# DecaYale/SYN3R

Hardware: AMD Instinct MI355X
Metric: llff_3view_train_loop_iters_per_sec (higher is better)
Workload: dtype f32 raster / f16 UNet (f32 accumulate); 1 GPU; LLFF fern-like 3-view block: 50 raster fwd+bwd iters (l1 loss) (200000 Gaussians, 1920x1080, SH3) + 1 SVD (step,pass): CFG UNet fwd [2,14,8,72,128] f16 + fused Euler step; frames=14, parallelism=scene-parallel x1

## Files before the change

include/syn3r_hip.h:

```cpp
#ifndef SYN3R_HIP_H
#define SYN3R_HIP_H

#include <stddef.h>
#include <stdint.h>

#ifdef __cplusplus
extern "C" {
#endif

#define SYN3R_OK 0
#define SYN3R_E_INVALID (-1)
#define SYN3R_E_WORKSPACE (-2)
#define SYN3R_E_HIP (-3)

#define SYN3R_F32 0
#define SYN3R_F16 1

const char* syn3r_last_error(void);
int syn3r_version(void);
const char* syn3r_arch(void);

int syn3r_trace_enable(int on);
void* syn3r_trace_session(void);
int syn3r_trace_attach(void* session);
// ... 119 lines not shown
                              float* dL_dconfidence, void* workspace, size_t workspace_bytes, int raw, int flags,
                              const float* filter3d, void* stream);
int syn3r_raster_backward_abs(int N, int sh_degree, int sh_coeffs, long long P, const float* means3D,
                              const float* scales, const float* rotations, const float* opacities, const float* shs,
                              const float* confidence, float scale_modifier, const float* viewmatrix,
                              const float* projmatrix, const float* campos, float tanfovx, float tanfovy, int H, int W,
                              const float* bg, const int* radii, void* geom, size_t geom_bytes,
                              const unsigned* point_list, void* image, size_t image_bytes, const float* dL_dcolor,
                              const float* dL_ddepth, const float* dL_dalpha, float* dL_dmeans3D, float* dL_dscales,
                              float* dL_drotations, float* dL_dopacities, float* dL_dshs, float* dL_dmeans2D,
                              float* dL_dconfidence, void* workspace, size_t workspace_bytes, int raw, int flags,
                              const float* filter3d, float* dL_dmeans2D_abs, void* stream);
size_t syn3r_raster_backward_cam_workspace_bytes(int N);
int syn3r_raster_backward_cam(int N, int sh_degree, int sh_coeffs, long long P, const float* means3D,
                              const float* scales, const float* rotations, const float* opacities, const float* shs,
                              const float* confidence, float scale_modifier, const float* viewmatrix,
                              const float* projmatrix, const float* campos, float tanfovx, float tanfovy, int H, int W,
                              const float* bg, const int* radii, void* geom, size_t geom_bytes,
                              const unsigned* point_list, void* image, size_t image_bytes, const float* dL_dcolor,
                              const float* dL_ddepth, const float* dL_dalpha, float* dL_dmeans3D, float* dL_dscales,
                              float* dL_drotations, float* dL_dopacities, float* dL_dshs, float* dL_dmeans2D,
                              float* dL_dconfidence, void* workspace, size_t workspace_bytes, int raw, int flags,
                              const float* filter3d, float* dL_dmeans2D_abs, float* dL_dcamera, int accumulate,
                              void* stream);

size_t syn3r_sort_pairs_workspace_bytes(long long n);
int syn3r_sort_pairs(unsigned long long* keys, unsigned* vals, unsigned long long* keys_tmp, unsigned* vals_tmp,
                     long long n, int nbits, void* workspace, size_t workspace_bytes, int* result_in_tmp,
                     void* stream);


int syn3r_gemm_f16(const void* A, long long lda, const void* W, void* out, long long ldc, const void* bias,
                   const void* rowvec, long long ldrv, int rows_per_vec, int rv_group_rows, const void* residual, long long ldr,
                   const void* aux, long long ldaux, float s_acc, float s_res, float s_aux, int M, int N, int K,
                   void* gn_partials, size_t gn_partials_bytes, int* gn_written, void* stream);

int syn3r_gemm_2src_supported(int M, int N, int K1, int K2, long long lda1, long long lda2);
int syn3r_gemm_2src_f16(const void* A1, long long lda1, int K1, const void* A2, long long lda2, int K2, const void* W,
                        void* out, long long ldc, const void* bias, int M, int N, void* gn_partials, size_t gn_partials_bytes,
                        int* gn_written, void* stream);

int syn3r_gemm_set_tile(int bm);

int syn3r_gemm_set_splitk_workspace(void* workspace, size_t bytes);

int syn3r_gemm_geglu_f16(const void* A, long long lda, const void* Wpacked, const void* bias_packed, void* out,
                         long long ldc, int M, int D, int K, void* stream);

size_t syn3r_feedforward_workspace_bytes(int M, int D);
int syn3r_feedforward_f16(const void* x, long long ldx, const void* w1_packed, const void* b1_packed, int D,
                          const void* w2, const void* b2, void* out, long long ldc, const void* residual,
                          long long ldr, const void* aux, long long ldaux, float s_acc, float s_res, float s_aux,
                          int M, int C_in, int C_out, void* workspace, size_t workspace_bytes, void* stream);

int syn3r_feedforward_p64_supported(int M, int D, int C_in);
int syn3r_feedforward_p64_f16(const void* x, long long ldx, const void* w1_packed64, const void* b1_packed64, int D,
                              const void* w2, const void* b2, void* out, long long ldc, const void* residual,
                              long long ldr, const void* aux, long long ldaux, float s_acc, float s_res, float s_aux,
                              int M, int C_in, int C_out, void* workspace, size_t workspace_bytes, void* stream);

int syn3r_feedforward_fused_f16(const void* x, long long ldx, const void* w1_chunked, const void* b1_chunked, int D,
                                const void* w2, const void* b2, void* out, long long ldc, const void* residual,
                                long long ldr, const void* aux, long long ldaux, float s_acc, float s_res, float s_aux,
                                int M, int C, void* stream);

int syn3r_feedforward_fused_ln_f16(const void* x, long long ldx, const void* ln_gamma, const void* ln_beta, float ln_eps,
                                   const void* w1_chunked, const void* b1_chunked, int D, const void* w2, const void* b2,
                                   void* out, long long ldc, const void* residual, long long ldr, const void* aux,
                                   long long ldaux, float s_acc, float s_res, float s_aux, int M, int C, void* stream);

int syn3r_feedforward_fused_addln_f16(const void* x, long long ldx, const void* addvec, int rows_per_vec, const void* ln_gamma,
                                      const void* ln_beta, float ln_eps, const void* w1_chunked, const void* b1_chunked, int D,
                                      const void* w2, const void* b2, void* out, long long ldc, const void* aux, long long ldaux,
                                      float s_acc, float s_res, float s_aux, int M, int C, void* stream);

int syn3r_layernorm_linear320_f16(const void* x, long long ldx, const void* ln_gamma, const void* ln_beta, float ln_eps,
                                  const void* W, void* out, long long ldc, int M, int N, int C, void* stream);

int syn3r_conv2d3x3_f16(const void* X, const void* W, void* out, long long ldc, const void* bias,
                        const void* rowvec, long long ldrv, int rows_per_vec, const void* residual, long long ldr,
                        float s_acc, float s_res, int NB, int Hi, int Wi, int Cin, int Cout, int stride, int upsample,
                        int pad_lo, void* gn_partials, size_t gn_partials_bytes, int* gn_written, void* stream);

int syn3r_tconv3_f16(const void* X, const void* W, void* out, long long ldc, const void* bias, const void* rowvec,
                     long long ldrv, int rows_per_vec, const void* residual, long long ldr, float s_acc, float s_res,
                     int B, int F, int HW, int Cin, int Cout, void* gn_partials, size_t gn_partials_bytes, int* gn_written,
                     void* stream);

int syn3r_attention_f16(const void* q, const void* k, const void* v, long long ld, void* out, long long ldo,
                        int nseq, int S, int heads, void* stream);

int syn3r_attention_temporal_f16(const void* q, const void* k, const void* v, long long ld, void* out,
                                 long long ldo, int B, int F, int HW, int heads, void* stream);

size_t syn3r_groupnorm_workspace_bytes(int samples, int rows);
int syn3r_groupnorm_f16(const void* x, void* y, int samples, int rows, int C, const void* gamma, const void* beta,
                        float eps, int silu, void* workspace, size_t workspace_bytes, void* stream);
int syn3r_groupnorm_2src_f16(const void* x1, int C1, const void* x2, int C2, void* y, int samples, int rows,
                             const void* gamma, const void* beta, float eps, int silu, void* workspace,
                             size_t workspace_bytes, void* stream);
size_t syn3r_gn_partials_bytes(int M, int N);
int syn3r_groupnorm_pre_f16(const void* x1, int C1, const void* part1, const void* x2, int C2, const void* part2, void* y,
                            int samples, int rows, const void* gamma, const void* beta, float eps, int silu,
                            void* workspace, size_t workspace_bytes, void* stream);

int syn3r_layernorm_f16(const void* x, void* y, void* xsum, const void* addvec, int rows_per_vec, long long M,
                        int C, const void* gamma, const void* beta, float eps, void* stream);

int syn3r_geglu_f16(const void* x, void* y, long long M, int D, void* stream);

int syn3r_softmax_rows_f16(const void* x, void* y, long long M, int N, long long ld, float scale, void* stream);

int syn3r_time_conv_out(const void* x, long long ldx, const float* w, const float* bias, float* out, int B, int F,
                        long long HW, void* stream);


size_t syn3r_l1_loss_workspace_bytes(long long n);
int syn3r_l1_loss(const float* image, const float* target, long long n, float weight, float* loss, void* ws,
                  size_t ws_bytes, void* stream);
int syn3r_l1_loss_backward(const float* image, const float* target, long long n, float weight,
                           const float* grad_loss, float* grad_image, void* stream);

int syn3r_image_mse(const float* image, const float* target, long long n, float* mse, void* ws, size_t ws_bytes,
                    void* stream);

size_t syn3r_photo_loss_workspace_bytes(int C, int H, int W);
int syn3r_photo_loss(const float* image, const float* target, int C, int H, int W, float lambda_dssim, float weight,
                     float* loss3, void* ws, size_t ws_bytes, void* stream);
int syn3r_photo_loss_backward(const float* image, const float* target, int C, int H, int W, float lambda_dssim,
                              float weight, const float* grad_loss, const void* ws, float* grad_image, void* stream);
int syn3r_photo_loss_step(const float* image, const float* target, int C, int H, int W, float lambda_dssim, float weight,
                          const float* grad_loss, float* loss3, float* grad_image, void* ws, size_t ws_bytes, void* stream);

size_t syn3r_photo_loss_map_workspace_bytes(int C, int H, int W);
int syn3r_photo_loss_map(const float* image, const float* target, const float* map, int C, int H, int W, float lambda_dssim,
                         float weight, float* loss4, void* ws, size_t ws_bytes, void* stream);
int syn3r_photo_loss_map_backward(const float* image, const float* target, const float* map, int C, int H, int W,
                                  float lambda_dssim, float weight, const float* grad_loss, const void* ws, float* grad_image,
                                  void* stream);
int syn3r_photo_loss_map_step(const float* image, const float* target, const float* map, int C, int H, int W, float lambda_dssim,
                              float weight, const float* grad_loss, float* loss4, float* grad_image, void* ws, size_t ws_bytes,
                              void* stream);
int syn3r_l1_loss_map(const float* image, const float* target, const float* map, long long n, long long plane, float weight,
                      float* loss, void* ws, size_t ws_bytes, void* stream);
int syn3r_l1_loss_map_backward(const float* image, const float* target, const float* map, long long n, long long plane,
                               float weight, const float* grad_loss, float* grad_image, void* stream);

#define SYN3R_DCORR_MIN 0
#define SYN3R_DCORR_A 1
#define SYN3R_DCORR_B 2
size_t syn3r_depth_corr_loss_workspace_bytes(long long n);
int syn3r_depth_corr_loss(const float* depth, const float* prior, long long n, float weight, float offset, int mode, float* parts,
                          void* ws, size_t ws_bytes, void* stream);
int syn3r_depth_corr_loss_backward(const float* depth, const float* prior, long long n, float weight, float offset, int mode,
                                   const float* grad_loss, const void* ws, size_t ws_bytes, float* grad_depth, void* stream);
int syn3r_depth_corr_loss_step(const float* depth, const float* prior, long long n, float weight, float offset, int mode,
                               const float* grad_loss, float* parts, float* grad_depth, void* ws, size_t ws_bytes, void* stream);

int syn3r_exposure_apply(const float* image, const float* A, int H, int W, float* out, void* stream);
size_t syn3r_exposure_backward_workspace_bytes(int H, int W);
int syn3r_exposure_backward(const float* image, const float* A, const float* grad_out, int H, int W, float* grad_image, float* grad_A,
                            int accumulate, void* ws, size_t ws_bytes, void* stream);

int syn3r_adam_step(float* param, const float* grad, float* exp_avg, float* exp_avg_sq, long long n, float lr,
                    float beta1, float beta2, float eps, int step, void* stream);
int syn3r_adam_step_multi(int count, float* const* params, const float* const* grads, float* const* exp_avgs,
// ... 74 lines not shown
```

syn3r_amd/_lib.py:

```python
from __future__ import annotations

import ctypes as C
from pathlib import Path

import torch

_LIB_PATH = Path(__file__).resolve().parent / "lib" / "libsyn3r_hip.so"
_lib = None

c_f = C.c_float
c_i = C.c_int
c_p = C.c_void_p
c_sz = C.c_size_t
c_ll = C.c_longlong
c_d = C.c_double

F32, F16 = 0, 1
RASTER_ANTIALIAS = 1

FILTER3D_VARIANCE, FILTER3D_NEAR, FILTER3D_MARGIN = 0.2, 0.2, 0.15

_SCENE = [c_p, c_p, c_p, c_p, c_p, c_p, c_f, c_p, c_p, c_p, c_f, c_f, c_i, c_i]
_RASTER_PREPROCESS = [c_i, c_i, c_i] + _SCENE + [c_p, c_p, c_sz, C.POINTER(c_ll)]
_RASTER_BACKWARD = ([c_i, c_i, c_i, c_ll] + _SCENE + [c_p, c_p, c_p, c_sz, c_p, c_p, c_sz]
                    + [c_p] * 10 + [c_p, c_sz])
_STREAM, _EX, _F3D, _ABS = [c_p], [c_i, c_i, c_p], [c_i, c_i, c_p, c_p], [c_i, c_i, c_p, c_p, c_p]
_CAM = [c_i, c_i, c_p, c_p, c_p, c_i, c_p]
CAMERA_GRAD = 35

SIGNATURES = {
    "syn3r_last_error": (C.c_char_p, []),
    "syn3r_version": (c_i, []),
    "syn3r_arch": (C.c_char_p, []),
    "syn3r_trace_enable": (c_i, [c_i]),
    "syn3r_trace_filter": (c_i, [C.c_char_p]),
    "syn3r_trace_report": (c_i, [C.c_char_p, c_sz]),
    "syn3r_trace_session": (c_p, []),
    "syn3r_trace_attach": (c_i, [c_p]),
    "syn3r_inverse_warp_workspace_bytes": (c_sz, [c_i]),
    "syn3r_inverse_warp": (c_i, [c_p, c_p, c_p, c_p, c_p, c_p, c_p, c_f, c_i, c_i, c_i,
                                 c_p, c_p, c_p, c_p, c_p, c_p, c_p, c_p, c_p, c_p, c_p, c_p, c_sz, c_p]),
    "syn3r_reproj_error": (c_i, [c_p, c_p, c_p, c_p, c_p, c_p, c_p, c_i, c_i, c_p, c_p]),
    "syn3r_warp_post": (c_i, [c_p, c_p, c_p, c_i, c_i, c_i, c_i, c_i, c_p, c_p, c_p, c_p, c_p, c_p, c_p]),
    "syn3r_fuse_uncertainty": (c_i, [c_p, c_p, c_p, c_i, c_i, c_i, c_i, c_i, c_p, c_p, c_p, c_p]),
    "syn3r_forward_warp_workspace_bytes": (c_sz, [c_i, c_i]),
    "syn3r_forward_warp": (c_i, [c_p, c_p, c_p, c_p, c_p, c_p, c_i, c_i, c_p, c_p, c_p, c_p, c_sz, c_p]),
    "syn3r_step_workspace_bytes": (c_sz, [c_i, c_i, c_i, c_i]),
    "syn3r_step_interp": (c_i, [c_p, c_i, c_p, c_i, c_p, c_p, c_p, c_f, c_f, c_f, c_f, c_f, c_f, c_i,
                                c_p, c_p, c_p, c_i, c_i, c_i, c_i, c_p, c_sz, c_p]),
    "syn3r_step_replace": (c_i, [c_p, c_i, c_p, c_i, c_p, c_p, c_p, c_f, c_f, c_f, c_f,
                                 c_p, c_p, c_i, c_i, c_i, c_i, c_p, c_sz, c_p]),
    "syn3r_raster_geom_bytes": (c_sz, [c_i]),
    "syn3r_raster_image_bytes": (c_sz, [c_i, c_i]),
    "syn3r_raster_binning_bytes": (c_sz, [c_ll]),
    "syn3r_raster_preprocess": (c_i, _RASTER_PREPROCESS + _STREAM),
    "syn3r_raster_preprocess_raw": (c_i, _RASTER_PREPROCESS + _STREAM),
    "syn3r_raster_preprocess_ex": (c_i, _RASTER_PREPROCESS + _EX),
    "syn3r_raster_preprocess_f3d": (c_i, _RASTER_PREPROCESS + _F3D),
    "syn3r_raster_render": (c_i, [c_i, c_i, c_i, c_p, c_p, c_p, c_sz, c_p, c_sz, c_p, c_sz, c_ll, c_p, c_p, c_p,
                                  C.POINTER(c_p), c_p]),
    "syn3r_raster_backward_workspace_bytes": (c_sz, [c_i]),
    "syn3r_raster_backward": (c_i, _RASTER_BACKWARD + _STREAM),
    "syn3r_raster_backward_raw": (c_i, _RASTER_BACKWARD + _STREAM),
    "syn3r_raster_backward_ex": (c_i, _RASTER_BACKWARD + _EX),
    "syn3r_raster_backward_f3d": (c_i, _RASTER_BACKWARD + _F3D),
    "syn3r_raster_backward_abs": (c_i, _RASTER_BACKWARD + _ABS),
    "syn3r_raster_backward_cam_workspace_bytes": (c_sz, [c_i]),
    "syn3r_raster_backward_cam": (c_i, _RASTER_BACKWARD + _CAM),
    "syn3r_filter3d_workspace_bytes": (c_sz, [c_i]),
    "syn3r_filter3d_compute": (c_i, [c_p, c_i, c_p, c_i, c_f, c_f, c_f, c_p, c_p, c_sz, c_p]),
    "syn3r_sort_pairs_workspace_bytes": (c_sz, [c_ll]),
    "syn3r_sort_pairs": (c_i, [c_p, c_p, c_p, c_p, c_ll, c_i, c_p, c_sz, C.POINTER(c_i), c_p]),
    "syn3r_gaussian_activate": (c_i, [c_i, c_p, c_p, c_p, c_p, c_p, c_p, c_p]),
    "syn3r_gaussian_activate_backward": (c_i, [c_i, c_p, c_p, c_p, c_p, c_p, c_p, c_p, c_p, c_p, c_p, c_p]),
    "syn3r_densification_stats": (c_i, [c_i, c_p, c_p, c_p, c_p, c_p, c_p]),
    "syn3r_densification_stats_abs": (c_i, [c_i, c_p, c_p, c_p, c_p, c_p, c_p, c_p, c_p]),
    "syn3r_gemm_f16": (c_i, [c_p, c_ll, c_p, c_p, c_ll, c_p, c_p, c_ll, c_i, c_i, c_p, c_ll, c_p, c_ll, c_f, c_f, c_f,
                             c_i, c_i, c_i, c_p, c_sz, C.POINTER(c_i), c_p]),
    "syn3r_gemm_set_tile": (c_i, [c_i]),
    "syn3r_gemm_geglu_f16": (c_i, [c_p, c_ll, c_p, c_p, c_p, c_ll, c_i, c_i, c_i, c_p]),
    "syn3r_feedforward_workspace_bytes": (c_sz, [c_i, c_i]),
    "syn3r_feedforward_f16": (c_i, [c_p, c_ll, c_p, c_p, c_i, c_p, c_p, c_p, c_ll, c_p, c_ll, c_p, c_ll, c_f, c_f, c_f,
                                    c_i, c_i, c_i, c_p, c_sz, c_p]),
    "syn3r_feedforward_p64_f16": (c_i, [c_p, c_ll, c_p, c_p, c_i, c_p, c_p, c_p, c_ll, c_p, c_ll, c_p, c_ll, c_f, c_f, c_f,
                                    c_i, c_i, c_i, c_p, c_sz, c_p]),
    "syn3r_feedforward_p64_supported": (c_i, [c_i, c_i, c_i]),
    "syn3r_feedforward_fused_f16": (c_i, [c_p, c_ll, c_p, c_p, c_i, c_p, c_p, c_p, c_ll, c_p, c_ll, c_p, c_ll, c_f, c_f, c_f,
                                          c_i, c_i, c_p]),
    "syn3r_feedforward_fused_ln_f16": (c_i, [c_p, c_ll, c_p, c_p, c_f, c_p, c_p, c_i, c_p, c_p, c_p, c_ll, c_p, c_ll, c_p, c_ll,
                                             c_f, c_f, c_f, c_i, c_i, c_p]),
    "syn3r_feedforward_fused_addln_f16": (c_i, [c_p, c_ll, c_p, c_i, c_p, c_p, c_f, c_p, c_p, c_i, c_p, c_p, c_p, c_ll, c_p, c_ll,
                                                c_f, c_f, c_f, c_i, c_i, c_p]),
    "syn3r_layernorm_linear320_f16": (c_i, [c_p, c_ll, c_p, c_p, c_f, c_p, c_p, c_ll, c_i, c_i, c_i, c_p]),
    "syn3r_conv2d3x3_f16": (c_i, [c_p, c_p, c_p, c_ll, c_p, c_p, c_ll, c_i, c_p, c_ll, c_f, c_f,
                                  c_i, c_i, c_i, c_i, c_i, c_i, c_i, c_i, c_p, c_sz, C.POINTER(c_i), c_p]),
    "syn3r_tconv3_f16": (c_i, [c_p, c_p, c_p, c_ll, c_p, c_p, c_ll, c_i, c_p, c_ll, c_f, c_f,
                               c_i, c_i, c_i, c_i, c_i, c_p, c_sz, C.POINTER(c_i), c_p]),
    "syn3r_attention_f16": (c_i, [c_p, c_p, c_p, c_ll, c_p, c_ll, c_i, c_i, c_i, c_p]),
    "syn3r_attention_temporal_f16": (c_i, [c_p, c_p, c_p, c_ll, c_p, c_ll, c_i, c_i, c_i, c_i, c_p]),
    "syn3r_groupnorm_workspace_bytes": (c_sz, [c_i, c_i]),
    "syn3r_groupnorm_f16": (c_i, [c_p, c_p, c_i, c_i, c_i, c_p, c_p, c_f, c_i, c_p, c_sz, c_p]),
    "syn3r_groupnorm_2src_f16": (c_i, [c_p, c_i, c_p, c_i, c_p, c_i, c_i, c_p, c_p, c_f, c_i, c_p, c_sz, c_p]),
    "syn3r_groupnorm_pre_f16": (c_i, [c_p, c_i, c_p, c_p, c_i, c_p, c_p, c_i, c_i, c_p, c_p, c_f, c_i, c_p, c_sz, c_p]),
    "syn3r_gn_partials_bytes": (c_sz, [c_i, c_i]),
    "syn3r_gemm_2src_supported": (c_i, [c_i, c_i, c_i, c_i, c_ll, c_ll]),
    "syn3r_gemm_2src_f16": (c_i, [c_p, c_ll, c_i, c_p, c_ll, c_i, c_p, c_p, c_ll, c_p, c_i, c_i, c_p, c_sz, C.POINTER(c_i), c_p]),
    "syn3r_layernorm_f16": (c_i, [c_p, c_p, c_p, c_p, c_i, c_ll, c_i, c_p, c_p, c_f, c_p]),
    "syn3r_geglu_f16": (c_i, [c_p, c_p, c_ll, c_i, c_p]),
    "syn3r_softmax_rows_f16": (c_i, [c_p, c_p, c_ll, c_i, c_ll, c_f, c_p]),
    "syn3r_time_conv_out": (c_i, [c_p, c_ll, c_p, c_p, c_p, c_i, c_i, c_ll, c_p]),
    "syn3r_l1_loss_workspace_bytes": (c_sz, [c_ll]),
    "syn3r_l1_loss": (c_i, [c_p, c_p, c_ll, c_f, c_p, c_p, c_sz, c_p]),
    "syn3r_l1_loss_backward": (c_i, [c_p, c_p, c_ll, c_f, c_p, c_p, c_p]),
    "syn3r_image_mse": (c_i, [c_p, c_p, c_ll, c_p, c_p, c_sz, c_p]),
    "syn3r_photo_loss_workspace_bytes": (c_sz, [c_i, c_i, c_i]),
    "syn3r_photo_loss": (c_i, [c_p, c_p, c_i, c_i, c_i, c_f, c_f, c_p, c_p, c_sz, c_p]),
    "syn3r_photo_loss_backward": (c_i, [c_p, c_p, c_i, c_i, c_i, c_f, c_f, c_p, c_p, c_p, c_p]),
    "syn3r_photo_loss_step": (c_i, [c_p, c_p, c_i, c_i, c_i, c_f, c_f, c_p, c_p, c_p, c_p, c_sz, c_p]),
    "syn3r_photo_loss_map_workspace_bytes": (c_sz, [c_i, c_i, c_i]),
    "syn3r_photo_loss_map": (c_i, [c_p, c_p, c_p, c_i, c_i, c_i, c_f, c_f, c_p, c_p, c_sz, c_p]),
    "syn3r_photo_loss_map_backward": (c_i, [c_p, c_p, c_p, c_i, c_i, c_i, c_f, c_f, c_p, c_p, c_p, c_p]),
    "syn3r_photo_loss_map_step": (c_i, [c_p, c_p, c_p, c_i, c_i, c_i, c_f, c_f, c_p, c_p, c_p, c_p, c_sz, c_p]),
    "syn3r_l1_loss_map": (c_i, [c_p, c_p, c_p, c_ll, c_ll, c_f, c_p, c_p, c_sz, c_p]),
    "syn3r_l1_loss_map_backward": (c_i, [c_p, c_p, c_p, c_ll, c_ll, c_f, c_p, c_p, c_p]),
    "syn3r_depth_corr_loss_workspace_bytes": (c_sz, [c_ll]),
    "syn3r_depth_corr_loss": (c_i, [c_p, c_p, c_ll, c_f, c_f, c_i, c_p, c_p, c_sz, c_p]),
    "syn3r_depth_corr_loss_backward": (c_i, [c_p, c_p, c_ll, c_f, c_f, c_i, c_p, c_p, c_sz, c_p, c_p]),
    "syn3r_depth_corr_loss_step": (c_i, [c_p, c_p, c_ll, c_f, c_f, c_i, c_p, c_p, c_p, c_p, c_sz, c_p]),
    "syn3r_exposure_apply": (c_i, [c_p, c_p, c_i, c_i, c_p, c_p]),
    "syn3r_exposure_backward_workspace_bytes": (c_sz, [c_i, c_i]),
    "syn3r_exposure_backward": (c_i, [c_p, c_p, c_p, c_i, c_i, c_p, c_p, c_i, c_p, c_sz, c_p]),
    "syn3r_adam_step": (c_i, [c_p, c_p, c_p, c_p, c_ll, c_f, c_f, c_f, c_f, c_i, c_p]),
    "syn3r_adam_step_multi": (c_i, [c_i, c_p, c_p, c_p, c_p, c_p, c_p, c_f, c_f, c_p, c_p, c_p]),
    "syn3r_adam_step_multi_rows": (c_i, [c_i, c_p, c_p, c_p, c_p, c_p, c_p, c_p, c_p, c_p, c_f, c_f, c_p, c_p, c_p]),
    "syn3r_knn3_workspace_bytes": (c_sz, [c_i]),
    "syn3r_knn3_mean_dist2": (c_i, [c_p, c_i, c_p, c_p, c_sz, c_p]),
    "syn3r_knn3_graph_workspace_bytes": (c_sz, [c_i]),
    "syn3r_knn3_graph": (c_i, [c_p, c_i, c_p, c_p, c_p, c_sz, c_p]),
    "syn3r_gaussian_unpool_workspace_bytes": (c_sz, [c_i]),
    "syn3r_gaussian_unpool_count": (c_i, [c_p, c_p, c_i, c_f, c_f, c_p, c_p, c_sz, c_p]),
    "syn3r_gaussian_unpool_emit": (c_i, [c_p, c_p, c_p, c_p, c_p, c_i, c_i, c_i, c_p, c_p, c_p, c_p, c_p, c_p, c_sz, c_p]),
    "syn3r_conv2d3x3_act_f16": (c_i, [c_p, c_p, c_p, c_p, c_i, c_p, c_i, c_i, c_i, c_i, c_i, c_p]),
    "syn3r_lpips_image_f16": (c_i, [c_p, c_i, c_i, c_p, c_p]),
    "syn3r_lpips_image_bwd": (c_i, [c_p, c_i, c_i, c_f, c_p, c_p]),
    "syn3r_maxpool2_f16": (c_i, [c_p, c_i, c_i, c_i, c_p, c_p]),
    "syn3r_maxpool2_bwd_f16": (c_i, [c_p, c_p, c_i, c_i, c_i, c_p, c_p]),
    "syn3r_lpips_layer_workspace_bytes": (c_sz, [c_ll, c_i]),
    "syn3r_lpips_layer_f16": (c_i, [c_p, c_p, c_p, c_ll, c_i, c_i, c_p, c_p, c_sz, c_p]),
    "syn3r_lpips_layer_bwd_f16": (c_i, [c_p, c_p, c_p, c_ll, c_i, c_f, c_i, c_p, c_p]),
    "syn3r_conv2d3x3_split_f16": (c_i, [c_p, c_p, c_p, c_ll, c_p, c_i, c_i, c_p, c_ll, c_i, c_i, c_i, c_i, c_i, c_p]),
    "syn3r_lpips_image_split_f16": (c_i, [c_p, c_i, c_i, c_p, c_p]),
    "syn3r_maxpool2_split_f16": (c_i, [c_p, c_i, c_i, c_i, c_p, c_p]),
    "syn3r_maxpool2_bwd_split_f16": (c_i, [c_p, c_p, c_i, c_i, c_i, c_p, c_p]),
    "syn3r_lpips_layer_split_f16": (c_i, [c_p, c_p, c_p, c_ll, c_i, c_i, c_p, c_p, c_sz, c_p]),
    "syn3r_lpips_layer_bwd_split_f16": (c_i, [c_p, c_p, c_p, c_ll, c_i, c_f, c_i, c_p, c_p]),
    "syn3r_pcd_outlier_workspace_bytes": (c_sz, [c_i]),
    "syn3r_pcd_statistical_outlier": (c_i, [c_p, c_i, c_i, c_d, c_p, c_p, c_p, c_p, c_sz, c_p]),
    "syn3r_flow_cycle_mask": (c_i, [c_p, c_p, c_i, c_i, c_i, c_f, c_p, c_p, c_p]),
    "syn3r_gemm_set_splitk_workspace": (c_i, [c_p, c_sz]),
    "syn3r_unet_create": (c_i, [C.c_char_p, C.c_char_p, C.POINTER(c_p)]),
    "syn3r_unet_destroy": (c_i, [c_p]),
    "syn3r_unet_workspace_bytes": (c_sz, [c_p, c_i, c_i, c_i, c_i, c_i]),
    "syn3r_unet_forward": (c_i, [c_p, c_p, c_d, c_p, c_i, c_p, c_p, c_i, c_i, c_i, c_i, c_i, c_p, c_sz, c_p]),
}


class Syn3rError(RuntimeError):
    pass


def lib_path() -> Path:
    return _LIB_PATH


def set_library_path(path) -> None:
    global _LIB_PATH
    if _lib is not None:
        raise Syn3rError("set_library_path() after the library was loaded")
# ... 119 lines not shown
```

syn3r_amd/csrc/gemm.hip:

```cpp
#include "common.h"
#include <cstdlib>
#include <algorithm>
#include <atomic>
#include <type_traits>

using namespace syn3r;

namespace {

#include "gemm_common.h"
#include "gemm_dma160.h"
#include "gemm_dma.h"
#include "gemm_wide.h"
#include "gemm_z.h"
#include "gemm_dmap.h"
#include "gemm_dmapd.h"
#include "gemm_g256.h"
#include "gemm_ffn.h"

int persistent_blocks() {
    static std::atomic<int> cus_of[64];
    static const int forced = tune_env("SYN3R_PERSISTENT_BLOCKS", 0);
    if (forced > 0) return forced < 8 ? 8 : forced;
    int dev = 0;
// ... 1 lines not shown
    int n = cus_of[dev].load(std::memory_order_relaxed);
    if (n == 0) {
        int v = 0;
        n = (hipDeviceGetAttribute(&v, hipDeviceAttributeMultiprocessorCount, dev) == hipSuccess && v > 0) ? v : 256;
        if (n < 8) n = 8;
        cus_of[dev].store(n, std::memory_order_relaxed);
    }
    return n;
}

size_t gn_partials_bytes(long long M, long long N) { return (size_t)(M / 32) * 2 * (size_t)(N / 10) * sizeof(float); }
int gn_request(GemmParams& p, void* buf, size_t bytes, const char* who) {
    SYN3R_REQUIRE((buf == nullptr) == (bytes == 0), "%s: gn_partials pointer and size must both be given or both be zero", who);
    SYN3R_REQUIRE(((uintptr_t)buf % 16) == 0, "%s: the gn_partials buffer must be 16-byte aligned", who);
    if (!buf || p.M % 32 != 0 || p.N % 80 != 0 || p.geglu_D > 0 || p.out_tiled || bytes < gn_partials_bytes(p.M, p.N)) return SYN3R_OK;
    p.gn_part = (float*)buf; p.gn_units = p.N / 10;
    return SYN3R_OK;
}

template <void (*KERNEL)(GemmParams)>
int launch_tiles(const char* family, size_t lds, long long grid, int block, hipStream_t stream, const GemmParams& q, int* gn_written,
                 const char* base, int b0 = 0, int b1 = 0) {
    static DevOnce once;
    if (int rc = set_max_lds(once, (const void*)KERNEL, (int)lds, family)) return rc;
    char name[96];
    if (trace_on()) {
        const int n = snprintf(name, sizeof(name), base, b0, b1);
        if (trace_detail()) snprintf(name + n, sizeof(name) - n, "[M%d,N%d,K%d,e%d]", q.M, q.N, q.K, q.geglu_D > 0 ? 2 : (q.residual != nullptr));
    }
    SYN3R_LAUNCH_NAMED(name, KERNEL, dim3((unsigned)grid), dim3(block), lds, stream, q);
    hipError_t e = hipGetLastError();
    if (e != hipSuccess) { set_error("%s launch: %s", family, hipGetErrorString(e)); return SYN3R_E_HIP; }
    if (gn_written) *gn_written = q.gn_part != nullptr;
    return SYN3R_OK;
}

long long wide_tiles(const GemmParams& p) { return (long long)((p.M + WBM - 1) / WBM) * ((p.N + WBN - 1) / WBN); }
bool wide_fills(const GemmParams& p) {
    const long long tiles = wide_tiles(p), rounds = (tiles + 255) / 256;
    return tiles * 10 >= rounds * 256 * 8;
}

int band_width(const GemmParams& p) {
    static const int band_env = tune_env("SYN3R_Z_BAND", 0);
    if (band_env > 0) return band_env;
    return ((p.N + WBN - 1) / WBN > 4 && p.K <= 640) ? 3 : 4;
}

int launch_widep(const GemmParams& p, hipStream_t stream, int* gn_written) {
    constexpr size_t lds = (size_t)2 * W_STAGE + 16384;
    static_assert(8 * WM * EPI_LD * sizeof(__half) <= lds - W_STAGE, "epilogue staging must fit behind ring slot 0");
    GemmParams q = p;
    q.band = band_width(p);
    return launch_tiles<k_gemm_widep>("gemm_widep", lds, std::min<long long>(wide_tiles(p), persistent_blocks()), 512, stream, q, gn_written, "k_gemm_widep");
}

bool g256_admits(const GemmParams& p) {
    return p.geglu_D > 0 && p.bias != nullptr && p.out_tiled && !p.a_tiled && !p.A2 && !p.rowvec && !p.residual && !p.aux && p.s_acc == 1.0f && p.M % 128 == 0 && p.M >= 256 &&
           p.geglu_D % 128 == 0 && p.N == 2 * p.geglu_D && p.K >= 2 * BK && p.lda % 8 == 0 && (long long)p.M * p.lda < (1ll << 31) &&
           (long long)p.N * p.K < (1ll << 31);
}
int launch_g256(const GemmParams& p, hipStream_t stream) {
    const int tiles = ((p.M + 255) / 256) * (p.N / 256);
    GemmParams q = p;
    static const int band_env = tune_env("SYN3R_G256_BAND", 0);
    q.band = band_env > 0 ? band_env : 4;
    return launch_tiles<k_gemm_g256>("gemm_g256", G_LDS, std::min(tiles, persistent_blocks()), 512, stream, q, nullptr, "k_gemm_g256");
}

template <int MODE = MODE_DENSE>
int launch_z(const GemmParams& p, hipStream_t stream, int* gn_written) {
    const long long blocks = std::min<long long>(wide_tiles(p), persistent_blocks());
    GemmParams q = p;
    q.band = band_width(p);
    if constexpr (MODE == MODE_CONV2D) q.a_bytes = (unsigned)((long long)(p.M / (p.Ho * p.Wo)) * p.Hi * p.Wi * p.Cin * 2);
    if constexpr (MODE == MODE_TCONV) q.a_bytes = (unsigned)((long long)p.M * p.Cin * 2);
    if constexpr (MODE == MODE_DENSE) {
        if (p.A2) return launch_tiles<k_gemm_z<true, MODE_DENSE>>("gemm_z", Z_LDS, blocks, 512, stream, q, gn_written, "k_gemm_z<%d>", MODE);
    }
    if constexpr (MODE == MODE_CONV2D) {
        if (p.ups) return launch_tiles<k_gemm_z<false, MODE_CONV2D, true>>("gemm_z", Z_LDS, blocks, 512, stream, q, gn_written, "k_gemm_z<%d>", MODE);
    }
    return launch_tiles<k_gemm_z<false, MODE>>("gemm_z", Z_LDS, blocks, 512, stream, q, gn_written, "k_gemm_z<%d>", MODE);
}

thread_local int g_dma_bm = 0;
thread_local void* g_splitk_ws = nullptr;
thread_local size_t g_splitk_bytes = 0;

int wide_launch(const GemmParams& p, hipStream_t stream, int* gn_written) {
    static const int z_env = tune_env("SYN3R_GEMM_Z", -1);
    const bool z = g_dma_bm == -322 ? true : (g_dma_bm == -320 ? false : (z_env < 0 ? p.geglu_D > 0 : z_env != 0));
    return z ? launch_z<MODE_DENSE>(p, stream, gn_written) : launch_widep(p, stream, gn_written);
}

bool widep_admits(const GemmParams& p) {
    const bool lean = (!p.rowvec || p.geglu_D <= 0) && (!p.aux || p.residual) && (p.geglu_D <= 0 || (p.geglu_D % 8 == 0 && p.s_acc == 1.0f));
    const bool small = (p.a_tiled ? (long long)((p.M + 127) / 128) * 128 * p.K : (long long)p.M * p.lda) < (1ll << 31) &&
                       (long long)p.N * p.K < (1ll << 31) && (!p.A2 || (long long)p.M * p.lda2 < (1ll << 31));
    return lean && small && p.M % 8 == 0 && p.N % 8 == 0 && p.M >= 8 && p.N >= 8;
}

long long tiles256(const GemmParams& p) { return (long long)((p.M + 255) / 256) * ((p.N + BN - 1) / BN); }

int launch_dmapd(const GemmParams& p, hipStream_t stream) {
    return launch_tiles<k_gemm_dmapd>("gemm_dmapd", DMA256_LDS, std::min<long long>(tiles256(p), persistent_blocks()), 512, stream, p, nullptr, "k_gemm_dmapd");
}

bool dmapd_admits(const GemmParams& p) {
    return p.geglu_D <= 0 && !p.A2 && !p.a_tiled && !p.out_tiled && !p.out_nt && !p.relu && !p.relu_mask && p.ksplit <= 1 && !p.aux &&
           !p.res_add && p.M % 256 == 0 && p.N % BN == 0 && p.K / BK >= 4 && p.ldc % 8 == 0 && (!p.residual || p.ldr % 8 == 0) &&
           (!p.rowvec || p.ldrv % 4 == 0);
}

template <int MODE>
int launch_dmap(const GemmParams& p, hipStream_t stream, int* gn_written) {
    static_assert(8 * 32 * EPI_LD * sizeof(__half) <= DMA256_STAGE, "the two-pass epilogue staging must fit in one ring slot");
    GemmParams q = p;
    q.tc_pb = q.tc_nf = 0;
    if constexpr (MODE == MODE_TCONV) {
        static const int tc_env = tune_env("SYN3R_TCONV_ORDER", 1);
        if (tc_env != 0 && p.HW % 256 == 0 && p.M % p.HW == 0 && p.M / p.HW > 1) { q.tc_pb = p.HW / 256; q.tc_nf = p.M / p.HW; }
    }
    return launch_tiles<k_gemm_dmap<MODE>>("gemm_dmap", DMA256_LDS, std::min<long long>(tiles256(p), persistent_blocks()), 512, stream, q, gn_written, "k_gemm_dmap<%d>", MODE);
}

template <int MODE, int BM>
int launch_dma_bm(const GemmParams& p, hipStream_t stream, int* gn_written) {
    if constexpr (BM == 256) {
        static const int pers_env = tune_env("SYN3R_DMA_PERSISTENT", 1);
        if (pers_env != 0 && MODE != MODE_CONV2D && p.geglu_D <= 0 && (!p.aux || p.residual) && p.N % 8 == 0 && p.N >= 8)
            return launch_dmap<MODE>(p, stream, gn_written);
    }
    constexpr size_t lds = BM == 256 ? DMA256_LDS : 2 * (BM * BK * 2 + DMA_B_BYTES);
    static_assert((BM / 32) * WM * EPI_LD * sizeof(__half) <= lds, "epilogue staging must fit in the ring");
    const int tiles = ((p.M + BM - 1) / BM) * ((p.N + BN - 1) / BN);
    return launch_tiles<k_gemm_dma<MODE, BM>>("gemm_dma", lds, tiles, BM * 2, stream, p, nullptr, "k_gemm_dma<%d,%d>", MODE, BM);
}

template <int MODE>
int launch_splitk(const GemmParams& p, hipStream_t stream, bool* done) {
    const long long tiles = tiles256(p);
    const int nkt_all = p.K / BK;
    const int S = (tiles * 4 <= 256 && nkt_all % 4 == 0 && nkt_all >= 16) ? 4 : ((tiles * 2 <= 256 && nkt_all % 2 == 0 && nkt_all >= 8) ? 2 : 1);
    const size_t need = (size_t)S * p.M * p.N * sizeof(float);
    if (S == 1 || g_dma_bm != 0 || !g_splitk_ws || need > g_splitk_bytes || p.N % 8 != 0 || p.M < 8 || p.relu || p.relu_mask ||
        p.geglu_D > 0 || p.out_tiled || (p.A2 && (MODE != MODE_DENSE || p.a_tiled || (p.K1 / BK) % (nkt_all / S) != 0)))
        return SYN3R_OK;
    GemmParams q = p;
    q.ksplit = S; q.split_ws = (float*)g_splitk_ws;
    if (int rc = launch_tiles<k_gemm_dma<MODE, 256>>("gemm split-K", DMA256_LDS, tiles * S, 512, stream, q, nullptr,
                                                     trace_detail() ? "k_gemm_dma<%d,256>/%d" : "k_gemm_dma<%d,256>/k", MODE, S))
        return rc;
    const long long chunks = (long long)p.M * (p.N / 8);
    SYN3R_LAUNCH(k_splitk_finish, dim3((unsigned)((chunks + 255) / 256)), dim3(256), 0, stream, q);
    SYN3R_LAUNCH_CHECK("gemm split-K launch");
    *done = true;
    return SYN3R_OK;
}

template <int MODE>
int launch_dma(const GemmParams& p, hipStream_t stream, int* gn_written = nullptr) {
    static const int wide_env = tune_env("SYN3R_GEMM_WIDE", -1);
    if constexpr (MODE == MODE_DENSE) {
        static const int ddw_env = tune_env("SYN3R_DMAPD_WIDE", 1);
        const bool won = p.residual ? (p.K >= 640 && p.K <= 1280 && p.N <= 1280) : (p.K == 1280 && p.N == 1280);
// ... 279 lines not shown
    return feedforward_fused(x, ldx, ln_gamma, ln_beta, ln_eps, w1_chunked, b1_chunked, D, w2, b2, out, ldc, residual, ldr, aux, ldaux,
                             s_acc, s_res, s_aux, M, C, stream);
}
extern "C" int syn3r_feedforward_fused_addln_f16(const void* x, long long ldx, const void* addvec, int rows_per_vec, const void* ln_gamma,
                                                 const void* ln_beta, float ln_eps, const void* w1_chunked, const void* b1_chunked, int D,
                                                 const void* w2, const void* b2, void* out, long long ldc, const void* aux, long long ldaux,
                                                 float s_acc, float s_res, float s_aux, int M, int C, void* stream) {
    SYN3R_REQUIRE(ln_gamma && ln_beta && addvec, "feedforward_fused_addln_f16: null LayerNorm parameters / add vector");
    SYN3R_REQUIRE(((uintptr_t)ln_gamma | (uintptr_t)ln_beta | (uintptr_t)addvec) % 16 == 0, "feedforward_fused_addln_f16: LayerNorm parameters and the add vector must be 16-byte aligned");
    SYN3R_REQUIRE(ln_eps > 0.f, "feedforward_fused_addln_f16: eps must be positive");
    SYN3R_REQUIRE(rows_per_vec > 0, "feedforward_fused_addln_f16: rows_per_vec=%d must be positive", rows_per_vec);
    return feedforward_fused(x, ldx, ln_gamma, ln_beta, ln_eps, w1_chunked, b1_chunked, D, w2, b2, out, ldc, x, ldx, aux, ldaux,
                             s_acc, s_res, s_aux, M, C, stream, addvec, rows_per_vec);
}
namespace {
int feedforward_fused(const void* x, long long ldx, const void* ln_gamma, const void* ln_beta, float ln_eps, const void* w1_chunked,
                      const void* b1_chunked, int D, const void* w2, const void* b2, void* out, long long ldc, const void* residual,
                      long long ldr, const void* aux, long long ldaux, float s_acc, float s_res, float s_aux, int M, int C, void* stream,
                      const void* addvec, int rows_per_vec) {
    SYN3R_REQUIRE(x && w1_chunked && b1_chunked && w2 && out, "feedforward_fused_f16: null operand");
    SYN3R_REQUIRE(C == F_C, "feedforward_fused_f16: the fused kernel is built for C = %d channels (got %d): use syn3r_feedforward_f16", F_C, C);
    SYN3R_REQUIRE(M > 0 && D >= F_HC && D % F_HC == 0, "feedforward_fused_f16: bad sizes M=%d D=%d (D must be a multiple of %d)", M, D, F_HC);
    FfnParams q{};
    GemmParams& p = q.e;
    p.A = (const __half*)x; p.lda = ldx; p.W = (const __half*)w2; p.out = (__half*)out; p.ldc = ldc;
    p.bias = (const __half*)b2; p.residual = (const __half*)residual; p.ldr = ldr; p.aux = (const __half*)aux; p.ldaux = ldaux;
    p.s_acc = s_acc; p.s_res = s_res; p.s_aux = s_aux; p.M = M; p.N = F_C; p.K = D;
    q.w1 = (const __half*)w1_chunked; q.b1 = (const __half*)b1_chunked; q.D = D;
    q.ln_g = (const __half*)ln_gamma; q.ln_b = (const __half*)ln_beta; q.ln_eps = ln_eps;
    q.ln_add = (const __half*)addvec; q.ln_add_rpv = rows_per_vec; p.res_add = (const __half*)addvec; p.res_add_rpv = rows_per_vec;
    int rc = check_common(p, "feedforward_fused_f16");
    if (rc) return rc;
    SYN3R_REQUIRE(ldx % 8 == 0 && ldx >= C, "feedforward_fused_f16: ldx=%lld must be >= C and a multiple of 8", ldx);
    SYN3R_REQUIRE(((uintptr_t)w1_chunked | (uintptr_t)b1_chunked) % 16 == 0, "feedforward_fused_f16: weights must be 16-byte aligned");
    return launch_ffn320(q, (hipStream_t)stream);
}
}

extern "C" int syn3r_layernorm_linear320_f16(const void* x, long long ldx, const void* ln_gamma, const void* ln_beta, float ln_eps,
                                             const void* W, void* out, long long ldc, int M, int N, int C, void* stream) {
    SYN3R_REQUIRE(x && ln_gamma && ln_beta && W && out, "layernorm_linear320_f16: null operand");
    SYN3R_REQUIRE(C == F_C, "layernorm_linear320_f16: the kernel is built for C = %d channels (got %d): use syn3r_layernorm_f16 + syn3r_gemm_f16", F_C, C);
    SYN3R_REQUIRE(SYN3R_DIM_OK(M) && SYN3R_DIM_OK(N) && N % F_C == 0, "layernorm_linear320_f16: bad sizes M=%d N=%d (N must be a multiple of %d)", M, N, F_C);
    SYN3R_REQUIRE(ldx % 8 == 0 && ldx >= C && ldc % 8 == 0 && ldc >= N, "layernorm_linear320_f16: bad strides ldx=%lld ldc=%lld", ldx, ldc);
    SYN3R_REQUIRE(((uintptr_t)x | (uintptr_t)ln_gamma | (uintptr_t)ln_beta | (uintptr_t)W | (uintptr_t)out) % 16 == 0, "layernorm_linear320_f16: operands must be 16-byte aligned");
    SYN3R_REQUIRE(ln_eps > 0.f, "layernorm_linear320_f16: eps must be positive");
    SYN3R_REQUIRE((long long)M * ldx < (1ll << 40) && (long long)M * ldc < (1ll << 40), "layernorm_linear320_f16: operand too large");
    LnLinParams p{};
    p.x = (const __half*)x; p.ldx = ldx; p.W = (const __half*)W; p.out = (__half*)out; p.ldc = ldc; p.M = M; p.N = N; p.C = C;
    p.ln_g = (const __half*)ln_gamma; p.ln_b = (const __half*)ln_beta; p.ln_eps = ln_eps;
    return launch_lnlin320(p, (hipStream_t)stream);
}

extern "C" int syn3r_conv2d3x3_f16(const void* X, const void* W, void* out, long long ldc, const void* bias,
                                   const void* rowvec, long long ldrv, int rows_per_vec, const void* residual,
                                   long long ldr, float s_acc, float s_res, int NB, int Hi, int Wi, int Cin, int Cout,
                                   int stride, int upsample, int pad_lo, void* gn_partials, size_t gn_partials_bytes, int* gn_written,
                                   void* stream) {
    if (gn_written) *gn_written = 0;
    SYN3R_REQUIRE(NB > 0 && Hi > 0 && Wi > 0 && Cin > 0 && Cout > 0, "conv2d3x3: bad sizes");
    SYN3R_REQUIRE(pad_lo == 0 || pad_lo == 1, "conv2d3x3: pad_lo must be 0 or 1");
    SYN3R_REQUIRE(stride == 1 || stride == 2, "conv2d3x3: stride must be 1 or 2");
    SYN3R_REQUIRE(!(upsample && stride != 1), "conv2d3x3: upsample requires stride 1");
    SYN3R_REQUIRE(Cin % BK == 0, "conv2d3x3: Cin=%d must be a multiple of %d (pad the input channels)", Cin, BK);
    GemmParams p{};
    p.A = (const __half*)X; p.W = (const __half*)W; p.out = (__half*)out; p.ldc = ldc; p.bias = (const __half*)bias;
    p.rowvec = (const __half*)rowvec; p.ldrv = ldrv; p.rows_per_vec = rows_per_vec;
    p.residual = (const __half*)residual; p.ldr = ldr; p.s_acc = s_acc; p.s_res = s_res; p.s_aux = 0.f;
    p.Hi = Hi; p.Wi = Wi; p.Cin = Cin; p.stride = stride; p.ups = upsample ? 1 : 0; p.pad = pad_lo;
    int Hg = upsample ? 2 * Hi : Hi, Wg = upsample ? 2 * Wi : Wi;
    p.Ho = (Hg + pad_lo + 1 - 3) / stride + 1;
    p.Wo = (Wg + pad_lo + 1 - 3) / stride + 1;
    SYN3R_REQUIRE(p.Ho > 0 && p.Wo > 0, "conv2d3x3: input too small");
    long long M = (long long)NB * p.Ho * p.Wo;
    SYN3R_REQUIRE(M < (1ll << 31), "conv2d3x3: too many output pixels");
    p.M = (int)M; p.N = Cout; p.K = 9 * Cin;
    int rc = gn_request(p, gn_partials, gn_partials_bytes, "conv2d3x3");
    if (rc) return rc;
    rc = check_common(p, "conv2d3x3");
    if (rc) return rc;
    return launch_dma<MODE_CONV2D>(p, (hipStream_t)stream, gn_written);
}

extern "C" int syn3r_conv2d3x3_act_f16(const void* X, const void* W, void* out, const void* bias, int relu, const void* relu_mask,
                                       int NB, int Hi, int Wi, int Cin, int Cout, void* stream) {
    SYN3R_REQUIRE(NB > 0 && Hi > 0 && Wi > 0 && Cin > 0 && Cout > 0, "conv2d3x3_act: bad sizes");
    SYN3R_REQUIRE(Cin % BK == 0 && Cout % 8 == 0, "conv2d3x3_act: Cin=%d must be a multiple of %d, Cout=%d of 8", Cin, BK, Cout);
    GemmParams p{};
    p.A = (const __half*)X; p.W = (const __half*)W; p.out = (__half*)out; p.ldc = Cout; p.bias = (const __half*)bias;
    p.s_acc = 1.0f; p.s_res = 0.f; p.s_aux = 0.f;
    p.relu = relu ? 1 : 0; p.relu_mask = (const __half*)relu_mask;
    p.Hi = Hi; p.Wi = Wi; p.Cin = Cin; p.stride = 1; p.ups = 0; p.pad = 1; p.Ho = Hi; p.Wo = Wi;
    long long M = (long long)NB * Hi * Wi;
    SYN3R_REQUIRE(M < (1ll << 31), "conv2d3x3_act: too many output pixels");
    p.M = (int)M; p.N = Cout; p.K = 9 * Cin;
    int rc = check_common(p, "conv2d3x3_act");
    if (rc) return rc;
    SYN3R_REQUIRE(((uintptr_t)relu_mask % 16) == 0, "conv2d3x3_act: mask must be 16-byte aligned");
    return launch_dma<MODE_CONV2D>(p, (hipStream_t)stream);
}

extern "C" int syn3r_conv2d3x3_split_f16(const void* X, const void* W, void* out, long long ld_out, const void* bias, int relu, int split_out,
                                         const void* relu_mask, long long ld_mask, int NB, int Hi, int Wi, int Cin, int Cout, void* stream) {
    SYN3R_REQUIRE(NB > 0 && Hi > 0 && Wi > 0 && Cin > 0 && Cout > 0, "conv2d3x3_split: bad sizes");
    SYN3R_REQUIRE(Cin % BK == 0 && Cout % 8 == 0, "conv2d3x3_split: Cin=%d must be a multiple of %d, Cout=%d of 8", Cin, BK, Cout);
    SYN3R_REQUIRE(ld_out >= (split_out ? 2ll : 1ll) * Cout, "conv2d3x3_split: ld_out=%lld is short of %d columns", ld_out, (split_out ? 2 : 1) * Cout);
    SYN3R_REQUIRE(!(split_out && relu_mask), "conv2d3x3_split: a mask goes with the plain output only");
    SYN3R_REQUIRE(!relu_mask || (ld_mask >= Cout && ld_mask % 8 == 0 && ld_mask < (1ll << 31)), "conv2d3x3_split: bad mask stride %lld", ld_mask);
    GemmParams p{};
    p.A = (const __half*)X; p.W = (const __half*)W; p.out = (__half*)out; p.ldc = ld_out; p.bias = (const __half*)bias;
    p.s_acc = 1.0f; p.s_res = 0.f; p.s_aux = 0.f;
    p.relu = relu ? 1 : 0; p.relu_mask = (const __half*)relu_mask; p.ld_mask = (int)ld_mask;
    p.Hi = Hi; p.Wi = Wi; p.Cin = Cin; p.stride = 1; p.ups = 0; p.pad = 1; p.Ho = Hi; p.Wo = Wi;
    long long M = (long long)NB * Hi * Wi;
    SYN3R_REQUIRE(M < (1ll << 31), "conv2d3x3_split: too many output pixels");
    p.M = (int)M; p.N = Cout; p.K = 9 * Cin;
    int rc = check_common(p, "conv2d3x3_split");
    if (rc) return rc;
    SYN3R_REQUIRE((((uintptr_t)relu_mask | (uintptr_t)bias) % 16) == 0, "conv2d3x3_split: mask and bias must be 16-byte aligned");
    static_assert(8 * WM * EPI_LD * sizeof(__half) <= DMA256_LDS, "one staged fp16 plane must fit in the ring");
    if (split_out)
        return launch_tiles<k_gemm_dma<MODE_CONV2D, 256, EPI_SPLIT_OUT>>("conv split", DMA256_LDS, tiles256(p), 512, (hipStream_t)stream, p, nullptr, "k_gemm_dma<1,256,split>");
    return launch_tiles<k_gemm_dma<MODE_CONV2D, 256, EPI_SPLIT_MASK>>("conv split", DMA256_LDS, tiles256(p), 512, (hipStream_t)stream, p, nullptr, "k_gemm_dma<1,256,mask>");
}

extern "C" int syn3r_tconv3_f16(const void* X, const void* W, void* out, long long ldc, const void* bias,
                                const void* rowvec, long long ldrv, int rows_per_vec, const void* residual,
                                long long ldr, float s_acc, float s_res, int B, int F, int HW, int Cin, int Cout,
                                void* gn_partials, size_t gn_partials_bytes, int* gn_written, void* stream) {
    if (gn_written) *gn_written = 0;
    SYN3R_REQUIRE(B > 0 && F > 0 && HW > 0 && Cin > 0 && Cout > 0, "tconv3: bad sizes");
    SYN3R_REQUIRE(Cin % BK == 0, "tconv3: Cin=%d must be a multiple of %d", Cin, BK);
    GemmParams p{};
    p.A = (const __half*)X; p.W = (const __half*)W; p.out = (__half*)out; p.ldc = ldc; p.bias = (const __half*)bias;
    p.rowvec = (const __half*)rowvec; p.ldrv = ldrv; p.rows_per_vec = rows_per_vec;
    p.residual = (const __half*)residual; p.ldr = ldr; p.s_acc = s_acc; p.s_res = s_res; p.s_aux = 0.f;
    p.F = F; p.HW = HW; p.Cin = Cin;
    long long M = (long long)B * F * HW;
    SYN3R_REQUIRE(M < (1ll << 31), "tconv3: too many rows");
    p.M = (int)M; p.N = Cout; p.K = 3 * Cin;
    int rc = gn_request(p, gn_partials, gn_partials_bytes, "tconv3");
    if (rc) return rc;
    rc = check_common(p, "tconv3");
    if (rc) return rc;
    return launch_dma<MODE_TCONV>(p, (hipStream_t)stream, gn_written);
}

#ifdef SYN3R_TIMING
extern "C" __attribute__((visibility("default"))) int syn3r_debug_wide_timing(unsigned long long* out64) {
    return (int)hipMemcpyFromSymbol(out64, HIP_SYMBOL(g_wide_timing), sizeof(unsigned long long) * 64);
}
extern "C" __attribute__((visibility("default"))) int syn3r_debug_g256_timing(unsigned long long* out64) {
    return (int)hipMemcpyFromSymbol(out64, HIP_SYMBOL(g_g256_timing), sizeof(unsigned long long) * 64);
}
#endif
```

syn3r_amd/csrc/gemm_common.h:

```cpp


typedef _Float16 half8 __attribute__((ext_vector_type(8)));
typedef float float4v __attribute__((ext_vector_type(4)));
typedef unsigned u32x4 __attribute__((ext_vector_type(4)));

constexpr int BN = 160, BK = 64;
constexpr int WM = 64, WN = 80;
constexpr int TM = WM / 16, TN = WN / 16;
constexpr int B_TILE = BN * BK;
constexpr int EPI_LD = 88;

enum { MODE_DENSE = 0, MODE_CONV2D = 1, MODE_TCONV = 2 };

__device__ __forceinline__ int rowvec_index(int m, int rows_per_vec, int rv_group) {
    if (rows_per_vec > 0) return m / rows_per_vec;
    const int P = -rows_per_vec;
    return (rv_group > 0 ? (m / rv_group) * P : 0) + m % P;
}

struct GemmParams {
    const __half* A; long long lda;
    const __half* W;
    __half* out; long long ldc;
    const __half* bias;
    const __half* rowvec; long long ldrv; int rows_per_vec;
    int rv_group;
    const __half* residual; long long ldr;
    const __half* aux; long long ldaux;
    float s_acc, s_res, s_aux;
    int M, N, K;
    int Ho, Wo, Hi, Wi, Cin, stride, ups, pad;
    int F, HW;
    int tc_pb, tc_nf;
    int geglu_D;
    int out_tiled;
    int out_nt;
    int a_tiled;
    const __half* A2; long long lda2; int K1;
    const __half* res_add; int res_add_rpv;
    int band;
    int ksplit; float* split_ws;
    int relu;
    int ld_mask;
    const __half* relu_mask;
    float* gn_part; int gn_units;
    unsigned a_bytes;
};

__device__ __forceinline__ long long tiled_off(int m, int d, int D) {
    return ((long long)(m >> 7) * (D >> 6) + (d >> 6)) * 8192 + (m & 127) * 64 + (d & 63);
}

struct XcdTiles { unsigned start, len, stride; };
__device__ __forceinline__ XcdTiles xcd_tiles(unsigned nblk) {
    const unsigned xcd = blockIdx.x % 8, q8 = nblk / 8, r8 = nblk % 8;
    XcdTiles t;
    t.start = xcd < r8 ? xcd * (q8 + 1) : r8 * (q8 + 1) + (xcd - r8) * q8;
    t.len = q8 + (xcd < r8 ? 1u : 0u);
    t.stride = (gridDim.x - xcd + 7) / 8;
    return t;
}

__device__ __forceinline__ int swz(int row, int chunk) { return row * BK + ((chunk ^ (row & 7)) << 3); }

#define OUT_STORE(ptr, val) do { if (p.out_nt) __builtin_nontemporal_store((val), (ptr)); else *(ptr) = (val); } while (0)

template <int PREFETCH_RES = 1, bool RES_ADD = false>
__device__ __forceinline__ void gemm_epilogue(const GemmParams& p, float4v (&acc)[TM][TN], char* smem_raw, int lane,
                                              int wv, int wm, int wn, int m0, int n0, int tile_n) {
    const int fr = lane & 15, fq = lane >> 4;
    __half* st = (__half*)smem_raw + wv * (WM * EPI_LD);
    const int gm0 = m0 + wm * WM, gn0 = n0 + wn * WN;
    typedef _Float16 half4e __attribute__((ext_vector_type(4)));
    half8 res[WM * (WN / 8) / 64];
    half8 radd[RES_ADD ? WM * (WN / 8) / 64 : 1];
    auto prefetch_residual = [&]() {
#pragma unroll
        for (int it = 0; it < WM * (WN / 8) / 64; ++it) {
            const int q = lane + it * 64;
            int row = q / (WN / 8), ch = q - row * (WN / 8);
            int m = gm0 + row, n = gn0 + ch * 8;
            if (m < p.M && n + 8 <= p.N) {
                res[it] = *(const half8*)(p.residual + (long long)m * p.ldr + n);
                if constexpr (RES_ADD) { if (p.res_add) radd[it] = *(const half8*)(p.res_add + (long long)(m / p.res_add_rpv) * p.N + n); }
            } else {
#pragma unroll
                for (int e = 0; e < 8; ++e) res[it][e] = (m < p.M && n + e < p.N) ? ((const _Float16*)p.residual)[(long long)m * p.ldr + n + e] : (_Float16)0.f;
            }
        }
    };
    if (PREFETCH_RES == 1 && p.residual && p.geglu_D <= 0) prefetch_residual();
    float bias4[TN][4];
#pragma unroll
    for (int j = 0; j < TN; ++j) {
        const int n = gn0 + j * 16 + fq * 4;
#pragma unroll
        for (int r = 0; r < 4; ++r) bias4[j][r] = 0.0f;
        if (p.bias) {
            if (n + 4 <= p.N) {
                half4e b = *(const half4e*)(p.bias + n);
#pragma unroll
                for (int r = 0; r < 4; ++r) bias4[j][r] = (float)b[r];
            } else {
                for (int r = 0; r < 4; ++r) if (n + r < p.N) bias4[j][r] = __half2float(p.bias[n + r]);
            }
        }
    }
#pragma unroll
    for (int i = 0; i < TM; ++i) {
        const int row = i * 16 + fr;
        const int m = gm0 + row;
        const __half* rv = nullptr;
        if (p.rowvec && m < p.M) {
            const int vi = rowvec_index(m, p.rows_per_vec, p.rv_group);
            rv = p.rowvec + (long long)vi * p.ldrv;
        }
#pragma unroll
        for (int j = 0; j < TN; ++j) {
            const int col = j * 16 + fq * 4;
            const int n = gn0 + col;
            float add[4];
#pragma unroll
            for (int r = 0; r < 4; ++r) add[r] = bias4[j][r];
            if (rv) {
                if (n + 4 <= p.N) {
                    half4e t = *(const half4e*)(rv + n);
#pragma unroll
                    for (int r = 0; r < 4; ++r) add[r] += (float)t[r];
                } else {
// ... 153 lines not shown
```

syn3r_amd/csrc/gemm_wide.h:

```cpp

constexpr int WBM = 256, WBN = 320, WTN = 10;
constexpr int W_A_BYTES = WBM * BK * 2;
constexpr int W_B_BYTES = WBN * BK * 2;
constexpr int W_STAGE = W_A_BYTES + W_B_BYTES;

#ifdef SYN3R_TIMING
__device__ unsigned long long g_wide_timing[64];
#endif

template <int NI>
__device__ __forceinline__ void gn_tile_stats(const GemmParams& p, const __half* st, int lane, int gm0, int gn0, int N) {
    typedef _Float16 half2e __attribute__((ext_vector_type(2)));
    constexpr int NU = NI == 4 ? 8 : 4, NC = NI == 4 ? 10 : 5;
    const int row = NI == 4 ? lane : (lane & 31);
    const int half_ = NI == 4 ? 0 : (lane >> 5);
    float s[NU], q[NU];
#pragma unroll
    for (int u = 0; u < NU; ++u) { s[u] = 0.f; q[u] = 0.f; }
    const half2e one = {(_Float16)1.0f, (_Float16)1.0f};
    const __half* src = st + row * EPI_LD + half_ * 40;
#pragma unroll
    for (int c = 0; c < NC; ++c) {
        const half8 v = *(const half8*)(src + c * 8);
#pragma unroll
        for (int k = 0; k < 4; ++k) {
            const half2e pr = {v[2 * k], v[2 * k + 1]};
            s[(4 * c + k) / 5] = __builtin_amdgcn_fdot2(pr, one, s[(4 * c + k) / 5], false);
            q[(4 * c + k) / 5] = __builtin_amdgcn_fdot2(pr, pr, q[(4 * c + k) / 5], false);
        }
    }
    float w[NU];
#pragma unroll
    for (int u = 0; u < NU; ++u) {
        auto r = __builtin_amdgcn_permlane16_swap(__float_as_int(s[u]), __float_as_int(q[u]), false, false);
        w[u] = __int_as_float(r[0]) + __int_as_float(r[1]);
        w[u] += __int_as_float(__builtin_amdgcn_update_dpp(0, __float_as_int(w[u]), 0x128 , 0xF, 0xF, false));
        w[u] += __int_as_float(__builtin_amdgcn_update_dpp(0, __float_as_int(w[u]), 0x124 , 0xF, 0xF, false));
        w[u] += __int_as_float(__builtin_amdgcn_update_dpp(0, __float_as_int(w[u]), 0x122 , 0xF, 0xF, false));
        w[u] += __int_as_float(__builtin_amdgcn_update_dpp(0, __float_as_int(w[u]), 0x121 , 0xF, 0xF, false));
    }
    if ((lane & 15) == 0) {
        const int rowp = lane >> 4;
        const int m = gm0 + (NI == 4 ? 32 * (rowp >> 1) : 0);
        const int n = gn0 + (NI == 4 ? 0 : 40 * (rowp >> 1));
        if (m < p.M && n < N) {
            float* dst = p.gn_part + ((size_t)(m >> 5) * 2 + (rowp & 1)) * (size_t)p.gn_units + n / 10;
#pragma unroll
            for (int u = 0; u < NU; u += 4) *(float4v*)(dst + u) = (float4v){w[u], w[u + 1], w[u + 2], w[u + 3]};
        }
    }
}

template <int NI, bool HOIST = false>
__device__ __forceinline__ void lean_store(const GemmParams& p, float4v (*acc)[TN], __half* st, int lane, int gm0,
                                           int gn0, int N, const __half* bias, const __half* residual, const __half* aux, bool full) {
    typedef _Float16 half4e __attribute__((ext_vector_type(4)));
    const int fr = lane & 15, fq = lane >> 4;
    const __half* rv[NI];
    if (p.rowvec) {
#pragma unroll
        for (int i = 0; i < NI; ++i) {
            const int m = gm0 + i * 16 + fr;
            const int vi = m < p.M ? rowvec_index(m, p.rows_per_vec, p.rv_group) : 0;
            rv[i] = p.rowvec + (long long)vi * p.ldrv;
        }
    }
    if constexpr (HOIST) {
        half4e bq[TN], rq[NI][TN];
#pragma unroll
        for (int j = 0; j < TN; ++j) {
            const int n = gn0 + j * 16 + fq * 4;
            bq[j] = (half4e){(_Float16)0.f, (_Float16)0.f, (_Float16)0.f, (_Float16)0.f};
            if (bias && n < N) bq[j] = *(const half4e*)(bias + n);
#pragma unroll
            for (int i = 0; i < NI; ++i) {
                rq[i][j] = (half4e){(_Float16)0.f, (_Float16)0.f, (_Float16)0.f, (_Float16)0.f};
                if (p.rowvec && n < N) rq[i][j] = *(const half4e*)(rv[i] + n);
            }
        }
#pragma unroll
        for (int j = 0; j < TN; ++j) {
            float b4[4];
#pragma unroll
            for (int r = 0; r < 4; ++r) b4[r] = (float)bq[j][r];
#pragma unroll
            for (int i = 0; i < NI; ++i) {
                float a4[4] = {b4[0], b4[1], b4[2], b4[3]};
                if (p.rowvec) {
#pragma unroll
                    for (int r = 0; r < 4; ++r) a4[r] += (float)rq[i][j][r];
                }
                half4e o;
#pragma unroll
                for (int r = 0; r < 4; ++r) o[r] = (_Float16)((acc[i][j][r] + a4[r]) * p.s_acc);
                *(half4e*)(st + (i * 16 + fr) * EPI_LD + j * 16 + fq * 4) = o;
            }
        }
    } else {
#pragma unroll
        for (int j = 0; j < TN; ++j) {
            const int n = gn0 + j * 16 + fq * 4;
            float b4[4] = {0.f, 0.f, 0.f, 0.f};
            if (bias && n < N) {
                const half4e b = *(const half4e*)(bias + n);
#pragma unroll
                for (int r = 0; r < 4; ++r) b4[r] = (float)b[r];
            }
#pragma unroll
            for (int i = 0; i < NI; ++i) {
                float a4[4] = {b4[0], b4[1], b4[2], b4[3]};
                if (p.rowvec && n < N) {
                    const half4e t = *(const half4e*)(rv[i] + n);
#pragma unroll
                    for (int r = 0; r < 4; ++r) a4[r] += (float)t[r];
                }
                half4e o;
#pragma unroll
                for (int r = 0; r < 4; ++r) o[r] = (_Float16)((acc[i][j][r] + a4[r]) * p.s_acc);
                *(half4e*)(st + (i * 16 + fr) * EPI_LD + j * 16 + fq * 4) = o;
            }
        }
    }
    __builtin_amdgcn_wave_barrier();
    static_assert(NI % 2 == 0, "lean_store: an even number of row tiles");
    constexpr int NQ = NI * 16 * (WN / 8) / 64;
    auto put = [&](int m, int n, const half8& v) {
        if (!(full || (m < p.M && n < N))) return;
        if (p.out_tiled) OUT_STORE((half8*)(p.out + tiled_off(m, n, N)), v);
        else OUT_STORE((half8*)(p.out + (long long)m * p.ldc + n), v);
    };
    if (residual && aux) {
        constexpr int RB = 5;
#pragma unroll
        for (int h5 = 0; h5 < NQ; h5 += RB) {
            half8 res[RB], ax[RB];
#pragma unroll
            for (int it = 0; it < RB; ++it) {
                const int q = lane + (h5 + it) * 64, row = q / (WN / 8), ch = q - row * (WN / 8);
                int m = gm0 + row, n = gn0 + ch * 8;
                m = m < p.M ? m : p.M - 1; n = n < N ? n : N - 8;
                res[it] = *(const half8*)(residual + (long long)m * p.ldr + n);
                ax[it] = *(const half8*)(aux + (long long)m * p.ldaux + n);
            }
#pragma unroll
            for (int it = 0; it < RB; ++it) {
                const int q = lane + (h5 + it) * 64, row = q / (WN / 8), ch = q - row * (WN / 8);
                half8 v = *(const half8*)(st + row * EPI_LD + ch * 8);
#pragma unroll
                for (int e = 0; e < 8; ++e) {
                    float f = (float)v[e];
                    f += p.s_res * (float)res[it][e];
                    f += p.s_aux * (float)ax[it][e];
                    v[e] = (_Float16)f;
                }
                if (p.gn_part) *(half8*)(st + row * EPI_LD + ch * 8) = v;
                put(gm0 + row, gn0 + ch * 8, v);
            }
        }
    } else if (residual) {
        half8 res[NQ];
#pragma unroll
        for (int it = 0; it < NQ; ++it) {
            const int q = lane + it * 64, row = q / (WN / 8), ch = q - row * (WN / 8);
            int m = gm0 + row, n = gn0 + ch * 8;
            m = m < p.M ? m : p.M - 1; n = n < N ? n : N - 8;
            res[it] = *(const half8*)(residual + (long long)m * p.ldr + n);
        }
#pragma unroll
        for (int it = 0; it < NQ; ++it) {
            const int q = lane + it * 64, row = q / (WN / 8), ch = q - row * (WN / 8);
            half8 v = *(const half8*)(st + row * EPI_LD + ch * 8);
#pragma unroll
            for (int e = 0; e < 8; ++e) v[e] = (_Float16)((float)v[e] + p.s_res * (float)res[it][e]);
            if (p.gn_part) *(half8*)(st + row * EPI_LD + ch * 8) = v;
            put(gm0 + row, gn0 + ch * 8, v);
        }
    } else {
#pragma unroll
        for (int it = 0; it < NQ; ++it) {
            const int q = lane + it * 64, row = q / (WN / 8), ch = q - row * (WN / 8);
            const half8 v = *(const half8*)(st + row * EPI_LD + ch * 8);
            put(gm0 + row, gn0 + ch * 8, v);
        }
    }
    __builtin_amdgcn_wave_barrier();
    if (p.gn_part) {
        gn_tile_stats<NI>(p, st, lane, gm0, gn0, N);
        __builtin_amdgcn_wave_barrier();
    }
}

__device__ __forceinline__ void widep_store(const GemmParams& p, float4v (&acc)[TM][TN], char* epi, int lane, int wv, int gm0,
                                            int gn0, int N, const __half* bias, const __half* residual, const __half* aux, bool full) {
    lean_store<TM>(p, acc, (__half*)epi + wv * (WM * EPI_LD), lane, gm0, gn0, N, bias, residual, aux, full);
}

__global__ void __launch_bounds__(512, 2) k_gemm_widep(GemmParams p) {
    extern __shared__ __attribute__((aligned(16))) char smem_raw[];
    const int tid = threadIdx.x, lane = tid & 63;
    const int wv = __builtin_amdgcn_readfirstlane(tid >> 6);
    const int wm = wv >> 1, wn = wv & 1;
    const int tiles_n = (p.N + WBN - 1) / WBN;
    const int tiles_m = (p.M + WBM - 1) / WBM;
    const unsigned nblk = (unsigned)(tiles_m * tiles_n);
    const XcdTiles tiles = xcd_tiles(nblk);

    unsigned oa[4], ob[5];
    int m0 = 0, n0 = 0, tile_n = 0;
    const unsigned a_step = p.a_tiled ? 16384u : 2u * BK;
    const char* abase = (const char*)p.A;
    const int kt_switch = p.A2 ? p.K1 / BK : 0x7fffffff;
    int ks = 0;
    const unsigned bw0 = p.band > 0 ? (unsigned)p.band : 4u;
    const unsigned bw = (unsigned)tiles_n >= bw0 ? bw0 : (unsigned)tiles_n;
    const unsigned band_sz = (unsigned)tiles_m * bw, full_bands = (unsigned)tiles_n / bw;
    auto setup_tile = [&](unsigned tile) {
        unsigned b = tile / band_sz, w = bw, t2 = tile - b * band_sz;
        if (b >= full_bands) { b = full_bands; t2 = tile - full_bands * band_sz; w = (unsigned)tiles_n - full_bands * bw; }
        const int tile_m = (int)(t2 / w);
        tile_n = (int)(b * bw + t2 % w);
        m0 = tile_m * WBM; n0 = tile_n * WBN;
        ks = 0; abase = (const char*)p.A;
#pragma unroll
        for (int i = 0; i < 4; ++i) {
            int r = m0 + wv * 32 + i * 8;
            r = r < p.M - 8 ? r : p.M - 8;
            if (p.a_tiled) oa[i] = 2u * ((unsigned)(r >> 7) * (unsigned)(p.K >> 6) * 8192u + (unsigned)(r & 127) * 64u);
            else oa[i] = 2u * (unsigned)r * (unsigned)p.lda;
        }
#pragma unroll
        for (int j = 0; j < 5; ++j) {
            int n = n0 + (wv * 5 + j) * 8;
            n = n < p.N - 8 ? n : p.N - 8;
            ob[j] = 2u * (unsigned)n * (unsigned)p.K;
        }
    };
    unsigned voff_a = 0, voff_a2 = 0, voff_b = 0;
    auto issue_stage = [&](int buf, auto LOAD) {
        constexpr bool load = decltype(LOAD)::value;
        char* st = smem_raw + buf * W_STAGE;
        if (ks == kt_switch) {
            abase = (const char*)p.A2;
#pragma unroll
            for (int i = 0; i < 4; ++i) {
                int r = m0 + wv * 32 + i * 8;
                r = r < p.M - 8 ? r : p.M - 8;
                oa[i] = 2u * (unsigned)r * (unsigned)p.lda2;
            }
        }
        const unsigned va = ks >= kt_switch ? voff_a2 : voff_a;
        ++ks;
#pragma unroll
        for (int i = 0; i < 4; ++i) {
            if constexpr (load) __builtin_amdgcn_global_load_lds((gbl_void_t*)(abase + (size_t)(oa[i] + va)), (lds_void_t*)(st + (wv * 4 + i) * 1024), 16, 0, 0);
            oa[i] += a_step;
        }
#pragma unroll
        for (int j = 0; j < 5; ++j) {
            if constexpr (load) __builtin_amdgcn_global_load_lds((gbl_void_t*)((const char*)p.W + (size_t)(ob[j] + voff_b)), (lds_void_t*)(st + W_A_BYTES + (wv * 5 + j) * 1024), 16, 0, 0);
            ob[j] += 2u * BK;
        }
    };

    float4v acc[2][TM][TN];
    const int nkt = p.K / BK;
    const unsigned lds0 = (unsigned)(size_t)(__attribute__((address_space(3))) char*)smem_raw;
    unsigned a_row = 0, b_row = 0, swz[2] = {0, 0};
    const bool defer = wv >= 4;
    const bool xpf = (nkt & 1) == 0;
#ifdef SYN3R_TIMING
    unsigned long long tph[3] = {0, 0, 0}, tkt[2] = {0, 0}, tgate = 0, ntile = 0, t_a = __builtin_amdgcn_s_memtime();
    const unsigned long long t_begin = t_a, r_begin = __builtin_amdgcn_s_memrealtime();
#define PSTAMP(i) { __builtin_amdgcn_sched_barrier(0); const unsigned long long t_ = __builtin_amdgcn_s_memtime(); tph[i] += t_ - t_a; t_a = t_; __builtin_amdgcn_sched_barrier(0); }
#else
#define PSTAMP(i)
#endif
    bool staged = false;
// ... 135 lines not shown
```

syn3r_amd/csrc/gemm_z.h:

```cpp

constexpr int Z_SLOT1 = W_STAGE + 16384;
constexpr int Z_LDS = Z_SLOT1 + W_STAGE;

#define Z_DS_READ128(dst, addr, OFF) asm volatile("ds_read_b128 %0, %1 offset:%2" : "=v"(dst) : "v"(addr), "i"(OFF))

template <int KH, int NAF>
__device__ __forceinline__ void z_read_a(half8 (&af)[NAF][TM], const unsigned (&ra)[2]) {
    Z_DS_READ128(af[KH % NAF][0], ra[KH], 0); Z_DS_READ128(af[KH % NAF][1], ra[KH], 2048);
    Z_DS_READ128(af[KH % NAF][2], ra[KH], 4096); Z_DS_READ128(af[KH % NAF][3], ra[KH], 6144);
}
template <int Q, int RB>
__device__ __forceinline__ void z_read_b(half8 (&bf)[RB], const unsigned (&rb)[2]) {
    Z_DS_READ128(bf[Q % RB], rb[Q / 10], (Q % 10) * 2048);
}
template <int Q, int RB, int NAF>
__device__ __forceinline__ void z_mma(float4v (&acc)[2][TM][TN], half8 (&af)[NAF][TM], half8 (&bf)[RB]) {
    constexpr int kh = (Q / 10) % NAF, j = Q % 10;
#pragma unroll
    for (int i = 0; i < TM; ++i)
        acc[j / TN][i][j % TN] = __builtin_amdgcn_mfma_f32_16x16x32_f16(bf[Q % RB], af[kh][i], acc[j / TN][i][j % TN], 0, 0, 0);
    __builtin_amdgcn_sched_barrier(0);
}
template <int Q, int RB, int N, int NAF>
__device__ __forceinline__ void z_wait(half8 (&af)[NAF][TM], half8 (&bf)[RB]) {
    constexpr int kh = (Q / 10) % NAF, j = Q % 10;
    if constexpr (j == 0)
        asm volatile("s_waitcnt lgkmcnt(%5)" : "+v"(bf[Q % RB]), "+v"(af[kh][0]), "+v"(af[kh][1]), "+v"(af[kh][2]), "+v"(af[kh][3]) : "i"(N));
    else
        asm volatile("s_waitcnt lgkmcnt(%1)" : "+v"(bf[Q % RB]) : "i"(N));
}

template <bool TWOSRC, int MODE, bool UPS = false>
__global__ void __launch_bounds__(512, 2) k_gemm_z(GemmParams p) {
    static_assert(!UPS || MODE == MODE_CONV2D, "UPS is a conv2d option");
    extern __shared__ __attribute__((aligned(16))) char smem_raw[];
    const int tid = threadIdx.x, lane = tid & 63;
    const int wv = __builtin_amdgcn_readfirstlane(tid >> 6);
    const int wm = wv >> 1, wn = wv & 1;
    const int tiles_n = (p.N + WBN - 1) / WBN;
    const int tiles_m = (p.M + WBM - 1) / WBM;
    const unsigned nblk = (unsigned)(tiles_m * tiles_n);
    const XcdTiles tiles = xcd_tiles(nblk);
    const int nkt = p.K / BK;
    const unsigned bw0 = p.band > 0 ? (unsigned)p.band : 4u;
    const unsigned bw = (unsigned)tiles_n >= bw0 ? bw0 : (unsigned)tiles_n;
    const unsigned band_sz = (unsigned)tiles_m * bw, full_bands = (unsigned)tiles_n / bw;
    auto tile_origin = [&](unsigned tile, int& m0, int& n0, int& tn) {
        unsigned b = tile / band_sz, w = bw, t2 = tile - b * band_sz;
        if (b >= full_bands) { b = full_bands; t2 = tile - full_bands * band_sz; w = (unsigned)tiles_n - full_bands * bw; }
        tn = (int)(b * bw + t2 % w);
        m0 = (int)(t2 / w) * WBM; n0 = tn * WBN;
    };

    unsigned oa[4], ob[5];
    const unsigned a_step = p.a_tiled ? 16384u : 2u * BK;
    const char* abase = (const char*)p.A;
    const int kt_switch = TWOSRC ? p.K1 / BK : 0x7fffffff;
    unsigned c_tl = blockIdx.x / 8;
    int c_ks = 0, c_m0 = 0;
    unsigned c_slot = 0;
    unsigned voff_a, voff_a2 = 0, voff_b;
    {
        const int prow = lane >> 3, csrc = (lane & 7) ^ prow;
        voff_a = p.a_tiled ? (unsigned)((prow * 64 + csrc * 8) * 2) : (unsigned)(prow * (int)p.lda + csrc * 8) * 2u;
        if constexpr (TWOSRC) voff_a2 = (unsigned)(prow * (int)p.lda2 + csrc * 8) * 2u;
        voff_b = (unsigned)(prow * p.K + csrc * 8) * 2u;
    }
    bool second = false;
    constexpr unsigned kPad = 0xffffffffu;
    constexpr int NCV = MODE == MODE_DENSE ? 1 : 4;
    const __amdgpu_buffer_rsrc_t rsrc_a = __builtin_amdgcn_make_buffer_rsrc((void*)p.A, 0, (int)(MODE == MODE_DENSE ? 0u : p.a_bytes), 0x00020000);
    unsigned cv_off[NCV];
    unsigned cv_base[MODE == MODE_CONV2D ? 4 : 1], cv_flags = 0;
    int c_tap = 0, c_left = 0, c_chunk = 0;
    unsigned kb = 0;
    int tap_off = 0;
    unsigned tap_mask = 0;
    unsigned add_y = 0, add_x = 0;
    const int cpb = MODE == MODE_DENSE ? 1 : p.Cin / BK;
    auto udiv = [](unsigned m, unsigned d, float rcp, unsigned& rem) -> unsigned {
        unsigned q = (unsigned)((float)m * rcp);
        int r = (int)(m - q * d);
        if (r < 0) { --q; r += (int)d; }
        if (r >= (int)d) { ++q; r -= (int)d; }
        rem = (unsigned)r;
        return q;
    };
    const unsigned d_hw = MODE == MODE_CONV2D ? (unsigned)(p.Ho * p.Wo) : (unsigned)(MODE == MODE_TCONV ? p.HW : 1);
    const unsigned d_w = MODE == MODE_CONV2D ? (unsigned)p.Wo : (unsigned)(MODE == MODE_TCONV ? p.F : 1);
    const float r_hw = 1.0f / (float)d_hw, r_w = 1.0f / (float)d_w;
    auto conv_tile = [&]() {
        if constexpr (MODE == MODE_CONV2D) {
            int l = (int)__builtin_amdgcn_mbcnt_hi(~0u, __builtin_amdgcn_mbcnt_lo(~0u, 0u));
            asm volatile("" : "+v"(l));
            const unsigned lanechunk = (unsigned)(((l & 7) ^ (l >> 3)) * 16);
            cv_flags = 0;
#pragma unroll
            for (int i = 0; i < 4; ++i) {
                unsigned m = (unsigned)(c_m0 + wv * 32 + i * 8 + (l >> 3));
                m = m < (unsigned)p.M ? m : (unsigned)p.M - 1u;
                unsigned r, x;
                const unsigned n = udiv(m, d_hw, r_hw, r), y = udiv(r, d_w, r_w, x);
                unsigned f = 0;
                if constexpr (UPS) {
                    const int yu = (int)y - 1, xu = (int)x - 1;
                    const int y0 = yu >> 1, x0 = xu >> 1;
                    cv_base[i] = (unsigned)(((int)(n * (unsigned)p.Hi) + y0) * p.Wi + x0) * (unsigned)p.Cin * 2u + lanechunk;
#pragma unroll
                    for (int t = 0; t < 3; ++t) {
                        f |= (unsigned)(yu + t >= 0 && yu + t < 2 * p.Hi) << t;
                        f |= (unsigned)(xu + t >= 0 && xu + t < 2 * p.Wi) << (3 + t);
                    }
                    cv_flags |= ((y & 1u) << (24 + 2 * i)) | ((x & 1u) << (25 + 2 * i));
                } else {
                    const int y0 = (int)y * p.stride - p.pad, x0 = (int)x * p.stride - p.pad;
                    cv_base[i] = (unsigned)(((int)(n * (unsigned)p.Hi) + y0) * p.Wi + x0) * (unsigned)p.Cin * 2u + lanechunk;
#pragma unroll
                    for (int t = 0; t < 3; ++t) {
                        f |= (unsigned)(y0 + t >= 0 && y0 + t < p.Hi) << t;
                        f |= (unsigned)(x0 + t >= 0 && x0 + t < p.Wi) << (3 + t);
                    }
                }
                cv_flags |= f << (6 * i);
            }
        }
    };
    auto conv_tap = [&](int tap) {
        if constexpr (MODE == MODE_TCONV) {
            int l = (int)__builtin_amdgcn_mbcnt_hi(~0u, __builtin_amdgcn_mbcnt_lo(~0u, 0u));
            asm volatile("" : "+v"(l));
            const unsigned chunk = (unsigned)(((l & 7) ^ (l >> 3)) * 16);
#pragma unroll
            for (int i = 0; i < NCV; ++i) {
                unsigned m = (unsigned)(c_m0 + wv * 32 + i * 8 + (l >> 3));
                m = m < (unsigned)p.M ? m : (unsigned)p.M - 1u;
                unsigned r, f;
                const unsigned bf_ = udiv(m, d_hw, r_hw, r);
                (void)udiv(bf_, d_w, r_w, f);
                const int ff = (int)f + tap - 1;
                cv_off[i] = (ff >= 0 && ff < p.F) ? (unsigned)((int)m + (tap - 1) * p.HW) * (unsigned)p.Cin * 2u + chunk : kPad;
            }
        }
    };
    auto cursor_begin = [&]() {
        if (c_tl >= tiles.len) return;
        if (c_ks == 0) {
            int n0_, tn_;
            tile_origin(tiles.start + c_tl, c_m0, n0_, tn_);
            abase = (const char*)p.A;
            second = false;
            if constexpr (MODE != MODE_DENSE) { c_tap = 0; c_left = 0; c_chunk = 0; }
            conv_tile();
#pragma unroll
            for (int i = 0; i < 4; ++i) {
                int r = c_m0 + wv * 32 + i * 8;
                r = r < p.M - 8 ? r : p.M - 8;
                if (p.a_tiled) oa[i] = 2u * ((unsigned)(r >> 7) * (unsigned)(p.K >> 6) * 8192u + (unsigned)(r & 127) * 64u);
                else oa[i] = 2u * (unsigned)r * (unsigned)p.lda;
            }
#pragma unroll
            for (int j = 0; j < 5; ++j) {
                int n = n0_ + (wv * 5 + j) * 8;
                n = n < p.N - 8 ? n : p.N - 8;
                ob[j] = 2u * (unsigned)n * (unsigned)p.K;
            }
            if constexpr (MODE != MODE_DENSE) __builtin_amdgcn_s_waitcnt(0x0F70);
        } else if (TWOSRC && c_ks == kt_switch) {
            abase = (const char*)p.A2;
            second = true;
#pragma unroll
            for (int i = 0; i < 4; ++i) {
                int r = c_m0 + wv * 32 + i * 8;
                r = r < p.M - 8 ? r : p.M - 8;
                oa[i] = 2u * (unsigned)r * (unsigned)p.lda2;
            }
#pragma unroll
            for (int j = 0; j < 5; ++j) ob[j] += 2u * BK;
        } else if constexpr (MODE != MODE_CONV2D) {
#pragma unroll
            for (int i = 0; i < 4; ++i) oa[i] += a_step;
#pragma unroll
            for (int j = 0; j < 5; ++j) ob[j] += 2u * BK;
        }
        if constexpr (MODE == MODE_CONV2D) {
            const int ty = c_tap / 3, tx = c_tap - 3 * ty;
            if constexpr (UPS) {
                tap_off = (((ty == 2 ? p.Wi : 0) + (tx == 2 ? 1 : 0)) * p.Cin + c_chunk * BK) * 2;
                add_y = ty == 1 ? (unsigned)(p.Wi * p.Cin * 2) : 0u;
                add_x = tx == 1 ? (unsigned)(p.Cin * 2) : 0u;
            } else {
                tap_off = ((ty * p.Wi + tx) * p.Cin + c_chunk * BK) * 2;
            }
            tap_mask = (1u << ty) | (8u << tx);
            kb = (unsigned)(c_tap * p.Cin + c_chunk * BK) * 2u;
            if (++c_tap == 9) { c_tap = 0; ++c_chunk; }
        } else if constexpr (MODE == MODE_TCONV) {
            if (c_left == 0) { conv_tap(c_tap); ++c_tap; c_left = cpb; }
            else {
#pragma unroll
                for (int i = 0; i < NCV; ++i) cv_off[i] = cv_off[i] == kPad ? kPad : cv_off[i] + 2u * BK;
            }
            --c_left;
        }
        if (++c_ks == nkt) { c_ks = 0; c_tl += tiles.stride; }
    };
    auto cursor_end = [&]() { c_slot = c_slot ? 0u : (unsigned)Z_SLOT1; };
    auto piece = [&](auto IDX) {
        constexpr int idx = decltype(IDX)::value;
        char* st = smem_raw + c_slot;
        if constexpr (idx < 4 && MODE == MODE_CONV2D) {
            const unsigned mk = tap_mask << (6 * idx);
            const bool ok = (cv_flags & mk) == mk;
            unsigned o = cv_base[idx < 4 ? idx : 0] + (unsigned)tap_off;
            if constexpr (UPS) {
                o += (cv_flags & (1u << (24 + 2 * (idx & 3)))) ? 0u : add_y;
                o += (cv_flags & (2u << (24 + 2 * (idx & 3)))) ? 0u : add_x;
            }
            __builtin_amdgcn_raw_ptr_buffer_load_lds(rsrc_a, (lds_void_t*)(st + (wv * 4 + idx) * 1024), 16, (int)(ok ? o : kPad), 0, 0, 0);
        } else if constexpr (idx < 4 && MODE != MODE_DENSE) {
            __builtin_amdgcn_raw_ptr_buffer_load_lds(rsrc_a, (lds_void_t*)(st + (wv * 4 + idx) * 1024), 16, (int)cv_off[idx < NCV ? idx : 0], 0, 0, 0);
        } else if constexpr (idx < 4) {
            const unsigned va = (TWOSRC && second) ? voff_a2 : voff_a;
            __builtin_amdgcn_global_load_lds((gbl_void_t*)(abase + (size_t)(oa[idx] + va)), (lds_void_t*)(st + (wv * 4 + idx) * 1024), 16, 0, 0);
        } else {
            constexpr int j = idx - 4;
            __builtin_amdgcn_global_load_lds((gbl_void_t*)((const char*)p.W + (size_t)(ob[j] + (MODE == MODE_CONV2D ? kb : 0u) + voff_b)), (lds_void_t*)(st + W_A_BYTES + (wv * 5 + j) * 1024), 16, 0, 0);
        }
    };

    const unsigned lds0 = (unsigned)(size_t)(__attribute__((address_space(3))) char*)smem_raw;
    unsigned ra[2], rb[2];
    {
        const int fr = lane & 15, fq = lane >> 4;
        const unsigned a_row = (unsigned)((wm * WM + fr) * 128), b_row = (unsigned)(W_A_BYTES + (wn * 160 + fr) * 128);
#pragma unroll
        for (int kh = 0; kh < 2; ++kh) {
            const unsigned sw = (unsigned)(((kh * 4 + fq) ^ (fr & 7)) << 4);
            ra[kh] = lds0 + a_row + sw; rb[kh] = lds0 + b_row + sw;
        }
    }
    unsigned rslot = 0;
    auto flip_read_slot = [&]() {
        const unsigned d = rslot ? (unsigned)(-Z_SLOT1) : (unsigned)Z_SLOT1;
        ra[0] += d; ra[1] += d; rb[0] += d; rb[1] += d;
        rslot = rslot ? 0u : (unsigned)Z_SLOT1;
    };

#ifndef Z_LA
#define Z_LA 3
#endif
    constexpr int LA = Z_LA, RB = LA + 1;
    static_assert(20 % RB == 0 && LA >= 3 && LA <= 4, "ring of 4 or 5 weight fragments");
    float4v acc[2][TM][TN];
    constexpr int NAF = MODE == MODE_DENSE ? 2 : 1;
    half8 af[NAF][TM], bf[RB];

    cursor_begin();
    piece(std::integral_constant<int, 0>{}); piece(std::integral_constant<int, 1>{}); piece(std::integral_constant<int, 2>{});
    piece(std::integral_constant<int, 3>{}); piece(std::integral_constant<int, 4>{}); piece(std::integral_constant<int, 5>{});
    piece(std::integral_constant<int, 6>{}); piece(std::integral_constant<int, 7>{}); piece(std::integral_constant<int, 8>{});
    cursor_end();
    asm volatile("s_waitcnt vmcnt(0)" ::: "memory");
    __builtin_amdgcn_s_barrier();

    auto group_piece = [&](auto QC) {
        constexpr int q = decltype(QC)::value;
        constexpr int order[9] = {0, 4, 1, 5, 2, 6, 3, 7, 8};
        if constexpr (q < 9) piece(std::integral_constant<int, order[q < 9 ? q : 0]>{});
        if constexpr (q == 8) cursor_end();
    };
#define Z_YOUNGER(q) ((19 - (q) < LA ? 19 - (q) : LA) + ((NAF == 2 && (q) >= 7 && (q) < 7 + LA && (q) != 10) ? 4 : 0))
#define Z_NWAIT(q) (NAF == 1 ? ((q) == 10 ? 1 : ((q) == 0 ? 2 : Z_YOUNGER(q))) \
                             : ((q) == 10 ? (LA < 4 ? LA : ((10 + LA < 19 ? 10 + LA : 19) - (7 + LA) + 1)) : Z_YOUNGER(q)))
#define Z_GROUP(q) do { \
        group_piece(ZQ(q)); \
        if constexpr (NAF == 2 && (q) == 7) z_read_a<1, NAF>(af, ra); \
        if constexpr ((q) + LA <= 19) z_read_b<((q) + LA <= 19 ? (q) + LA : 0), RB>(bf, rb); \
        z_wait<(q), RB, Z_NWAIT(q), NAF>(af, bf); \
        z_mma<(q), RB, NAF>(acc, af, bf); \
        if constexpr (NAF == 1 && (q) == 9) z_read_a<1, NAF>(af, ra); } while (0)
#define ZQ(q) std::integral_constant<int, q>{}

#ifdef SYN3R_TIMING
    unsigned long long zt[8] = {0, 0, 0, 0, 0, 0, 0, 0}, z_a = __builtin_amdgcn_s_memtime();
#define ZSTAMP(i) { __builtin_amdgcn_sched_barrier(0); const unsigned long long t_ = __builtin_amdgcn_s_memtime(); zt[i] += t_ - z_a; z_a = t_; __builtin_amdgcn_sched_barrier(0); }
#else
#define ZSTAMP(i)
#endif
    for (unsigned tl = blockIdx.x / 8; tl < tiles.len; tl += tiles.stride) {
        int m0, n0, tile_n;
        tile_origin(tiles.start + tl, m0, n0, tile_n);
        if constexpr (MODE != MODE_DENSE) {
            if (c_ks == 1 && c_m0 == m0) {
                conv_tile();
                if constexpr (MODE == MODE_TCONV) conv_tap(0);
            }
        }
#pragma unroll
        for (int hh = 0; hh < 2; ++hh)
#pragma unroll
            for (int i = 0; i < TM; ++i)
#pragma unroll
                for (int j = 0; j < TN; ++j) acc[hh][i][j] = (float4v){0.f, 0.f, 0.f, 0.f};
#pragma unroll
        for (int i = 0; i < TM; ++i) { asm volatile("" : "=v"(af[0][i])); asm volatile("" : "=v"(af[NAF - 1][i])); }
#pragma unroll
        for (int j = 0; j < RB; ++j) asm volatile("" : "=v"(bf[j]));
        if constexpr (NAF == 1) {
            z_read_b<0, RB>(bf, rb); z_read_b<1, RB>(bf, rb);
            z_read_a<0, NAF>(af, ra);
            z_read_b<2, RB>(bf, rb);
        } else {
            z_read_a<0, NAF>(af, ra);
            z_read_b<0, RB>(bf, rb); z_read_b<1, RB>(bf, rb); z_read_b<2, RB>(bf, rb);
            if constexpr (LA >= 4) z_read_b<3, RB>(bf, rb);
        }
        asm volatile("" :: "v"(voff_a), "v"(voff_a2), "v"(voff_b), "v"(ra[0]), "v"(ra[1]), "v"(rb[0]), "v"(rb[1]));
        if constexpr (MODE == MODE_CONV2D) asm volatile("" :: "v"(cv_base[0]), "v"(cv_base[1]), "v"(cv_base[2]), "v"(cv_base[3]), "v"(cv_flags));
        if constexpr (MODE == MODE_TCONV) asm volatile("" :: "v"(cv_off[0]), "v"(cv_off[1]), "v"(cv_off[2]), "v"(cv_off[3]));
        for (int kt = 0; kt < nkt; ++kt) {
            ZSTAMP(5);
            cursor_begin();
            if constexpr (MODE == MODE_CONV2D) asm volatile("" :: "v"(cv_base[0]), "v"(cv_base[1]), "v"(cv_base[2]), "v"(cv_base[3]), "v"(cv_flags));
            if constexpr (MODE == MODE_TCONV) asm volatile("" :: "v"(cv_off[0]), "v"(cv_off[1]), "v"(cv_off[2]), "v"(cv_off[3]));
            Z_GROUP(0); Z_GROUP(1); Z_GROUP(2); Z_GROUP(3); Z_GROUP(4); Z_GROUP(5); Z_GROUP(6); Z_GROUP(7);
            Z_GROUP(8);
            ZSTAMP(0);
            Z_GROUP(9); Z_GROUP(10); Z_GROUP(11); Z_GROUP(12); Z_GROUP(13); Z_GROUP(14); Z_GROUP(15);
            Z_GROUP(16);
            ZSTAMP(1);
            asm volatile("s_waitcnt lgkmcnt(0)" : "+v"(bf[17 % RB]), "+v"(bf[18 % RB]), "+v"(bf[19 % RB]));
            z_mma<17, RB, NAF>(acc, af, bf);
            ZSTAMP(2);
            asm volatile("s_waitcnt vmcnt(0)" ::: "memory");
            ZSTAMP(3);
            __builtin_amdgcn_s_barrier();
            ZSTAMP(4);
            flip_read_slot();
#ifdef SYN3R_TIMING
            ++zt[7];
#endif
            if (kt + 1 < nkt) {
                if constexpr (NAF == 1) {
                    z_read_b<0, RB>(bf, rb);
                    z_mma<18, RB, NAF>(acc, af, bf);
                    z_read_b<1, RB>(bf, rb);
                    z_mma<19, RB, NAF>(acc, af, bf);
                    z_read_a<0, NAF>(af, ra);
                    z_read_b<2, RB>(bf, rb);
                } else {
                    z_read_a<0, NAF>(af, ra);
                    z_read_b<0, RB>(bf, rb);
                    z_mma<18, RB, NAF>(acc, af, bf);
                    z_read_b<1, RB>(bf, rb);
                    z_mma<19, RB, NAF>(acc, af, bf);
                    z_read_b<2, RB>(bf, rb);
                    if constexpr (LA == 4) z_read_b<3, RB>(bf, rb);
                }
            } else {
                z_mma<18, RB, NAF>(acc, af, bf);
                z_mma<19, RB, NAF>(acc, af, bf);
            }
        }
        ZSTAMP(5);
        int le = lane;
        asm volatile("" : "+v"(le));
        char* const epi = smem_raw + (rslot ? 0 : W_STAGE);
        const int gm0 = m0 + wm * WM;
        if (p.geglu_D > 0) {
            const int fq = le >> 4;
            const int gn = n0 + wn * 160;
#pragma unroll
            for (int j = 0; j < TN; ++j) {
                const int n = gn + j * 16 + fq * 4;
                float bh[4], bg[4];
#pragma unroll
                for (int r = 0; r < 4; ++r) {
                    bh[r] = (p.bias && n + r < p.N) ? __half2float(p.bias[n + r]) : 0.f;
                    bg[r] = (p.bias && n + 80 + r < p.N) ? __half2float(p.bias[n + 80 + r]) : 0.f;
                }
#pragma unroll
                for (int i = 0; i < TM; ++i)
#pragma unroll
                    for (int r = 0; r < 4; r += 2) {
                        const syn3r_f2 hv = (syn3r_f2){(float)(_Float16)(acc[0][i][j][r] + bh[r]), (float)(_Float16)(acc[0][i][j][r + 1] + bh[r + 1])};
                        const syn3r_f2 gv = (syn3r_f2){(float)(_Float16)(acc[1][i][j][r] + bg[r]), (float)(_Float16)(acc[1][i][j][r + 1] + bg[r + 1])};
                        const syn3r_f2 y = hv * gelu_pk(gv);
                        acc[0][i][j][r] = y.x; acc[0][i][j][r + 1] = y.y;
                    }
            }
            const int go0 = tile_n * 160 + wn * WN;
            const bool full = gm0 + WM <= p.M && go0 + WN <= p.geglu_D;
            widep_store(p, acc[0], epi, le, wv, gm0, go0, p.geglu_D, nullptr, nullptr, nullptr, full);
        } else {
            const int gn0 = n0 + wn * 160;
            const bool full = gm0 + WM <= p.M && gn0 + 160 <= p.N;
            widep_store(p, acc[0], epi, le, wv, gm0, gn0, p.N, p.bias, p.residual, p.aux, full);
            widep_store(p, acc[1], epi, le, wv, gm0, gn0 + WN, p.N, p.bias, p.residual, p.aux, full);
        }
        __builtin_amdgcn_s_barrier();
        ZSTAMP(6);
    }
#ifdef SYN3R_TIMING
    if (blockIdx.x == gridDim.x / 2 && lane == 0)
        for (int i = 0; i < 8; ++i) g_wide_timing[wv * 8 + i] = zt[i];
#endif
#undef ZSTAMP
#undef ZQ
#undef Z_GROUP
#undef Z_NWAIT
#undef Z_YOUNGER
}
```

syn3r_amd/csrc/unet.hip:

```cpp
#include "common.h"
#include <sys/mman.h>
#include <sys/stat.h>
#include <fcntl.h>
#include <unistd.h>
#include <math.h>
#include <string.h>
#include <ctype.h>
#include <exception>
#include <map>
#include <memory>
#include <algorithm>
#include <string>
#include <unordered_map>
#include <unordered_set>
#include <mutex>
#include <vector>

using namespace syn3r;

namespace {

typedef unsigned short u16;

__global__ void k_timestep_embedding(const float* __restrict__ t_dev, double t_host, float t_step, int n, int dim, __half* __restrict__ out) {
// ... 281 lines not shown
        const bool attn = dt[i] == "CrossAttnDownBlockSpatioTemporal";
        if (!attn && dt[i] != "DownBlockSpatioTemporal") return fail("unet_create: %s does not exist", dt[i]);
        BlockPlan bp{(int)i, attn, {}, i != n - 1, out_ch, m.heads[i]};
        for (int j = 0; j < m.layers[i]; ++j) bp.layers.emplace_back(j == 0 ? in_ch : out_ch, out_ch);
        m.down.push_back(bp);
    }
    std::vector<int> rev(m.boc.rbegin(), m.boc.rend()), rev_heads(m.heads.rbegin(), m.heads.rend()), rev_layers(m.layers.rbegin(), m.layers.rend());
    out_ch = rev[0];
    for (size_t i = 0; i < n; ++i) {
        const bool attn = ut[i] == "CrossAttnUpBlockSpatioTemporal";
        if (!attn && ut[i] != "UpBlockSpatioTemporal") return fail("unet_create: %s does not exist", ut[i]);
        const int prev_out = out_ch;
        out_ch = rev[i];
        const int in_ch = rev[std::min(i + 1, n - 1)];
        const int nl = rev_layers[i] + 1;
        BlockPlan bp{(int)i, attn, {}, i != n - 1, out_ch, rev_heads[i]};
        for (int j = 0; j < nl; ++j) {
            const int res_skip = j == nl - 1 ? in_ch : out_ch, res_in = j == 0 ? prev_out : out_ch;
            bp.layers.emplace_back(res_in + res_skip, out_ch);
        }
        m.up.push_back(bp);
    }
    return SYN3R_OK;
}

int pack_weights(syn3r_unet& m, const StFile& f, std::vector<HostPack>& packs) {
    std::string err;
    auto has_suffix = [](const std::string& s, const char* suf) { size_t n = strlen(suf); return s.size() >= n && !s.compare(s.size() - n, n, suf); };
    std::map<std::string, const StEntry*> names;
    for (auto& kv : f.entries) names[kv.first] = &kv.second;
    auto get = [&](const std::string& k, std::vector<u16>& out, std::vector<long long>* shape = nullptr) -> bool {
        auto it = f.entries.find(k);
        if (it == f.entries.end()) { err = "missing tensor " + k; return false; }
        if (shape) *shape = it->second.shape;
        return host_f16(f, it->second, out, err);
    };
    auto res_names = [&](const std::string& pre, std::vector<std::string>& out) {
        out.push_back(pre + ".spatial_res_block.time_emb_proj");
        out.push_back(pre + ".temporal_res_block.time_emb_proj");
    };
    for (auto& bp : m.down) for (size_t j = 0; j < bp.layers.size(); ++j) res_names("down_blocks." + std::to_string(bp.idx) + ".resnets." + std::to_string(j), m.temb_names);
    res_names("mid_block.resnets.0", m.temb_names);
    res_names("mid_block.resnets.1", m.temb_names);
    for (auto& bp : m.up) for (size_t j = 0; j < bp.layers.size(); ++j) res_names("up_blocks." + std::to_string(bp.idx) + ".resnets." + std::to_string(j), m.temb_names);

    for (auto& kv : names) {
        const std::string& k = kv.first;
        const StEntry& e = *kv.second;
        std::vector<u16> t;
        if (!host_f16(f, e, t, err)) return fail("unet_create: %s", k + ": " + err);
        const auto& s = e.shape;
        HostPack hp; hp.name = k;
        if (has_suffix(k, ".weight") && s.size() == 4 && s[3] == 3) {
            const long long O = s[0], I = s[1], IP = (I + 63) / 64 * 64, OP = (O + 7) / 8 * 8;
            hp.rows = OP; hp.cols = 9 * IP; hp.d.assign((size_t)(OP * 9 * IP), 0);
            for (long long o = 0; o < O; ++o) for (long long i = 0; i < I; ++i) for (int y = 0; y < 3; ++y) for (int x = 0; x < 3; ++x)
                hp.d[(size_t)(((o * 3 + y) * 3 + x) * IP + i)] = t[(size_t)(((o * I + i) * 3 + y) * 3 + x)];
        } else if (has_suffix(k, ".weight") && s.size() == 5) {
            const long long O = s[0], I = s[1];
            hp.rows = O; hp.cols = 3 * I; hp.d.resize((size_t)(O * 3 * I));
            for (long long o = 0; o < O; ++o) for (long long i = 0; i < I; ++i) for (int tt = 0; tt < 3; ++tt)
                hp.d[(size_t)((o * 3 + tt) * I + i)] = t[(size_t)((o * I + i) * 3 + tt)];
        } else if (has_suffix(k, "mix_factor")) {
            const float mf = f16_bits_to_f32(t[0]);
            const _Float16 a = (_Float16)(1.0f / (1.0f + expf(-mf)));
            const _Float16 om = (_Float16)((_Float16)1.0f - a);
            m.alpha[k] = {(double)(float)a, (double)(float)om};
            continue;
        } else {
            hp.rows = s.empty() ? 1 : s[0];
            long long n = 1;
            for (long long d : s) n *= d;
            hp.cols = hp.rows ? n / hp.rows : 0;
            hp.d = std::move(t);
        }
        packs.push_back(std::move(hp));
    }
    {
        std::vector<u16> b;
        if (!get("conv_out.bias", b)) return fail("unet_create: %s", err);
        b.resize((b.size() + 7) / 8 * 8, 0);
        for (auto& hp : packs) if (hp.name == "conv_out.bias") { hp.rows = (long long)b.size(); hp.cols = 1; hp.d = b; }
    }
    for (auto& kv : names) {
        const std::string& k = kv.first;
        if (has_suffix(k, "attn1.to_q.weight")) {
            const std::string pre = k.substr(0, k.size() - strlen("to_q.weight"));
            HostPack hp; hp.name = pre + "qkv";
            std::vector<long long> sh;
            for (const char* part : {"to_q.weight", "to_k.weight", "to_v.weight"}) {
                std::vector<u16> t;
                if (!get(pre + part, t, &sh)) return fail("unet_create: %s", err);
                hp.d.insert(hp.d.end(), t.begin(), t.end());
            }
            hp.cols = sh[1]; hp.rows = (long long)hp.d.size() / hp.cols;
            packs.push_back(std::move(hp));
        } else if (has_suffix(k, ".net.0.proj.weight")) {
            const std::string pre = k.substr(0, k.size() - strlen("weight"));
            std::vector<u16> wv, bv;
            std::vector<long long> sh;
            if (!get(k, wv, &sh) || !get(pre + "bias", bv)) return fail("unet_create: %s", err);
            const long long D2 = sh[0], K = sh[1], D = D2 / 2;
            HostPack pw, pb;
            if (K == 320) {
                if (D % 64) return fail("unet_create: %s: hidden width must be a multiple of 64", k);
                pw.name = pre + "geglu_cw"; pb.name = pre + "geglu_cb";
                pw.rows = 2 * D; pw.cols = K; pw.d.resize((size_t)(2 * D * K)); pb.rows = 2 * D; pb.cols = 1; pb.d.resize((size_t)(2 * D));
                long long r = 0;
                for (long long j = 0; j < D / 64; ++j) for (int q = 0; q < 64; q += 16) for (int half = 0; half < 2; ++half) for (int i = 0; i < 16; ++i, ++r) {
                    const long long src = (half ? D : 0) + 64 * j + q + i;
                    memcpy(&pw.d[(size_t)(r * K)], &wv[(size_t)(src * K)], (size_t)K * 2);
                    pb.d[(size_t)r] = bv[(size_t)src];
                }
            } else {
                const long long tiles = (D + 79) / 80;
                pw.name = pre + "geglu_w"; pb.name = pre + "geglu_b";
                pw.rows = tiles * 160; pw.cols = K; pw.d.assign((size_t)(tiles * 160 * K), 0); pb.rows = tiles * 160; pb.cols = 1; pb.d.assign((size_t)(tiles * 160), 0);
                for (long long t = 0; t < tiles; ++t) {
                    const long long n = std::min<long long>(80, D - 80 * t);
                    memcpy(&pw.d[(size_t)(160 * t * K)], &wv[(size_t)(80 * t * K)], (size_t)(n * K) * 2);
                    memcpy(&pw.d[(size_t)((160 * t + 80) * K)], &wv[(size_t)((D + 80 * t) * K)], (size_t)(n * K) * 2);
                    memcpy(&pb.d[(size_t)(160 * t)], &bv[(size_t)(80 * t)], (size_t)n * 2);
                    memcpy(&pb.d[(size_t)(160 * t + 80)], &bv[(size_t)(D + 80 * t)], (size_t)n * 2);
                }
            }
            packs.push_back(std::move(pw)); packs.push_back(std::move(pb));
            if (K != 320 && D % 128 == 0) {
                HostPack qw, qb;
                qw.name = pre + "geglu_w64"; qb.name = pre + "geglu_b64";
                qw.rows = 2 * D; qw.cols = K; qw.d.resize((size_t)(2 * D * K)); qb.rows = 2 * D; qb.cols = 1; qb.d.resize((size_t)(2 * D));
                for (long long j = 0; j < D / 64; ++j) {
                    memcpy(&qw.d[(size_t)(128 * j * K)], &wv[(size_t)(64 * j * K)], (size_t)(64 * K) * 2);
                    memcpy(&qw.d[(size_t)((128 * j + 64) * K)], &wv[(size_t)((D + 64 * j) * K)], (size_t)(64 * K) * 2);
                    memcpy(&qb.d[(size_t)(128 * j)], &bv[(size_t)(64 * j)], 64 * 2);
                    memcpy(&qb.d[(size_t)(128 * j + 64)], &bv[(size_t)(D + 64 * j)], 64 * 2);
                }
                packs.push_back(std::move(qw)); packs.push_back(std::move(qb));
            }
        }
    }
    {
        HostPack pw, pb; pw.name = "time_emb_proj.all.weight"; pb.name = "time_emb_proj.all.bias";
        int off = 0; long long K = 0;
        for (auto& nme : m.temb_names) {
            std::vector<u16> wv, bv;
            std::vector<long long> sh;
            if (!get(nme + ".weight", wv, &sh) || !get(nme + ".bias", bv)) return fail("unet_create: %s", err);
            K = sh[1];
            m.temb_slice[nme] = {off, off + (int)sh[0]};
            off += (int)sh[0];
            pw.d.insert(pw.d.end(), wv.begin(), wv.end());
            pb.d.insert(pb.d.end(), bv.begin(), bv.end());
        }
        pw.rows = off; pw.cols = K; pb.rows = off; pb.cols = 1;
        packs.push_back(std::move(pw)); packs.push_back(std::move(pb));
    }
    return SYN3R_OK;
}

}

namespace {
int unet_create_impl(const char* weights_dir, const char* variant, syn3r_unet** out);
}
extern "C" int syn3r_unet_create(const char* weights_dir, const char* variant, syn3r_unet** out) {
    SYN3R_REQUIRE(weights_dir && out, "unet_create: null argument");
    *out = nullptr;
    try {
        return unet_create_impl(weights_dir, variant, out);
    } catch (const std::exception& e) {
        set_error("unet_create: %s", e.what());
    } catch (...) {
        set_error("unet_create: unexpected exception");
    }
    *out = nullptr;
    return SYN3R_E_INVALID;
}
namespace {
int unet_create_impl(const char* weights_dir, const char* variant, syn3r_unet** out) {
    const std::string dir(weights_dir);
    std::string cfg_text;
    if (!read_file(dir + "/config.json", cfg_text)) return fail("unet_create: cannot read %s/config.json", dir);
    JParser jp{cfg_text.data(), cfg_text.data() + cfg_text.size()};
    JVal cfg = jp.value();
    if (!jp.ok || cfg.type != JVal::OBJ) return fail("unet_create: %s/config.json is not a JSON object", dir);
    std::unique_ptr<syn3r_unet> m(new syn3r_unet);
    int rc = build_plan(*m, cfg);
    if (rc) return rc;
    std::unique_ptr<StFile> fp;
    std::string err;
    auto absent = [](const std::string& e) { return e.compare(0, 11, "cannot open") == 0; };
    if (variant && *variant) {
        fp.reset(new StFile);
        if (!fp->open_(dir + "/diffusion_pytorch_model." + variant + ".safetensors", err)) {
            if (!absent(err)) return fail("unet_create: %s", err);
            fp.reset();
        }
    }
    if (!fp) {
        fp.reset(new StFile);
        if (!fp->open_(dir + "/diffusion_pytorch_model.safetensors", err)) {
            if (!absent(err)) return fail("unet_create: %s", err);
            return fail("unet_create: no safetensors weights under %s (diffusion_pytorch_model[.variant].safetensors)", dir);
        }
    }
    const StFile& f = *fp;
    std::vector<HostPack> packs;
    rc = pack_weights(*m, f, packs);
    if (rc) return rc;
    rc = check_hip(hipGetDevice(&m->device), "hipGetDevice");
    if (rc) return rc;
    size_t total = 0;
    for (auto& hp : packs) total += (hp.d.size() * 2 + 255) / 256 * 256;
    rc = check_hip(hipMalloc((void**)&m->blob, total ? total : 256), "hipMalloc(unet weights)");
    if (rc) return rc;
    m->blob_bytes = total;
    size_t off = 0;
    for (auto& hp : packs) {
        rc = check_hip(hipMemcpy(m->blob + off, hp.d.data(), hp.d.size() * 2, hipMemcpyHostToDevice), "hipMemcpy(unet weights)");
        if (rc) { (void)hipFree(m->blob); return rc; }
        m->w[hp.name] = Wt{(__half*)(m->blob + off), hp.rows, hp.cols};
        off += (hp.d.size() * 2 + 255) / 256 * 256;
    }
    m->ff_ln = tune_env("SYN3R_FF_LN", 1) != 0;
    m->ln_qkv = tune_env("SYN3R_LN_QKV", 1) != 0;
    *out = m.release();
    {
        std::lock_guard<std::mutex> lk(g_unet_mu);
        unet_registry().insert(*out);
    }
    return SYN3R_OK;
}
}

extern "C" int syn3r_unet_destroy(syn3r_unet* m) {
    if (!m) return SYN3R_OK;
    {
        std::lock_guard<std::mutex> lk(g_unet_mu);
        if (!unet_registry().erase(m)) { set_error("unet_destroy: not a live handle"); return SYN3R_E_INVALID; }
    }
    for (auto& kv : m->pos_cache) {
        if (kv.second.ready) (void)hipEventDestroy(kv.second.ready);
        (void)hipFree(kv.second.p);
    }
// ... 51 lines not shown

struct Run {
    syn3r_unet& m;
    Arena ar;
    bool dry = false;
    hipStream_t stream = nullptr;
    int B = 0, F = 0, h = 0, w = 0, G = 0;
    bool shared_ctx = false;
    T ehs, temb_all;
    std::unordered_map<std::string, T> cross;
    int rc = SYN3R_OK;
    explicit Run(syn3r_unet& m_) : m(m_) {}

    const Wt* W(const std::string& k) {
        auto it = m.w.find(k);
        if (it == m.w.end()) { if (!rc) { set_error("unet_forward: the checkpoint has no tensor %s", k.c_str()); rc = SYN3R_E_INVALID; } return nullptr; }
        return &it->second;
    }
    const __half* Wp(const std::string& k) { const Wt* t = W(k); return t ? t->p : nullptr; }
    bool ok() const { return rc == SYN3R_OK; }
    T make(long long rows, int cols) {
        T t; t.rows = rows; t.cols = cols;
        if (!ok()) return t;
        t.p = (__half*)ar.alloc((size_t)rows * cols * 2);
        if (!t.p) { set_error("unet_forward: workspace too small (needs syn3r_unet_workspace_bytes)"); rc = SYN3R_E_WORKSPACE; }
        return t;
    }
    void drop(T& t) { ar.release(t.p); t.p = nullptr; ar.release(t.gnp); t.gnp = nullptr; t.gn_ok = 0; }
    size_t gn_begin(T& out, bool want) {
        static const int gn_env = tune_env("SYN3R_GN_EPILOGUE", 1);
        const size_t nb = (want && gn_env != 0 && out.rows <= SYN3R_DIM_MAX) ? syn3r_gn_partials_bytes((int)out.rows, out.cols) : 0;
        if (!nb || !ok()) return 0;
        out.gnp = (float*)ar.alloc(nb);
        if (!out.gnp) { set_error("unet_forward: workspace too small (needs syn3r_unet_workspace_bytes)"); rc = SYN3R_E_WORKSPACE; return 0; }
        return nb;
    }
    void chk(int r) { if (r && !rc) rc = r; }
    bool go() const { return ok() && !dry; }

    T linear(const T& x, long long ldx, int K, const std::string& wname, const char* bias_name, const Epi& e = Epi(), bool gn = false) {
        const Wt* wt = W(wname);
        const __half* b = bias_name ? Wp(bias_name) : nullptr;
        T out = make(x.rows, wt ? (int)wt->rows : 0);
        const size_t gnb = gn_begin(out, gn);
        if (go())
            chk(syn3r_gemm_f16(x.p, ldx, wt->p, out.p, out.cols, b, e.rowvec, e.ldrv, e.rows_per_vec, e.rv_group,
                               e.residual ? e.residual->p : nullptr, e.residual ? e.residual->cols : 0, e.aux ? e.aux->p : nullptr,
                               e.aux ? e.aux->cols : 0, e.s_acc, e.s_res, e.s_aux, (int)x.rows, out.cols, K, out.gnp, gnb, &out.gn_ok, stream));
        return out;
    }
    T linear(const T& x, const std::string& wname, const std::string& bname, const Epi& e = Epi(), bool gn = false) {
        return linear(x, x.cols, x.cols, wname, bname.empty() ? nullptr : bname.c_str(), e, gn);
    }
    T linear_cat(const T& x1, const T& x2, const std::string& wname, const std::string& bname) {
        const Wt* wt = W(wname);
        const int N = wt ? (int)wt->rows : 0;
        if (ok() && syn3r_gemm_2src_supported((int)x1.rows, N, x1.cols, x2.cols, x1.cols, x2.cols)) {
            T out = make(x1.rows, N);
            if (go()) chk(syn3r_gemm_2src_f16(x1.p, x1.cols, x1.cols, x2.p, x2.cols, x2.cols, wt->p, out.p, N, Wp(bname), (int)x1.rows, N, nullptr, 0, nullptr, stream));
            return out;
        }
        T cat = make(x1.rows, x1.cols + x2.cols);
        if (go()) {
            const long long n = cat.rows * cat.cols;
            hipLaunchKernelGGL(k_cat_cols, dim3((unsigned)((n + 255) / 256)), dim3(256), 0, stream, x1.p, x1.cols, x2.p, x2.cols, cat.p, cat.rows);
        }
        T out = linear(cat, wname, bname);
        drop(cat);
        return out;
    }
    T conv3x3(const T& x, int NB, int Hi, int Wi, int Cin, const std::string& wname, const std::string& bname, int stride, bool ups,
              const Epi& e, int* Ho_ = nullptr, int* Wo_ = nullptr, bool gn = true) {
        const Wt* wt = W(wname);
        const int Cout = wt ? (int)wt->rows : 0;
        const int Hg = ups ? 2 * Hi : Hi, Wg = ups ? 2 * Wi : Wi;
        const int Ho = (Hg + 1 - 2) / stride + 1, Wo = (Wg + 1 - 2) / stride + 1;
        if (Ho_) *Ho_ = Ho;
        if (Wo_) *Wo_ = Wo;
        T out = make((long long)NB * Ho * Wo, Cout);
        const size_t gnb = gn_begin(out, gn);
        if (go())
            chk(syn3r_conv2d3x3_f16(x.p, wt->p, out.p, Cout, Wp(bname), e.rowvec, e.ldrv, e.rows_per_vec, e.residual ? e.residual->p : nullptr,
                                    e.residual ? Cout : 0, e.s_acc, e.s_res, NB, Hi, Wi, Cin, Cout, stride, ups ? 1 : 0, 1, out.gnp, gnb, &out.gn_ok, stream));
        return out;
    }
    T tconv3(const T& x, const std::string& wname, const std::string& bname, int HW, const Epi& e) {
        const Wt* wt = W(wname);
        const int Cout = wt ? (int)wt->rows : 0;
        T out = make(x.rows, Cout);
        const size_t gnb = gn_begin(out, true);
        if (go())
            chk(syn3r_tconv3_f16(x.p, wt->p, out.p, Cout, Wp(bname), e.rowvec, e.ldrv, e.rows_per_vec, e.residual ? e.residual->p : nullptr,
                                 e.residual ? Cout : 0, e.s_acc, e.s_res, B, F, HW, x.cols, Cout, out.gnp, gnb, &out.gn_ok, stream));
        return out;
    }
    T groupnorm(const T& x, const std::string& pre, int samples, float eps, bool silu, const T* x2 = nullptr) {
        const int rows = (int)(x.rows / samples);
        const size_t wsb = syn3r_groupnorm_workspace_bytes(samples, rows);
        T out = make(x.rows, x.cols + (x2 ? x2->cols : 0));
        void* ws = ok() ? ar.alloc(wsb) : nullptr;
        if (ok() && !ws) { set_error("unet_forward: workspace too small (needs syn3r_unet_workspace_bytes)"); rc = SYN3R_E_WORKSPACE; }
        const int Ct = x.cols + (x2 ? x2->cols : 0);
        if (go() && x.gn_ok && (!x2 || x2->gn_ok) && rows % 32 == 0 && Ct % 320 == 0 && x.cols % 10 == 0) {
            chk(syn3r_groupnorm_pre_f16(x.p, x.cols, x.gnp, x2 ? x2->p : nullptr, x2 ? x2->cols : 0, x2 ? x2->gnp : nullptr, out.p, samples, rows,
                                        Wp(pre + ".weight"), Wp(pre + ".bias"), eps, silu, ws, wsb, stream));
        } else if (go()) {
            if (x2) chk(syn3r_groupnorm_2src_f16(x.p, x.cols, x2->p, x2->cols, out.p, samples, rows, Wp(pre + ".weight"), Wp(pre + ".bias"), eps, silu, ws, wsb, stream));
            else chk(syn3r_groupnorm_f16(x.p, out.p, samples, rows, x.cols, Wp(pre + ".weight"), Wp(pre + ".bias"), eps, silu, ws, wsb, stream));
        }
        ar.release(ws);
        return out;
    }
    T layernorm(const T& x, const std::string& pre, const __half* addvec = nullptr, int rows_per_vec = 0, T* xsum = nullptr) {
        T out = make(x.rows, x.cols);
        if (xsum) *xsum = make(x.rows, x.cols);
        if (go())
            chk(syn3r_layernorm_f16(x.p, out.p, xsum ? xsum->p : nullptr, addvec, rows_per_vec, x.rows, x.cols, Wp(pre + ".weight"), Wp(pre + ".bias"), 1e-5f, stream));
        return out;
    }
    T norm_qkv(const std::string& blk, const T& x) {
        const Wt* wq = W(blk + ".attn1.qkv");
        if (m.ln_qkv && x.cols == 320 && wq && wq->rows % 320 == 0) {
            T out = make(x.rows, (int)wq->rows);
            if (go())
                chk(syn3r_layernorm_linear320_f16(x.p, x.cols, Wp(blk + ".norm1.weight"), Wp(blk + ".norm1.bias"), 1e-5f, wq->p, out.p, out.cols,
                                                  (int)x.rows, (int)wq->rows, x.cols, stream));
            return out;
        }
        T n1 = layernorm(x, blk + ".norm1");
        T qkv = linear(n1, blk + ".attn1.qkv", "");
        drop(n1);
        return qkv;
    }
    T attention(const T& qkv, int nseq, int S, int heads) {
        const int C = heads * 64;
        T out = make(qkv.rows, C);
        if (go()) chk(syn3r_attention_f16(qkv.p, qkv.p + C, qkv.p + 2 * C, 3 * C, out.p, C, nseq, S, heads, stream));
        return out;
    }
    T attention_temporal(const T& qkv, int HW, int heads) {
        const int C = heads * 64;
        T out = make(qkv.rows, C);
        if (go()) chk(syn3r_attention_temporal_f16(qkv.p, qkv.p + C, qkv.p + 2 * C, 3 * C, out.p, C, B, F, HW, heads, stream));
        return out;
    }
    T ff(const std::string& pre, const T& x_in, const std::string& norm, const Epi& e) {
        const Wt* w0 = W(pre + ".net.0.proj.weight");
        const int D = w0 ? (int)(w0->rows / 2) : 0;
        const std::string w2 = pre + ".net.2.weight", b2 = pre + ".net.2.bias";
        T x = x_in;
        bool own = false;
        T out;
        if (m.w.count(pre + ".net.0.proj.geglu_cw")) {
            const bool fuse_ln = !norm.empty() && m.ff_ln;
            if (!norm.empty() && !fuse_ln) { x = layernorm(x_in, norm); own = true; }
            out = make(x.rows, x.cols);
            if (go()) {
                const void *r = e.residual ? e.residual->p : nullptr, *a = e.aux ? e.aux->p : nullptr;
                const long long ldr = e.residual ? e.residual->cols : 0, lda = e.aux ? e.aux->cols : 0;
                if (fuse_ln)
                    chk(syn3r_feedforward_fused_ln_f16(x.p, x.cols, Wp(norm + ".weight"), Wp(norm + ".bias"), 1e-5f, Wp(pre + ".net.0.proj.geglu_cw"),
                                                       Wp(pre + ".net.0.proj.geglu_cb"), D, Wp(w2), Wp(b2), out.p, out.cols, r, ldr, a, lda,
                                                       e.s_acc, e.s_res, e.s_aux, (int)x.rows, x.cols, stream));
                else
                    chk(syn3r_feedforward_fused_f16(x.p, x.cols, Wp(pre + ".net.0.proj.geglu_cw"), Wp(pre + ".net.0.proj.geglu_cb"), D, Wp(w2), Wp(b2),
                                                    out.p, out.cols, r, ldr, a, lda, e.s_acc, e.s_res, e.s_aux, (int)x.rows, x.cols, stream));
// ... 189 lines not shown
                splitk = ok() ? ar.alloc(bytes) : nullptr;
                if (ok() && !splitk) { set_error("unet_forward: workspace too small (needs syn3r_unet_workspace_bytes)"); rc = SYN3R_E_WORKSPACE; }
                if (go()) chk(syn3r_gemm_set_splitk_workspace(splitk, bytes));
            }
        }
        forward_body(sample, timestep, ehs_in, ehs_rows, added_ids, out);
        if (splitk) {
            if (!dry) syn3r_gemm_set_splitk_workspace(nullptr, 0);
            ar.release(splitk);
        }
    }
    void forward_body(const __half* sample, double timestep, const __half* ehs_in, int ehs_rows, const float* added_ids, __half* out) {
        const int c0 = m.boc[0];
        T te = make(B, c0);
        if (go()) hipLaunchKernelGGL(k_timestep_embedding, dim3((unsigned)((B * (c0 / 2) + 255) / 256)), dim3(256), 0, stream, (const float*)nullptr, timestep, 0.0f, B, c0, te.p);
        T e1 = linear(te, "time_embedding.linear_1.weight", "time_embedding.linear_1.bias");
        drop(te);
        T e1s = silu(e1);
        drop(e1);
        T emb = linear(e1s, "time_embedding.linear_2.weight", "time_embedding.linear_2.bias");
        drop(e1s);
        const int nid = m.proj_in / m.add_dim;
        T ta = make((long long)B * nid, m.add_dim);
        if (go()) hipLaunchKernelGGL(k_timestep_embedding, dim3((unsigned)((B * nid * (m.add_dim / 2) + 255) / 256)), dim3(256), 0, stream, added_ids, 0.0, 0.0f, B * nid, m.add_dim, ta.p);
        T ta2 = ta; ta2.rows = B; ta2.cols = nid * m.add_dim;
        T a1 = linear(ta2, "add_embedding.linear_1.weight", "add_embedding.linear_1.bias");
        drop(ta);
        T a1s = silu(a1);
        drop(a1);
        T aug = linear(a1s, "add_embedding.linear_2.weight", "add_embedding.linear_2.bias");
        drop(a1s);
        T es = make(emb.rows, emb.cols);
        if (go()) { const long long n = es.rows * es.cols; hipLaunchKernelGGL(k_add, dim3((unsigned)((n + 255) / 256)), dim3(256), 0, stream, emb.p, aug.p, es.p, n); }
        drop(emb);
        drop(aug);
        T act = silu(es);
        drop(es);
        temb_all = linear(act, "time_emb_proj.all.weight", "time_emb_proj.all.bias");
        drop(act);
        ehs.p = (__half*)ehs_in; ehs.rows = ehs_rows; ehs.cols = m.cross[0];
        const int CP = (m.in_ch + 63) / 64 * 64;
        T xin = make((long long)B * F * h * w, CP);
        if (go()) { const long long n = xin.rows * CP; hipLaunchKernelGGL(k_nchw_to_nhwc, dim3((unsigned)((n + 255) / 256)), dim3(256), 0, stream, sample, xin.p, B * F, m.in_ch, h * w, CP); }
        T x = conv3x3(xin, B * F, h, w, CP, "conv_in.weight", "conv_in.bias", 1, false, Epi());
        drop(xin);
        std::vector<T> skips{x};
        for (auto& bp : m.down) {
            const std::string bpre = "down_blocks." + std::to_string(bp.idx);
            for (size_t j = 0; j < bp.layers.size(); ++j) {
                T y = resblock(bpre + ".resnets." + std::to_string(j), x, bp.layers[j].first, bp.layers[j].second, nullptr);
                if (bp.attn) { T z = transformer(bpre + ".attentions." + std::to_string(j), y, bp.layers[j].second, bp.heads); drop(y); y = z; }
                x = y;
                skips.push_back(x);
            }
            if (bp.resample) {
                int Ho, Wo;
                T y = conv3x3(x, B * F, h, w, bp.ch, bpre + ".downsamplers.0.conv.weight", bpre + ".downsamplers.0.conv.bias", 2, false, Epi(), &Ho, &Wo);
                h = Ho; w = Wo;
                x = y;
                skips.push_back(x);
            }
        }
        {
            const int mid = m.boc.back();
            T y = resblock("mid_block.resnets.0", x, mid, mid, nullptr);
            T z = transformer("mid_block.attentions.0", y, mid, m.heads.back());
            drop(y);
            x = resblock("mid_block.resnets.1", z, mid, mid, nullptr);
            drop(z);
        }
        for (auto& bp : m.up) {
            const std::string bpre = "up_blocks." + std::to_string(bp.idx);
            for (size_t j = 0; j < bp.layers.size(); ++j) {
                T sk = skips.back();
                skips.pop_back();
                T y = resblock(bpre + ".resnets." + std::to_string(j), x, bp.layers[j].first, bp.layers[j].second, &sk);
                drop(x);
                drop(sk);
                if (bp.attn) { T z = transformer(bpre + ".attentions." + std::to_string(j), y, bp.layers[j].second, bp.heads); drop(y); y = z; }
                x = y;
            }
            if (bp.resample) {
                int Ho, Wo;
                T y = conv3x3(x, B * F, h, w, bp.ch, bpre + ".upsamplers.0.conv.weight", bpre + ".upsamplers.0.conv.bias", 1, true, Epi(), &Ho, &Wo);
                drop(x);
                h = Ho; w = Wo;
                x = y;
            }
        }
        T gn = groupnorm(x, "conv_norm_out", B * F, 1e-5f, true);
        drop(x);
        T y = conv3x3(gn, B * F, h, w, c0, "conv_out.weight", "conv_out.bias", 1, false, Epi(), nullptr, nullptr, false);
        drop(gn);
        if (go()) { const long long n = (long long)B * F * m.out_ch * h * w; hipLaunchKernelGGL(k_nhwc_to_nchw, dim3((unsigned)((n + 255) / 256)), dim3(256), 0, stream, y.p, out, B * F, m.out_ch, h * w, y.cols); }
        drop(y);
        for (auto& kv : cross) drop(kv.second);
        cross.clear();
        drop(temb_all);
    }
};

int check_shape(const syn3r_unet* m, int B, int F, int h, int w, int ehs_rows, int ctx_group) {
    SYN3R_REQUIRE(unet_live(m), "unet: not a live handle (syn3r_unet_create)");
    SYN3R_REQUIRE(B > 0 && B <= 64 && F > 0 && F <= 32 && SYN3R_SIDE_OK(h) && SYN3R_SIDE_OK(w), "unet: bad sizes B=%d F=%d h=%d w=%d (F <= 32)", B, F, h, w);
    SYN3R_REQUIRE((long long)B * F * h * w <= SYN3R_DIM_MAX, "unet: B*F*h*w = %lld rows is beyond the operators' limit", (long long)B * F * h * w);
    const int down = 1 << (m->boc.size() - 1);
    SYN3R_REQUIRE(h % down == 0 && w % down == 0, "unet: h and w must be multiples of %d", down);
    SYN3R_REQUIRE(ehs_rows == 1 || ehs_rows == B, "unet: encoder_hidden_states must have 1 (shared) or B rows, got %d", ehs_rows);
    SYN3R_REQUIRE(ctx_group >= 0 && (ctx_group == 0 || B % ctx_group == 0), "unet: ctx_group=%d must divide the batch size %d", ctx_group, B);
    return SYN3R_OK;
}

}

extern "C" size_t syn3r_unet_workspace_bytes(syn3r_unet* m, int B, int F, int h, int w, int ehs_rows) {
    if (check_shape(m, B, F, h, w, ehs_rows, 0)) return 0;
    try {
    Run r(*m);
    r.dry = true;
    r.ar.reset((char*)4096, (size_t)1 << 46);
    r.B = B; r.F = F; r.h = h; r.w = w; r.G = 1;
    r.shared_ctx = B == 1 || ehs_rows == 1;
    r.forward(nullptr, 0.0, (const __half*)4096, r.shared_ctx ? 1 : B, nullptr, nullptr);
    return r.ok() ? r.ar.peak + 256 : 0;
    } catch (...) { set_error("unet_workspace_bytes: unexpected exception"); return 0; }
}

extern "C" int syn3r_unet_forward(syn3r_unet* m, const void* sample, double timestep, const void* encoder_hidden_states, int ehs_rows,
                                  const float* added_time_ids, void* out, int B, int F, int h, int w, int ctx_group, void* workspace,
                                  size_t workspace_bytes, void* stream) {
    int rc = check_shape(m, B, F, h, w, ehs_rows, ctx_group);
    if (rc) return rc;
    SYN3R_REQUIRE(sample && encoder_hidden_states && added_time_ids && out, "unet_forward: null tensor");
    SYN3R_REQUIRE(workspace && ((uintptr_t)workspace % 256) == 0, "unet_forward: workspace must be non-null and 256-byte aligned");
    SYN3R_REQUIRE((((uintptr_t)sample | (uintptr_t)encoder_hidden_states | (uintptr_t)out) % 16) == 0, "unet_forward: misaligned tensor");
    try {
    Run r(*m);
    r.ar.reset((char*)workspace, workspace_bytes / 256 * 256);
    r.stream = (hipStream_t)stream;
    r.B = B; r.F = F; r.h = h; r.w = w;
    r.G = ctx_group > 0 ? ctx_group : B;
    r.shared_ctx = B == 1 || ehs_rows == 1;
    r.forward((const __half*)sample, timestep, (const __half*)encoder_hidden_states, r.shared_ctx ? 1 : B, added_time_ids, (__half*)out);
    if (r.ok()) {
        hipError_t e = hipGetLastError();
        if (e != hipSuccess) return check_hip(e, "unet_forward launch");
    }
    return r.rc;
    } catch (const std::exception& e) { set_error("unet_forward: %s", e.what()); return SYN3R_E_INVALID;
    } catch (...) { set_error("unet_forward: unexpected exception"); return SYN3R_E_INVALID; }
}
```

syn3r_amd/unet/model.py:

```python
from __future__ import annotations

import math
from typing import Dict, Optional, Sequence, Tuple, Union

import torch
import torch.nn.functional as Fn

from .. import _lib as L
from ..tuning import FLAGS as TUNE
from . import ops

H = torch.float16


def timestep_embedding(t: torch.Tensor, dim: int) -> torch.Tensor:
    half = dim // 2
    exponent = -math.log(10000) * torch.arange(half, dtype=torch.float32, device=t.device) / half
    emb = t[:, None].float() * torch.exp(exponent)[None, :]
    return torch.cat([torch.cos(emb), torch.sin(emb)], dim=-1)


class _Params:

    def __init__(self):
# ... 150 lines not shown
            layers = []
            for j in range(nl):
                res_skip = in_ch if j == nl - 1 else out_ch
                res_in = prev_out if j == 0 else out_ch
                self._declare_resblock(f"up_blocks.{i}.resnets.{j}", res_in + res_skip, out_ch, temb)
                if has_attn:
                    self._declare_transformer(f"up_blocks.{i}.attentions.{j}", out_ch, rev_cross[i])
                layers.append((res_in + res_skip, out_ch))
            up = i != len(boc) - 1
            if up:
                p.declare(f"up_blocks.{i}.upsamplers.0.conv.weight", out_ch, out_ch, 3, 3)
                p.declare(f"up_blocks.{i}.upsamplers.0.conv.bias", out_ch)
            self.up_plan.append(dict(idx=i, attn=has_attn, layers=layers, up=up, ch=out_ch, heads=rev_heads[i]))
        p.norm("conv_norm_out", boc[0])
        p.declare("conv_out.weight", c["out_channels"], boc[0], 3, 3); p.declare("conv_out.bias", c["out_channels"])

    def parameter_shapes(self) -> Dict[str, Tuple[int, ...]]:
        return dict(self.p.shapes)

    def num_parameters(self) -> int:
        return sum(math.prod(s) for s in self.p.shapes.values())

    def load_state_dict(self, sd: Dict[str, torch.Tensor], device) -> "UNetSpatioTemporalConditionModel":
        missing = [k for k in self.p.shapes if k not in sd]
        extra = [k for k in sd if k not in self.p.shapes]
        if missing or extra:
            raise KeyError(f"state_dict mismatch: missing {missing[:5]} (+{max(0, len(missing) - 5)}), "
                           f"unexpected {extra[:5]} (+{max(0, len(extra) - 5)})")
        dev = torch.device(device)
        for k, shape in self.p.shapes.items():
            t = sd[k]
            if tuple(t.shape) != shape:
                raise ValueError(f"{k}: shape {tuple(t.shape)} != {shape}")
            self.p.t[k] = t.detach().to(device=dev, dtype=H)
        self.device = dev
        self._pack()
        return self

    def init_random(self, device, seed: int = 0, std: float = 0.02) -> "UNetSpatioTemporalConditionModel":
        dev = torch.device(device)
        g = torch.Generator(device=dev).manual_seed(seed)
        sd = {}
        for k, shape in self.p.shapes.items():
            if k.endswith("mix_factor"):
                sd[k] = torch.full(shape, 0.5, device=dev)
            elif ".norm" in k and k.endswith(".weight") or k == "conv_norm_out.weight":
                sd[k] = torch.ones(shape, device=dev)
            elif k.endswith(".bias"):
                sd[k] = torch.zeros(shape, device=dev)
            else:
                fan_in = math.prod(shape[1:])
                sd[k] = torch.randn(shape, generator=g, device=dev, dtype=torch.float32) * min(std, fan_in ** -0.5)
        return self.load_state_dict(sd, dev)

    @classmethod
    def from_pretrained(cls, directory: str, device, variant: Optional[str] = "fp16", **kw):
        import json
        from pathlib import Path
        from safetensors.torch import load_file
        d = Path(directory)
        cfg = json.loads((d / "config.json").read_text())
        keys = ("sample_size in_channels out_channels down_block_types up_block_types block_out_channels "
                "addition_time_embed_dim projection_class_embeddings_input_dim layers_per_block cross_attention_dim "
                "transformer_layers_per_block num_attention_heads num_frames").split()
        model = cls(**{k: cfg[k] for k in keys if k in cfg})
        names = ([f"diffusion_pytorch_model.{variant}.safetensors"] if variant else []) + ["diffusion_pytorch_model.safetensors"]
        for name in names:
            if (d / name).exists():
                return model.load_state_dict(load_file(str(d / name)), device)
        raise FileNotFoundError(f"no safetensors weights under {d} (looked for {names})")

    def _pack(self):
        self._pos_cache = {}
        self._ctx_store = {}
        p, pk = self.p, {}
        for k, t in p.t.items():
            if k.endswith(".weight") and t.dim() == 4 and t.shape[-1] == 3:
                w = t
                if w.shape[1] % 64:
                    w = Fn.pad(w, (0, 0, 0, 0, 0, 64 - w.shape[1] % 64))
                if w.shape[0] % 8:
                    w = Fn.pad(w, (0, 0, 0, 0, 0, 0, 0, 8 - w.shape[0] % 8))
                pk[k] = w.permute(0, 2, 3, 1).contiguous()
            elif k.endswith(".weight") and t.dim() == 5:
                pk[k] = t[..., 0, 0].permute(0, 2, 1).contiguous()
            elif k.endswith("conv_shortcut.weight"):
                pk[k] = t.reshape(t.shape[0], t.shape[1]).contiguous()
        if p.t["conv_out.bias"].shape[0] % 8:
            pk["conv_out.bias"] = Fn.pad(p.t["conv_out.bias"], (0, 8 - p.t["conv_out.bias"].shape[0] % 8))
        for k in list(p.t):
            if k.endswith("attn1.to_q.weight"):
                pre = k[: -len("to_q.weight")]
                pk[pre + "qkv"] = torch.cat([p.t[pre + "to_q.weight"], p.t[pre + "to_k.weight"],
                                             p.t[pre + "to_v.weight"]], 0).contiguous()
        for k in list(p.t):
            if k.endswith(".net.0.proj.weight"):
                pre = k[: -len("weight")]
                if p.t[k].shape[1] == ops.FUSED_FF_CHANNELS and TUNE["ff_fused"]:
                    wp, bp, D = ops.pack_geglu_chunked(p.t[k], p.t[pre + "bias"])
                    pk[pre + "geglu_cw"], pk[pre + "geglu_cb"] = wp, bp
                else:
                    wp, bp, D = ops.pack_geglu(p.t[k], p.t[pre + "bias"])
                    pk[pre + "geglu_w"], pk[pre + "geglu_b"] = wp, bp
                    if TUNE["ff_g256"] and D % 128 == 0:
                        pk[pre + "geglu_w64"], pk[pre + "geglu_b64"], _ = ops.pack_geglu64(p.t[k], p.t[pre + "bias"])
        names = [k[: -len(".weight")] for k in p.t if k.endswith("time_emb_proj.weight")]
        self._temb_slices, off = {}, 0
        for nme in names:
            n_out = p.t[nme + ".weight"].shape[0]
            self._temb_slices[nme] = (off, off + n_out)
            off += n_out
        if names:
            pk["time_emb_proj.all.weight"] = torch.cat([p.t[nme + ".weight"] for nme in names], 0).contiguous()
            pk["time_emb_proj.all.bias"] = torch.cat([p.t[nme + ".bias"] for nme in names], 0).contiguous()
        self.packed = pk
        self.alpha = {}
        for k, t in p.t.items():
            if k.endswith("mix_factor"):
                a = torch.sigmoid(t.float()).to(H)
                self.alpha[k] = (float(a), float((1.0 - a).to(H)))

    def _context_cache(self, ehs: torch.Tensor, shared: bool) -> dict:
        key = (ehs.untyped_storage().data_ptr(), ehs.storage_offset(), tuple(ehs.shape), tuple(ehs.stride()), ehs._version, shared)
        store = self.__dict__.setdefault("_ctx_store", {})
        ent = store.get(key)
        if ent is None:
            if len(store) >= 8:
                store.pop(next(iter(store)))
            ent = store[key] = (ehs, {})
        return ent[1]

    def invalidate_context_cache(self) -> None:
        self.__dict__.setdefault("_ctx_store", {}).clear()
        self.__dict__.setdefault("_graphs", {}).clear()

    def w(self, name: str) -> torch.Tensor:
        return self.packed.get(name, self.p.t.get(name))

    def _blend_scales(self, name: str):
        return self.alpha[name]

    def _resblock(self, pre: str, x: torch.Tensor, st: dict, cin: int, cout: int, x2: Optional[torch.Tensor] = None) -> torch.Tensor:
        B, F, h, w_ = st["B"], st["F"], st["h"], st["w"]
        HW = h * w_
        s, t = pre + ".spatial_res_block", pre + ".temporal_res_block"
        W = self.w
        a0, a1 = self._temb_slices[s + ".time_emb_proj"]
        tp_s = st["temb_all"][:, a0:a1]
        hcur = ops.groupnorm(x, W(s + ".norm1.weight"), W(s + ".norm1.bias"), B * F, 1e-5, True, x2=x2)
        hcur = ops.conv3x3(hcur.view(B * F, h, w_, cin), W(s + ".conv1.weight"), W(s + ".conv1.bias"),
                           rowvec=tp_s, rows_per_vec=F * HW, gn_stats=TUNE["gn_epilogue"])
        hcur = ops.keep_gn(hcur.view(-1, cout), hcur)
        hcur = ops.groupnorm(hcur, W(s + ".norm2.weight"), W(s + ".norm2.bias"), B * F, 1e-5, True)
        skip = x
        if x2 is not None:
            skip = ops.linear_cat(x, x2, W(s + ".conv_shortcut.weight"), W(s + ".conv_shortcut.bias"))
        elif cin != cout:
            skip = ops.linear(x, W(s + ".conv_shortcut.weight"), W(s + ".conv_shortcut.bias"))
        xs = ops.conv3x3(hcur.view(B * F, h, w_, cout), W(s + ".conv2.weight"), W(s + ".conv2.bias"),
                         residual=skip, gn_stats=TUNE["gn_epilogue"])
        xs = ops.keep_gn(xs.view(-1, cout), xs)
        a0, a1 = self._temb_slices[t + ".time_emb_proj"]
        tp_t = st["temb_all"][:, a0:a1]
        hcur = ops.groupnorm(xs, W(t + ".norm1.weight"), W(t + ".norm1.bias"), B, 1e-5, True)
        hcur = ops.tconv3(hcur, W(t + ".conv1.weight"), W(t + ".conv1.bias"), B, F, HW, rowvec=tp_t, rows_per_vec=F * HW, gn_stats=TUNE["gn_epilogue"])
        hcur = ops.groupnorm(hcur, W(t + ".norm2.weight"), W(t + ".norm2.bias"), B, 1e-5, True)
# ... 84 lines not shown
                added_time_ids: torch.Tensor, return_dict: bool = False, ctx_group: Optional[int] = None):
        if self.device is None:
            raise L.Syn3rError("UNet weights are not loaded (load_state_dict / from_pretrained / init_random)")
        dev = L.require_gpu(sample, encoder_hidden_states, added_time_ids)
        c = self.config
        B, F, Cin, h, w_ = sample.shape
        if Cin != c["in_channels"]:
            raise ValueError(f"sample has {Cin} channels, the model expects {c['in_channels']}")
        if F > 32:
            raise NotImplementedError("temporal attention kernel supports up to 32 frames")
        W = self.w
        boc = c["block_out_channels"]
        down = 2 ** (len(boc) - 1)
        m_low = B * F * (h // down) * (w_ // down)
        splitk = None
        if TUNE["splitk"] and ((m_low + 255) // 256) * ((boc[-1] + 159) // 160) * 2 <= 256:
            nbytes = 4 * m_low * boc[-1] * 4
            splitk = L.workspace(dev, nbytes, "splitk")
            L.check(L.load().syn3r_gemm_set_splitk_workspace(L.ptr(splitk), nbytes), "syn3r_gemm_set_splitk_workspace")
        try:
            return self._forward(sample, timestep, encoder_hidden_states, added_time_ids, return_dict, ctx_group)
        finally:
            if splitk is not None:
                L.load().syn3r_gemm_set_splitk_workspace(None, 0)

    def _forward(self, sample, timestep, encoder_hidden_states, added_time_ids, return_dict, ctx_group):
        dev = L.require_gpu(sample, encoder_hidden_states, added_time_ids)
        c = self.config
        B, F, Cin, h, w_ = sample.shape
        W = self.w
        boc = c["block_out_channels"]
        ts = timestep if torch.is_tensor(timestep) else torch.tensor([timestep], dtype=torch.float64)
        ts = ts.reshape(-1).to(dev).expand(B)
        t_emb = timestep_embedding(ts, boc[0]).to(H)
        emb = ops.linear(t_emb, W("time_embedding.linear_1.weight"), W("time_embedding.linear_1.bias"))
        emb = ops.linear(Fn.silu(emb), W("time_embedding.linear_2.weight"), W("time_embedding.linear_2.bias"))
        te = timestep_embedding(added_time_ids.flatten().to(dev), c["addition_time_embed_dim"]).reshape(B, -1).to(H)
        aug = ops.linear(te, W("add_embedding.linear_1.weight"), W("add_embedding.linear_1.bias"))
        aug = ops.linear(Fn.silu(aug), W("add_embedding.linear_2.weight"), W("add_embedding.linear_2.bias"))
        emb = emb + aug
        shared_ctx = B == 1 or encoder_hidden_states.stride(0) == 0
        ctx = encoder_hidden_states[:1] if shared_ctx else encoder_hidden_states
        G = B if ctx_group is None else int(ctx_group)
        if G < 1 or B % G:
            raise ValueError(f"ctx_group={ctx_group} must divide the batch size {B}")
        st = dict(B=B, F=F, h=h, w=w_, temb_act=Fn.silu(emb).contiguous(), shared_ctx=shared_ctx, ctx_group=G,
                  ehs=ctx.reshape(ctx.shape[0], -1).to(H).contiguous(), ctx_cache=self._context_cache(encoder_hidden_states, shared_ctx))
        st["temb_all"] = ops.linear(st["temb_act"], W("time_emb_proj.all.weight"), W("time_emb_proj.all.bias"))
        x = sample.to(H).flatten(0, 1).permute(0, 2, 3, 1)
        x = Fn.pad(x, (0, 64 - Cin % 64 if Cin % 64 else 0)).contiguous()
        x = ops.conv3x3(x, W("conv_in.weight"), W("conv_in.bias"), gn_stats=TUNE["gn_epilogue"])
        x = ops.keep_gn(x.view(-1, boc[0]), x)
        skips = [(x, boc[0])]
        for blk in self.down_plan:
            i = blk["idx"]
            for j, (cin, cout) in enumerate(blk["layers"]):
                x = self._resblock(f"down_blocks.{i}.resnets.{j}", x, st, cin, cout)
                if blk["attn"]:
                    x = self._transformer(f"down_blocks.{i}.attentions.{j}", x, st, cout, blk["heads"])
                skips.append((x, cout))
            if blk["down"]:
                ch = blk["ch"]
                x = ops.conv3x3(x.view(B * F, st["h"], st["w"], ch), W(f"down_blocks.{i}.downsamplers.0.conv.weight"),
                                W(f"down_blocks.{i}.downsamplers.0.conv.bias"), stride=2, gn_stats=TUNE["gn_epilogue"])
                st["h"], st["w"] = x.shape[1], x.shape[2]
                x = ops.keep_gn(x.view(-1, ch), x)
                skips.append((x, ch))
        mid = boc[-1]
        x = self._resblock("mid_block.resnets.0", x, st, mid, mid)
        x = self._transformer("mid_block.attentions.0", x, st, mid, c["num_attention_heads"][-1])
        x = self._resblock("mid_block.resnets.1", x, st, mid, mid)
        for blk in self.up_plan:
            i = blk["idx"]
            for j, (cin, cout) in enumerate(blk["layers"]):
                sk, sk_ch = skips.pop()
                if TUNE["unet_cat"]:
                    x = self._resblock(f"up_blocks.{i}.resnets.{j}", torch.cat([x, sk], dim=1), st, cin, cout)
                else:
                    x = self._resblock(f"up_blocks.{i}.resnets.{j}", x, st, cin, cout, x2=sk)
                if blk["attn"]:
                    x = self._transformer(f"up_blocks.{i}.attentions.{j}", x, st, cout, blk["heads"])
            if blk["up"]:
                ch = blk["ch"]
                x = ops.conv3x3(x.view(B * F, st["h"], st["w"], ch), W(f"up_blocks.{i}.upsamplers.0.conv.weight"),
                                W(f"up_blocks.{i}.upsamplers.0.conv.bias"), upsample=True, gn_stats=TUNE["gn_epilogue"])
                st["h"], st["w"] = x.shape[1], x.shape[2]
                x = ops.keep_gn(x.view(-1, ch), x)
        x = ops.groupnorm(x, W("conv_norm_out.weight"), W("conv_norm_out.bias"), B * F, 1e-5, True)
        y = ops.conv3x3(x.view(B * F, st["h"], st["w"], boc[0]), W("conv_out.weight"), W("conv_out.bias"))
        y = y[..., : c["out_channels"]].permute(0, 3, 1, 2).reshape(B, F, c["out_channels"], st["h"], st["w"]).contiguous()
        if return_dict:
            from types import SimpleNamespace
            return SimpleNamespace(sample=y)
        return (y,)

    def forward_graphed(self, sample: torch.Tensor, timestep, encoder_hidden_states: torch.Tensor, added_time_ids: torch.Tensor,
                        ctx_group: Optional[int] = None):
        if L._active_trace is not None:
            return self.forward(sample, timestep, encoder_hidden_states, added_time_ids, ctx_group=ctx_group)
        dev = L.require_gpu(sample, encoder_hidden_states, added_time_ids)
        ehs = encoder_hidden_states
        ts = timestep if torch.is_tensor(timestep) else torch.tensor([timestep], dtype=torch.float64)
        ts = ts.reshape(-1)[:1].to(dev)
        key = (tuple(sample.shape), ctx_group, ehs.untyped_storage().data_ptr(), ehs.storage_offset(), tuple(ehs.shape),
               tuple(ehs.stride()), ehs._version, tuple(added_time_ids.shape), ts.dtype)
        graphs = self.__dict__.setdefault("_graphs", {})
        ent = graphs.get(key)
        if ent is None:
            if len(graphs) >= 8:
                graphs.pop(next(iter(graphs)))
            s_in, t_in, a_in = sample.to(H).clone(), ts.clone(), added_time_ids.clone()
            side = torch.cuda.Stream(device=dev)
            side.wait_stream(torch.cuda.current_stream(dev))
            with torch.cuda.stream(side):
                for _ in range(2):
                    self.forward(s_in, t_in, ehs, a_in, ctx_group=ctx_group)
            torch.cuda.current_stream(dev).wait_stream(side)
            g = torch.cuda.CUDAGraph()
            with torch.cuda.graph(g, stream=side):
                y = self.forward(s_in, t_in, ehs, a_in, ctx_group=ctx_group)[0]
            shared_ctx = sample.shape[0] == 1 or ehs.stride(0) == 0
            pinned = (self._context_cache(ehs, shared_ctx),
                      [buf for (di, st_, _tag), buf in L._ws_cache.items() if di == dev.index and st_ == side.cuda_stream], side)
            ent = graphs[key] = (g, s_in, t_in, a_in, y, ehs, pinned)
        g, s_in, t_in, a_in, y = ent[:5]
        s_in.copy_(sample)
        t_in.copy_(ts)
        a_in.copy_(added_time_ids)
        g.replay()
        return (y.clone(),)

    __call__ = forward
```

syn3r_amd/unet/ops.py:

```python
from __future__ import annotations

import ctypes
from typing import Optional

import torch

from .. import _lib as L

H = torch.float16

FLOPS = {"enabled": False, "gemm": 0.0, "attn": 0.0}


def _count(kind: str, flops: float) -> None:
    if FLOPS["enabled"]:
        FLOPS[kind] += flops


def _chk(*ts):
    dev = L.require_gpu(*[t for t in ts if t is not None])
    for t in ts:
        if t is not None and (t.dtype != H or not t.is_contiguous()):
            raise L.Syn3rError(f"UNet operators need contiguous fp16 tensors, got {t.dtype} contiguous={t.is_contiguous()}")
    return dev
# ... 119 lines not shown


def pack_geglu_chunked(weight: torch.Tensor, bias: torch.Tensor):
    D2, K = weight.shape
    D = D2 // 2
    if D % 64:
        raise ValueError("pack_geglu_chunked: hidden width must be a multiple of 64")
    idx = []
    for j in range(D // 64):
        for q in (0, 16, 32, 48):
            idx.extend(range(64 * j + q, 64 * j + q + 16))
            idx.extend(range(D + 64 * j + q, D + 64 * j + q + 16))
    idx = torch.tensor(idx, device=weight.device)
    return weight.index_select(0, idx).contiguous(), bias.index_select(0, idx).contiguous(), D


FUSED_FF_CHANNELS = 320


def feedforward_fused(x: torch.Tensor, w1_chunked: torch.Tensor, b1_chunked: torch.Tensor, D: int, w2: torch.Tensor,
                      b2: Optional[torch.Tensor] = None, *, residual: Optional[torch.Tensor] = None,
                      aux: Optional[torch.Tensor] = None, s_acc: float = 1.0, s_res: float = 1.0, s_aux: float = 1.0,
                      ln: Optional[tuple] = None, addvec: Optional[tuple] = None) -> torch.Tensor:
    dev = _chk(w1_chunked, b1_chunked, w2, b2, residual, aux)
    L.require_gpu(x)
    M, K = x.shape
    N = w2.shape[0]
    if x.stride(1) != 1 or K != N or w2.shape[1] != D or tuple(w1_chunked.shape) != (2 * D, K):
        raise ValueError(f"feedforward_fused: x {tuple(x.shape)} / w1 {tuple(w1_chunked.shape)} / w2 {tuple(w2.shape)} / D={D} mismatch")
    out = torch.empty((M, N), dtype=H, device=dev)
    tail = (L.ptr(w1_chunked), L.ptr(b1_chunked), D, L.ptr(w2), L.ptr(b2), L.ptr(out), N,
            residual.data_ptr() if residual is not None else None, residual.stride(0) if residual is not None else 0,
            aux.data_ptr() if aux is not None else None, aux.stride(0) if aux is not None else 0,
            float(s_acc), float(s_res), float(s_aux), M, K, L.stream_ptr(dev))
    if addvec is not None and (ln is None or residual is not None):
        raise ValueError("feedforward_fused: addvec needs ln and takes the place of the residual")
    if ln is not None:
        gamma, beta, eps = ln
        _chk(gamma, beta)
        if gamma.numel() != K or beta.numel() != K:
            raise ValueError(f"feedforward_fused: LayerNorm parameters of {gamma.numel()} / {beta.numel()} channels for C = {K}")
    if addvec is not None:
        vec, rpv = addvec
        _chk(vec)
        if vec.dim() != 2 or vec.shape[1] != K or not vec.is_contiguous() or rpv <= 0 or (M + rpv - 1) // rpv > vec.shape[0]:
            raise ValueError(f"feedforward_fused: add vector {tuple(vec.shape)} / rows_per_vec={rpv} for x {tuple(x.shape)}")
        rc = L.load().syn3r_feedforward_fused_addln_f16(x.data_ptr(), x.stride(0), L.ptr(vec), int(rpv), L.ptr(gamma), L.ptr(beta), float(eps),
                                                        *tail[:7], *tail[9:])
        L.check(rc, "syn3r_feedforward_fused_addln_f16")
    elif ln is not None:
        rc = L.load().syn3r_feedforward_fused_ln_f16(x.data_ptr(), x.stride(0), L.ptr(gamma), L.ptr(beta), float(eps), *tail)
        L.check(rc, "syn3r_feedforward_fused_ln_f16")
    else:
        rc = L.load().syn3r_feedforward_fused_f16(x.data_ptr(), x.stride(0), *tail)
        L.check(rc, "syn3r_feedforward_fused_f16")
    _count("gemm", 2.0 * M * 2 * D * K + 2.0 * M * N * D)
    return out


def conv3x3(x: torch.Tensor, weight: torch.Tensor, bias: Optional[torch.Tensor] = None, *, stride: int = 1,
            upsample: bool = False, rowvec: Optional[torch.Tensor] = None, rows_per_vec: int = 0,
            residual: Optional[torch.Tensor] = None, s_acc: float = 1.0, s_res: float = 1.0,
            pad_lo: int = 1, gn_stats: bool = False) -> torch.Tensor:
    dev = _chk(x, weight, bias, residual)
    rv_ptr, rv_ld = _rowvec(rowvec)
    NB, Hi, Wi, Cin = x.shape
    Cout = weight.shape[0]
    if tuple(weight.shape[1:]) != (3, 3, Cin):
        raise ValueError(f"conv3x3: weight {tuple(weight.shape)} does not match Cin={Cin}")
    Hg, Wg = (2 * Hi, 2 * Wi) if upsample else (Hi, Wi)
    Ho, Wo = (Hg + pad_lo - 2) // stride + 1, (Wg + pad_lo - 2) // stride + 1
    out = torch.empty((NB, Ho, Wo, Cout), dtype=H, device=dev)
    lib = L.load()
    part, gn = _gn_request(dev, NB * Ho * Wo, Cout, gn_stats)
    rc = lib.syn3r_conv2d3x3_f16(L.ptr(x), L.ptr(weight), L.ptr(out), Cout, L.ptr(bias), rv_ptr, rv_ld, int(rows_per_vec),
                                 L.ptr(residual), Cout if residual is not None else 0, float(s_acc), float(s_res),
                                 NB, Hi, Wi, Cin, Cout, int(stride), 1 if upsample else 0, int(pad_lo), *gn,
                                 L.stream_ptr(dev))
    L.check(rc, "syn3r_conv2d3x3_f16")
    _count("gemm", 2.0 * NB * Ho * Wo * Cout * 9 * Cin)
    return _gn_collect(out, part, gn[2])


def tconv3(x: torch.Tensor, weight: torch.Tensor, bias: Optional[torch.Tensor], B: int, F: int, HW: int, *,
           rowvec: Optional[torch.Tensor] = None, rows_per_vec: int = 0, residual: Optional[torch.Tensor] = None,
           s_acc: float = 1.0, s_res: float = 1.0, gn_stats: bool = False) -> torch.Tensor:
    dev = _chk(x, weight, bias, residual)
    rv_ptr, rv_ld = _rowvec(rowvec)
    M, Cin = x.shape
    Cout = weight.shape[0]
    if M != B * F * HW or tuple(weight.shape[1:]) != (3, Cin):
        raise ValueError("tconv3: shape mismatch")
    out = torch.empty((M, Cout), dtype=H, device=dev)
    lib = L.load()
    part, gn = _gn_request(dev, M, Cout, gn_stats)
    rc = lib.syn3r_tconv3_f16(L.ptr(x), L.ptr(weight), L.ptr(out), Cout, L.ptr(bias), rv_ptr, rv_ld, int(rows_per_vec), L.ptr(residual),
                              Cout if residual is not None else 0, float(s_acc), float(s_res), B, F, HW, Cin, Cout, *gn,
                              L.stream_ptr(dev))
    L.check(rc, "syn3r_tconv3_f16")
    _count("gemm", 2.0 * M * Cout * 3 * Cin)
    return _gn_collect(out, part, gn[2])


def attention(qkv: torch.Tensor, nseq: int, S: int, heads: int) -> torch.Tensor:
    dev = _chk(qkv)
    C = heads * 64
    if qkv.shape != (nseq * S, 3 * C):
        raise ValueError(f"attention: qkv {tuple(qkv.shape)} != {(nseq * S, 3 * C)}")
    out = torch.empty((nseq * S, C), dtype=H, device=dev)
    base = qkv.data_ptr()
    lib = L.load()
    rc = lib.syn3r_attention_f16(base, base + 2 * C, base + 4 * C, 3 * C, L.ptr(out), C, nseq, S, heads,
                                 L.stream_ptr(dev))
    L.check(rc, "syn3r_attention_f16")
    _count("attn", 4.0 * nseq * heads * S * S * 64)
    return out


def attention_temporal(qkv: torch.Tensor, B: int, F: int, HW: int, heads: int) -> torch.Tensor:
    dev = _chk(qkv)
    C = heads * 64
    if qkv.shape != (B * F * HW, 3 * C):
        raise ValueError(f"attention_temporal: qkv {tuple(qkv.shape)} != {(B * F * HW, 3 * C)}")
    out = torch.empty((B * F * HW, C), dtype=H, device=dev)
    base = qkv.data_ptr()
    lib = L.load()
    rc = lib.syn3r_attention_temporal_f16(base, base + 2 * C, base + 4 * C, 3 * C, L.ptr(out), C, B, F, HW, heads,
                                          L.stream_ptr(dev))
    L.check(rc, "syn3r_attention_temporal_f16")
    _count("attn", 4.0 * B * HW * heads * F * F * 64)
    return out


def groupnorm(x: torch.Tensor, gamma: torch.Tensor, beta: torch.Tensor, samples: int, eps: float, silu: bool,
              x2: Optional[torch.Tensor] = None, use_partials: bool = True) -> torch.Tensor:
    dev = _chk(x, gamma, beta, x2)
    M, C = x.shape
    if M % samples:
        raise ValueError("groupnorm: rows not divisible by samples")
    lib = L.load()
    ws = L.workspace(dev, lib.syn3r_groupnorm_workspace_bytes(samples, M // samples), "gn")
    p1 = getattr(x, "gn_part", None) if use_partials else None
    p2 = getattr(x2, "gn_part", None) if (use_partials and x2 is not None) else None
    Ct = C + (x2.shape[1] if x2 is not None else 0)
    if p1 is not None and (x2 is None or p2 is not None) and (M // samples) % 32 == 0 and Ct % 320 == 0 and C % 10 == 0:
        if x2 is not None and x2.shape[0] != M:
            raise ValueError("groupnorm: the two sources must have the same rows")
        y = torch.empty((M, Ct), dtype=H, device=dev)
        rc = lib.syn3r_groupnorm_pre_f16(L.ptr(x), C, L.ptr(p1), L.ptr(x2), Ct - C, L.ptr(p2), L.ptr(y), samples, M // samples,
                                         L.ptr(gamma), L.ptr(beta), float(eps), 1 if silu else 0, L.ptr(ws), ws.numel(), L.stream_ptr(dev))
        L.check(rc, "syn3r_groupnorm_pre_f16")
        return y
    if x2 is not None:
        if x2.shape[0] != M:
            raise ValueError("groupnorm: the two sources must have the same rows")
        C2 = x2.shape[1]
        y = torch.empty((M, C + C2), dtype=H, device=dev)
        rc = lib.syn3r_groupnorm_2src_f16(L.ptr(x), C, L.ptr(x2), C2, L.ptr(y), samples, M // samples, L.ptr(gamma), L.ptr(beta),
                                          float(eps), 1 if silu else 0, L.ptr(ws), ws.numel(), L.stream_ptr(dev))
        L.check(rc, "syn3r_groupnorm_2src_f16")
        return y
    y = torch.empty_like(x)
    rc = lib.syn3r_groupnorm_f16(L.ptr(x), L.ptr(y), samples, M // samples, C, L.ptr(gamma), L.ptr(beta), float(eps),
                                 1 if silu else 0, L.ptr(ws), ws.numel(), L.stream_ptr(dev))
    L.check(rc, "syn3r_groupnorm_f16")
    return y
# ... 88 lines not shown
```

Baseline: 411.8 iters/s.

## Replace nearest-upsample+3x3 conv with four-phase 2x2 subpixel convolution

Upsampler convolutions in the SVD UNet now use a phase-decomposed form. Nearest-2x upsampling followed by a 3x3 conv is algebraically folded into four 2x2 kernels, one per output phase, with the weights pre-summed at pack time. A new UP4 variant of the z-GEMM kernel iterates the four phases, gathers from the un-upsampled input, scatters rows to interleaved output positions, and remaps the GroupNorm partial slots. This cuts the reduction length from 9*Cin to 4*Cin per output pixel, reducing UNet FLOPs, but the summed weights are rounded to fp16 and the scattered stores are less regular.

```diff
diff --git a/include/syn3r_hip.h b/include/syn3r_hip.h
--- a/include/syn3r_hip.h
+++ b/include/syn3r_hip.h
@@ -225,6 +225,10 @@
                         float s_acc, float s_res, int NB, int Hi, int Wi, int Cin, int Cout, int stride, int upsample,
                         int pad_lo, void* gn_partials, size_t gn_partials_bytes, int* gn_written, void* stream);
 
+int syn3r_pack_upsample4_f16(const void* w, void* w4, int Cout, int Cin);
+int syn3r_conv2d3x3_up4_f16(const void* X, const void* w4, void* out, const void* bias, const void* residual, int NB, int Hi, int Wi,
+                            int Cin, int Cout, void* gn_partials, size_t gn_partials_bytes, int* gn_written, void* stream);
+
 int syn3r_tconv3_f16(const void* X, const void* W, void* out, long long ldc, const void* bias, const void* rowvec,
                      long long ldrv, int rows_per_vec, const void* residual, long long ldr, float s_acc, float s_res,
                      int B, int F, int HW, int Cin, int Cout, void* gn_partials, size_t gn_partials_bytes, int* gn_written,
diff --git a/syn3r_amd/_lib.py b/syn3r_amd/_lib.py
--- a/syn3r_amd/_lib.py
+++ b/syn3r_amd/_lib.py
@@ -94,6 +94,8 @@
     "syn3r_layernorm_linear320_f16": (c_i, [c_p, c_ll, c_p, c_p, c_f, c_p, c_p, c_ll, c_i, c_i, c_i, c_p]),
     "syn3r_conv2d3x3_f16": (c_i, [c_p, c_p, c_p, c_ll, c_p, c_p, c_ll, c_i, c_p, c_ll, c_f, c_f,
                                   c_i, c_i, c_i, c_i, c_i, c_i, c_i, c_i, c_p, c_sz, C.POINTER(c_i), c_p]),
+    "syn3r_pack_upsample4_f16": (c_i, [c_p, c_p, c_i, c_i]),
+    "syn3r_conv2d3x3_up4_f16": (c_i, [c_p, c_p, c_p, c_p, c_p, c_i, c_i, c_i, c_i, c_i, c_p, c_sz, C.POINTER(c_i), c_p]),
     "syn3r_tconv3_f16": (c_i, [c_p, c_p, c_p, c_ll, c_p, c_p, c_ll, c_i, c_p, c_ll, c_f, c_f,
                                c_i, c_i, c_i, c_i, c_i, c_p, c_sz, C.POINTER(c_i), c_p]),
     "syn3r_attention_f16": (c_i, [c_p, c_p, c_p, c_ll, c_p, c_ll, c_i, c_i, c_i, c_p]),
diff --git a/syn3r_amd/csrc/gemm.hip b/syn3r_amd/csrc/gemm.hip
--- a/syn3r_amd/csrc/gemm.hip
+++ b/syn3r_amd/csrc/gemm.hip
@@ -107,6 +107,14 @@
         if (p.ups) return launch_tiles<k_gemm_z<false, MODE_CONV2D, true>>("gemm_z", Z_LDS, blocks, 512, stream, q, gn_written, "k_gemm_z<%d>", MODE);
     }
     return launch_tiles<k_gemm_z<false, MODE>>("gemm_z", Z_LDS, blocks, 512, stream, q, gn_written, "k_gemm_z<%d>", MODE);
+}
+
+int launch_z_up4(const GemmParams& p, hipStream_t stream, int* gn_written) {
+    const long long blocks = std::min<long long>(4 * wide_tiles(p), persistent_blocks());
+    GemmParams q = p;
+    q.band = band_width(p);
+    q.a_bytes = (unsigned)((long long)p.M * p.Cin * 2);
+    return launch_tiles<k_gemm_z<false, MODE_CONV2D, false, true>>("gemm_z", Z_LDS, blocks, 512, stream, q, gn_written, "k_gemm_z<%d>/up4", MODE_CONV2D);
 }
 
 thread_local int g_dma_bm = 0;
@@ -552,6 +560,32 @@
     return launch_dma<MODE_CONV2D>(p, (hipStream_t)stream, gn_written);
 }
 
+extern "C" int syn3r_conv2d3x3_up4_f16(const void* X, const void* W4, void* out, const void* bias, const void* residual, int NB, int Hi,
+                                       int Wi, int Cin, int Cout, void* gn_partials, size_t gn_partials_bytes, int* gn_written,
+                                       void* stream) {
+    if (gn_written) *gn_written = 0;
+    SYN3R_REQUIRE(X && W4 && out, "conv2d3x3_up4: null operand");
+    SYN3R_REQUIRE(!residual, "conv2d3x3_up4: the phase form takes no residual (use syn3r_conv2d3x3_f16 with upsample = 1)");
+    SYN3R_REQUIRE(SYN3R_DIM_OK(NB) && SYN3R_SIDE_OK(Hi) && SYN3R_SIDE_OK(Wi) && SYN3R_DIM_OK(Cin) && SYN3R_DIM_OK(Cout), "conv2d3x3_up4: bad sizes");
+    SYN3R_REQUIRE(Cin % BK == 0, "conv2d3x3_up4: Cin=%d must be a multiple of %d (a k-tile is %d channels of one tap)", Cin, BK, BK);
+    SYN3R_REQUIRE(Cout % 8 == 0, "conv2d3x3_up4: Cout=%d must be a multiple of 8", Cout);
+    const long long M4 = (long long)NB * Hi * Wi;
+    SYN3R_REQUIRE(M4 < (1ll << 24), "conv2d3x3_up4: %lld input pixels (the phase form takes fewer than 2^24)", M4);
+    SYN3R_REQUIRE(M4 * Cin * 2 < (1ll << 32) - (1 << 20) && (long long)Cout * 4 * Cin < (1ll << 29), "conv2d3x3_up4: operand too large");
+    SYN3R_REQUIRE(((uintptr_t)X | (uintptr_t)W4 | (uintptr_t)out | (uintptr_t)bias) % 16 == 0, "conv2d3x3_up4: operands must be 16-byte aligned");
+    SYN3R_REQUIRE((gn_partials == nullptr) == (gn_partials_bytes == 0), "conv2d3x3_up4: gn_partials pointer and size must both be given or both be zero");
+    SYN3R_REQUIRE(((uintptr_t)gn_partials % 16) == 0, "conv2d3x3_up4: the gn_partials buffer must be 16-byte aligned");
+    GemmParams p{};
+    p.A = (const __half*)X; p.W = (const __half*)W4; p.out = (__half*)out; p.ldc = Cout; p.bias = (const __half*)bias;
+    p.s_acc = 1.0f; p.s_res = 0.f; p.s_aux = 0.f;
+    p.Hi = Hi; p.Wi = Wi; p.Cin = Cin; p.stride = 1; p.ups = 0; p.pad = 1; p.Ho = Hi; p.Wo = Wi;
+    p.M = (int)M4; p.N = Cout; p.K = 4 * Cin;
+    if (gn_partials && ((long long)Hi * Wi) % 32 == 0 && Cout % 80 == 0 && gn_partials_bytes >= ::gn_partials_bytes(4 * M4, Cout)) {
+        p.gn_part = (float*)gn_partials; p.gn_units = Cout / 10; p.up4_bpi = Hi * Wi / 32;
+    }
+    return launch_z_up4(p, (hipStream_t)stream, gn_written);
+}
+
 extern "C" int syn3r_conv2d3x3_act_f16(const void* X, const void* W, void* out, const void* bias, int relu, const void* relu_mask,
                                        int NB, int Hi, int Wi, int Cin, int Cout, void* stream) {
     SYN3R_REQUIRE(NB > 0 && Hi > 0 && Wi > 0 && Cin > 0 && Cout > 0, "conv2d3x3_act: bad sizes");
diff --git a/syn3r_amd/csrc/gemm_common.h b/syn3r_amd/csrc/gemm_common.h
--- a/syn3r_amd/csrc/gemm_common.h
+++ b/syn3r_amd/csrc/gemm_common.h
@@ -45,6 +45,7 @@
     const __half* relu_mask;
     float* gn_part; int gn_units;
     unsigned a_bytes;
+    int up4_bpi;
 };
 
 __device__ __forceinline__ long long tiled_off(int m, int d, int D) {
diff --git a/syn3r_amd/csrc/gemm_wide.h b/syn3r_amd/csrc/gemm_wide.h
--- a/syn3r_amd/csrc/gemm_wide.h
+++ b/syn3r_amd/csrc/gemm_wide.h
@@ -8,8 +8,8 @@
 __device__ unsigned long long g_wide_timing[64];
 #endif
 
-template <int NI>
-__device__ __forceinline__ void gn_tile_stats(const GemmParams& p, const __half* st, int lane, int gm0, int gn0, int N) {
+template <int NI, bool UP4 = false>
+__device__ __forceinline__ void gn_tile_stats(const GemmParams& p, const __half* st, int lane, int gm0, int gn0, int N, int ph = 0) {
     typedef _Float16 half2e __attribute__((ext_vector_type(2)));
     constexpr int NU = NI == 4 ? 8 : 4, NC = NI == 4 ? 10 : 5;
     const int row = NI == 4 ? lane : (lane & 31);
@@ -44,16 +44,20 @@
         const int m = gm0 + (NI == 4 ? 32 * (rowp >> 1) : 0);
         const int n = gn0 + (NI == 4 ? 0 : 40 * (rowp >> 1));
         if (m < p.M && n < N) {
-            float* dst = p.gn_part + ((size_t)(m >> 5) * 2 + (rowp & 1)) * (size_t)p.gn_units + n / 10;
+            int slot = m >> 5;
+            if constexpr (UP4) { const int img = slot / p.up4_bpi; slot += (3 * img + ph) * p.up4_bpi; }
+            float* dst = p.gn_part + ((size_t)slot * 2 + (rowp & 1)) * (size_t)p.gn_units + n / 10;
 #pragma unroll
             for (int u = 0; u < NU; u += 4) *(float4v*)(dst + u) = (float4v){w[u], w[u + 1], w[u + 2], w[u + 3]};
         }
     }
 }
 
-template <int NI, bool HOIST = false>
+template <int NI, bool HOIST = false, bool UP4 = false>
 __device__ __forceinline__ void lean_store(const GemmParams& p, float4v (*acc)[TN], __half* st, int lane, int gm0,
-                                           int gn0, int N, const __half* bias, const __half* residual, const __half* aux, bool full) {
+                                           int gn0, int N, const __half* bias, const __half* residual, const __half* aux, bool full,
+                                           int orow = 0, int ph = 0) {
+    static_assert(!UP4 || NI == 4, "UP4: one lane per row of the tile");
     typedef _Float16 half4e __attribute__((ext_vector_type(4)));
     const int fr = lane & 15, fq = lane >> 4;
     const __half* rv[NI];
@@ -124,10 +128,10 @@
     __builtin_amdgcn_wave_barrier();
     static_assert(NI % 2 == 0, "lean_store: an even number of row tiles");
     constexpr int NQ = NI * 16 * (WN / 8) / 64;
-    auto put = [&](int m, int n, const half8& v) {
+    auto put = [&](int m, int n, const half8& v, int mo = -1) {
         if (!(full || (m < p.M && n < N))) return;
         if (p.out_tiled) OUT_STORE((half8*)(p.out + tiled_off(m, n, N)), v);
-        else OUT_STORE((half8*)(p.out + (long long)m * p.ldc + n), v);
+        else OUT_STORE((half8*)(p.out + (long long)(UP4 ? mo : m) * p.ldc + n), v);
     };
     if (residual && aux) {
         constexpr int RB = 5;
@@ -180,19 +184,22 @@
         for (int it = 0; it < NQ; ++it) {
             const int q = lane + it * 64, row = q / (WN / 8), ch = q - row * (WN / 8);
             const half8 v = *(const half8*)(st + row * EPI_LD + ch * 8);
-            put(gm0 + row, gn0 + ch * 8, v);
+            if constexpr (UP4) put(gm0 + row, gn0 + ch * 8, v, __builtin_amdgcn_ds_bpermute(row << 2, orow));
+            else put(gm0 + row, gn0 + ch * 8, v);
         }
     }
     __builtin_amdgcn_wave_barrier();
     if (p.gn_part) {
-        gn_tile_stats<NI>(p, st, lane, gm0, gn0, N);
+        gn_tile_stats<NI, UP4>(p, st, lane, gm0, gn0, N, ph);
         __builtin_amdgcn_wave_barrier();
     }
 }
 
+template <bool UP4 = false>
 __device__ __forceinline__ void widep_store(const GemmParams& p, float4v (&acc)[TM][TN], char* epi, int lane, int wv, int gm0,
-                                            int gn0, int N, const __half* bias, const __half* residual, const __half* aux, bool full) {
-    lean_store<TM>(p, acc, (__half*)epi + wv * (WM * EPI_LD), lane, gm0, gn0, N, bias, residual, aux, full);
+                                            int gn0, int N, const __half* bias, const __half* residual, const __half* aux, bool full,
+                                            int orow = 0, int ph = 0) {
+    lean_store<TM, false, UP4>(p, acc, (__half*)epi + wv * (WM * EPI_LD), lane, gm0, gn0, N, bias, residual, aux, full, orow, ph);
 }
 
 __global__ void __launch_bounds__(512, 2) k_gemm_widep(GemmParams p) {
diff --git a/syn3r_amd/csrc/gemm_z.h b/syn3r_amd/csrc/gemm_z.h
--- a/syn3r_amd/csrc/gemm_z.h
+++ b/syn3r_amd/csrc/gemm_z.h
@@ -30,22 +30,26 @@
         asm volatile("s_waitcnt lgkmcnt(%1)" : "+v"(bf[Q % RB]) : "i"(N));
 }
 
-template <bool TWOSRC, int MODE, bool UPS = false>
+template <bool TWOSRC, int MODE, bool UPS = false, bool UP4 = false>
 __global__ void __launch_bounds__(512, 2) k_gemm_z(GemmParams p) {
     static_assert(!UPS || MODE == MODE_CONV2D, "UPS is a conv2d option");
+    static_assert(!UP4 || (MODE == MODE_CONV2D && !UPS), "UP4 is a conv2d option of its own");
     extern __shared__ __attribute__((aligned(16))) char smem_raw[];
     const int tid = threadIdx.x, lane = tid & 63;
     const int wv = __builtin_amdgcn_readfirstlane(tid >> 6);
     const int wm = wv >> 1, wn = wv & 1;
     const int tiles_n = (p.N + WBN - 1) / WBN;
     const int tiles_m = (p.M + WBM - 1) / WBM;
-    const unsigned nblk = (unsigned)(tiles_m * tiles_n);
+    const unsigned per_ph = (unsigned)(tiles_m * tiles_n);
+    const unsigned nblk = UP4 ? 4u * per_ph : per_ph;
     const XcdTiles tiles = xcd_tiles(nblk);
     const int nkt = p.K / BK;
     const unsigned bw0 = p.band > 0 ? (unsigned)p.band : 4u;
     const unsigned bw = (unsigned)tiles_n >= bw0 ? bw0 : (unsigned)tiles_n;
     const unsigned band_sz = (unsigned)tiles_m * bw, full_bands = (unsigned)tiles_n / bw;
-    auto tile_origin = [&](unsigned tile, int& m0, int& n0, int& tn) {
+    auto tile_origin = [&](unsigned tile, int& m0, int& n0, int& tn, int& ph) {
+        ph = 0;
+        if constexpr (UP4) { const unsigned q = tile / per_ph; ph = (int)q; tile -= q * per_ph; }
         unsigned b = tile / band_sz, w = bw, t2 = tile - b * band_sz;
         if (b >= full_bands) { b = full_bands; t2 = tile - full_bands * band_sz; w = (unsigned)tiles_n - full_bands * bw; }
         tn = (int)(b * bw + t2 % w);
@@ -57,7 +61,7 @@
     const char* abase = (const char*)p.A;
     const int kt_switch = TWOSRC ? p.K1 / BK : 0x7fffffff;
     unsigned c_tl = blockIdx.x / 8;
-    int c_ks = 0, c_m0 = 0;
+    int c_ks = 0, c_m0 = 0, c_ph = 0;
     unsigned c_slot = 0;
     unsigned voff_a, voff_a2 = 0, voff_b;
     {
@@ -102,7 +106,15 @@
                 unsigned r, x;
                 const unsigned n = udiv(m, d_hw, r_hw, r), y = udiv(r, d_w, r_w, x);
                 unsigned f = 0;
-                if constexpr (UPS) {
+                if constexpr (UP4) {
+                    const int y0 = (int)y + (c_ph >> 1) - 1, x0 = (int)x + (c_ph & 1) - 1;
+                    cv_base[i] = (unsigned)(((int)(n * (unsigned)p.Hi) + y0) * p.Wi + x0) * (unsigned)p.Cin * 2u + lanechunk;
+#pragma unroll
+                    for (int t = 0; t < 2; ++t) {
+                        f |= (unsigned)(y0 + t >= 0 && y0 + t < p.Hi) << t;
+                        f |= (unsigned)(x0 + t >= 0 && x0 + t < p.Wi) << (3 + t);
+                    }
+                } else if constexpr (UPS) {
                     const int yu = (int)y - 1, xu = (int)x - 1;
                     const int y0 = yu >> 1, x0 = xu >> 1;
                     cv_base[i] = (unsigned)(((int)(n * (unsigned)p.Hi) + y0) * p.Wi + x0) * (unsigned)p.Cin * 2u + lanechunk;
@@ -146,7 +158,7 @@
         if (c_tl >= tiles.len) return;
         if (c_ks == 0) {
             int n0_, tn_;
-            tile_origin(tiles.start + c_tl, c_m0, n0_, tn_);
+            tile_origin(tiles.start + c_tl, c_m0, n0_, tn_, c_ph);
             abase = (const char*)p.A;
             second = false;
             if constexpr (MODE != MODE_DENSE) { c_tap = 0; c_left = 0; c_chunk = 0; }
@@ -163,6 +175,7 @@
                 int n = n0_ + (wv * 5 + j) * 8;
                 n = n < p.N - 8 ? n : p.N - 8;
                 ob[j] = 2u * (unsigned)n * (unsigned)p.K;
+                if constexpr (UP4) ob[j] += (unsigned)c_ph * (2u * (unsigned)p.N * (unsigned)p.K);
             }
             if constexpr (MODE != MODE_DENSE) __builtin_amdgcn_s_waitcnt(0x0F70);
         } else if (TWOSRC && c_ks == kt_switch) {
@@ -183,7 +196,8 @@
             for (int j = 0; j < 5; ++j) ob[j] += 2u * BK;
         }
         if constexpr (MODE == MODE_CONV2D) {
-            const int ty = c_tap / 3, tx = c_tap - 3 * ty;
+            constexpr int TW = UP4 ? 2 : 3;
+            const int ty = c_tap / TW, tx = c_tap - TW * ty;
             if constexpr (UPS) {
                 tap_off = (((ty == 2 ? p.Wi : 0) + (tx == 2 ? 1 : 0)) * p.Cin + c_chunk * BK) * 2;
                 add_y = ty == 1 ? (unsigned)(p.Wi * p.Cin * 2) : 0u;
@@ -193,7 +207,7 @@
             }
             tap_mask = (1u << ty) | (8u << tx);
             kb = (unsigned)(c_tap * p.Cin + c_chunk * BK) * 2u;
-            if (++c_tap == 9) { c_tap = 0; ++c_chunk; }
+            if (++c_tap == TW * TW) { c_tap = 0; ++c_chunk; }
         } else if constexpr (MODE == MODE_TCONV) {
             if (c_left == 0) { conv_tap(c_tap); ++c_tap; c_left = cpb; }
             else {
@@ -288,8 +302,8 @@
 #define ZSTAMP(i)
 #endif
     for (unsigned tl = blockIdx.x / 8; tl < tiles.len; tl += tiles.stride) {
-        int m0, n0, tile_n;
-        tile_origin(tiles.start + tl, m0, n0, tile_n);
+        int m0, n0, tile_n, ph;
+        tile_origin(tiles.start + tl, m0, n0, tile_n, ph);
         if constexpr (MODE != MODE_DENSE) {
             if (c_ks == 1 && c_m0 == m0) {
                 conv_tile();
@@ -395,8 +409,17 @@
         } else {
             const int gn0 = n0 + wn * 160;
             const bool full = gm0 + WM <= p.M && gn0 + 160 <= p.N;
-            widep_store(p, acc[0], epi, le, wv, gm0, gn0, p.N, p.bias, p.residual, p.aux, full);
-            widep_store(p, acc[1], epi, le, wv, gm0, gn0 + WN, p.N, p.bias, p.residual, p.aux, full);
+            if constexpr (UP4) {
+                unsigned m = (unsigned)(gm0 + le), r, x;
+                m = m < (unsigned)p.M ? m : (unsigned)p.M - 1u;
+                const unsigned n = udiv(m, d_hw, r_hw, r), y = udiv(r, d_w, r_w, x);
+                const int orow = (int)((n * 2u * (unsigned)p.Hi + 2u * y + (unsigned)(ph >> 1)) * 2u * (unsigned)p.Wi + 2u * x + (unsigned)(ph & 1));
+                widep_store<true>(p, acc[0], epi, le, wv, gm0, gn0, p.N, p.bias, nullptr, nullptr, full, orow, ph);
+                widep_store<true>(p, acc[1], epi, le, wv, gm0, gn0 + WN, p.N, p.bias, nullptr, nullptr, full, orow, ph);
+            } else {
+                widep_store(p, acc[0], epi, le, wv, gm0, gn0, p.N, p.bias, p.residual, p.aux, full);
+                widep_store(p, acc[1], epi, le, wv, gm0, gn0 + WN, p.N, p.bias, p.residual, p.aux, full);
+            }
         }
         __builtin_amdgcn_s_barrier();
         ZSTAMP(6);
diff --git a/syn3r_amd/csrc/unet.hip b/syn3r_amd/csrc/unet.hip
--- a/syn3r_amd/csrc/unet.hip
+++ b/syn3r_amd/csrc/unet.hip
@@ -387,6 +387,13 @@
         b.resize((b.size() + 7) / 8 * 8, 0);
         for (auto& hp : packs) if (hp.name == "conv_out.bias") { hp.rows = (long long)b.size(); hp.cols = 1; hp.d = b; }
     }
+    for (size_t i = 0, n = packs.size(); i < n; ++i) {
+        if (!has_suffix(packs[i].name, ".upsamplers.0.conv.weight")) continue;
+        const long long O = packs[i].rows, I = packs[i].cols / 9;
+        HostPack hp; hp.name = packs[i].name + "_up4"; hp.rows = 4 * O; hp.cols = 4 * I; hp.d.resize((size_t)(16 * O * I));
+        if (syn3r_pack_upsample4_f16(packs[i].d.data(), hp.d.data(), (int)O, (int)I) != SYN3R_OK) return SYN3R_E_INVALID;
+        packs.push_back(std::move(hp));
+    }
     for (auto& kv : names) {
         const std::string& k = kv.first;
         if (has_suffix(k, "attn1.to_q.weight")) {
@@ -465,6 +472,36 @@
 
 }
 
+extern "C" int syn3r_pack_upsample4_f16(const void* w, void* w4, int Cout, int Cin) {
+    SYN3R_REQUIRE(w && w4, "pack_upsample4: null operand");
+    SYN3R_REQUIRE(Cout > 0 && Cin > 0 && Cout <= (1 << 15) && Cin <= (1 << 15), "pack_upsample4: bad sizes Cout=%d Cin=%d", Cout, Cin);
+    const _Float16* src = (const _Float16*)w;
+    _Float16* dst = (_Float16*)w4;
+    const size_t C = (size_t)Cin;
+    for (int ph = 0; ph < 4; ++ph) {
+        const int py = ph >> 1, px = ph & 1;
+        for (int o = 0; o < Cout; ++o)
+            for (int a = 0; a < 2; ++a)
+                for (int b = 0; b < 2; ++b) {
+                    const int ty0 = py == 0 ? (a == 0 ? 0 : 1) : (a == 0 ? 0 : 2), ty1 = py == 0 ? (a == 0 ? 0 : 2) : (a == 0 ? 1 : 2);
+                    const int tx0 = px == 0 ? (b == 0 ? 0 : 1) : (b == 0 ? 0 : 2), tx1 = px == 0 ? (b == 0 ? 0 : 2) : (b == 0 ? 1 : 2);
+                    _Float16* d = dst + ((((size_t)ph * Cout + o) * 2 + a) * 2 + b) * C;
+                    for (size_t c = 0; c < C; ++c) {
+                        float s = 0.f;
+                        bool first = true;
+                        for (int ty = ty0; ty <= ty1; ++ty)
+                            for (int tx = tx0; tx <= tx1; ++tx) {
+                                const float v = (float)src[(((size_t)o * 3 + ty) * 3 + tx) * C + c];
+                                s = first ? v : s + v;
+                                first = false;
+                            }
+                        d[c] = (_Float16)s;
+                    }
+                }
+    }
+    return SYN3R_OK;
+}
+
 namespace {
 int unet_create_impl(const char* weights_dir, const char* variant, syn3r_unet** out);
 }
@@ -682,6 +719,15 @@
         if (go())
             chk(syn3r_conv2d3x3_f16(x.p, wt->p, out.p, Cout, Wp(bname), e.rowvec, e.ldrv, e.rows_per_vec, e.residual ? e.residual->p : nullptr,
                                     e.residual ? Cout : 0, e.s_acc, e.s_res, NB, Hi, Wi, Cin, Cout, stride, ups ? 1 : 0, 1, out.gnp, gnb, &out.gn_ok, stream));
+        return out;
+    }
+    T conv3x3_up4(const T& x, int NB, int Hi, int Wi, int Cin, const std::string& wname, const std::string& bname, int* Ho_, int* Wo_) {
+        const Wt* wt = W(wname + "_up4");
+        const int Cout = wt ? (int)(wt->rows / 4) : 0;
+        *Ho_ = 2 * Hi; *Wo_ = 2 * Wi;
+        T out = make((long long)NB * 4 * Hi * Wi, Cout);
+        const size_t gnb = gn_begin(out, true);
+        if (go()) chk(syn3r_conv2d3x3_up4_f16(x.p, wt->p, out.p, Wp(bname), nullptr, NB, Hi, Wi, Cin, Cout, out.gnp, gnb, &out.gn_ok, stream));
         return out;
     }
     T tconv3(const T& x, const std::string& wname, const std::string& bname, int HW, const Epi& e) {
@@ -1037,7 +1083,7 @@
             }
             if (bp.resample) {
                 int Ho, Wo;
-                T y = conv3x3(x, B * F, h, w, bp.ch, bpre + ".upsamplers.0.conv.weight", bpre + ".upsamplers.0.conv.bias", 1, true, Epi(), &Ho, &Wo);
+                T y = conv3x3_up4(x, B * F, h, w, bp.ch, bpre + ".upsamplers.0.conv.weight", bpre + ".upsamplers.0.conv.bias", &Ho, &Wo);
                 drop(x);
                 h = Ho; w = Wo;
                 x = y;
diff --git a/syn3r_amd/unet/model.py b/syn3r_amd/unet/model.py
--- a/syn3r_amd/unet/model.py
+++ b/syn3r_amd/unet/model.py
@@ -256,6 +256,8 @@
                 if w.shape[0] % 8:
                     w = Fn.pad(w, (0, 0, 0, 0, 0, 0, 0, 8 - w.shape[0] % 8))
                 pk[k] = w.permute(0, 2, 3, 1).contiguous()
+                if k.endswith(".upsamplers.0.conv.weight"):
+                    pk[k + "_up4"] = ops.pack_upsample4(pk[k])
             elif k.endswith(".weight") and t.dim() == 5:
                 pk[k] = t[..., 0, 0].permute(0, 2, 1).contiguous()
             elif k.endswith("conv_shortcut.weight"):
@@ -506,8 +508,8 @@
                     x = self._transformer(f"up_blocks.{i}.attentions.{j}", x, st, cout, blk["heads"])
             if blk["up"]:
                 ch = blk["ch"]
-                x = ops.conv3x3(x.view(B * F, st["h"], st["w"], ch), W(f"up_blocks.{i}.upsamplers.0.conv.weight"),
-                                W(f"up_blocks.{i}.upsamplers.0.conv.bias"), upsample=True, gn_stats=TUNE["gn_epilogue"])
+                x = ops.conv3x3_up4(x.view(B * F, st["h"], st["w"], ch), W(f"up_blocks.{i}.upsamplers.0.conv.weight_up4"),
+                                    W(f"up_blocks.{i}.upsamplers.0.conv.bias"), gn_stats=TUNE["gn_epilogue"])
                 st["h"], st["w"] = x.shape[1], x.shape[2]
                 x = ops.keep_gn(x.view(-1, ch), x)
         x = ops.groupnorm(x, W("conv_norm_out.weight"), W("conv_norm_out.bias"), B * F, 1e-5, True)
diff --git a/syn3r_amd/unet/ops.py b/syn3r_amd/unet/ops.py
--- a/syn3r_amd/unet/ops.py
+++ b/syn3r_amd/unet/ops.py
@@ -225,6 +225,39 @@
     return _gn_collect(out, part, gn[2])
 
 
+def pack_upsample4(weight: torch.Tensor) -> torch.Tensor:
+    if weight.dim() != 4 or tuple(weight.shape[1:3]) != (3, 3):
+        raise ValueError(f"pack_upsample4: weight {tuple(weight.shape)} is not [Cout,3,3,Cin]")
+    groups = (((0,), (1, 2)), ((0, 1), (2,)))
+    w = weight.float()
+    out = torch.empty((4, weight.shape[0], 2, 2, weight.shape[3]), dtype=H, device=weight.device)
+    for py in range(2):
+        for px in range(2):
+            for a in range(2):
+                for b in range(2):
+                    acc = None
+                    for ty in groups[py][a]:
+                        for tx in groups[px][b]:
+                            acc = w[:, ty, tx] if acc is None else acc + w[:, ty, tx]
+                    out[2 * py + px, :, a, b] = acc.to(H)
+    return out
+
+
+def conv3x3_up4(x: torch.Tensor, w4: torch.Tensor, bias: Optional[torch.Tensor] = None, *, gn_stats: bool = False) -> torch.Tensor:
+    dev = _chk(x, w4, bias)
+    NB, Hi, Wi, Cin = x.shape
+    if w4.dim() != 5 or w4.shape[0] != 4 or tuple(w4.shape[2:]) != (2, 2, Cin):
+        raise ValueError(f"conv3x3_up4: w4 {tuple(w4.shape)} does not match Cin={Cin}")
+    Cout = w4.shape[1]
+    out = torch.empty((NB, 2 * Hi, 2 * Wi, Cout), dtype=H, device=dev)
+    lib = L.load()
+    part, gn = _gn_request(dev, NB * 4 * Hi * Wi, Cout, gn_stats)
+    rc = lib.syn3r_conv2d3x3_up4_f16(L.ptr(x), L.ptr(w4), L.ptr(out), L.ptr(bias), None, NB, Hi, Wi, Cin, Cout, *gn, L.stream_ptr(dev))
+    L.check(rc, "syn3r_conv2d3x3_up4_f16")
+    _count("gemm", 2.0 * NB * 4 * Hi * Wi * Cout * 4 * Cin)
+    return _gn_collect(out, part, gn[2])
+
+
 def tconv3(x: torch.Tensor, weight: torch.Tensor, bias: Optional[torch.Tensor], B: int, F: int, HW: int, *,
            rowvec: Optional[torch.Tensor] = None, rows_per_vec: int = 0, residual: Optional[torch.Tensor] = None,
            s_acc: float = 1.0, s_res: float = 1.0, gn_stats: bool = False) -> torch.Tensor:
```

New measurement: 418.2 iters/s (median of 6 runs). +1.6%, better.
